# zenghjian/SceneSplat

Hardware: AMD Instinct MI355X
Metric: Gaussians/s encoder fwd+bwd, 102k-pt chunks (higher is better)
Workload: dtype bf16

## Files before the change

include/scenesplat_hip.h:

```cpp
#ifndef SCENESPLAT_HIP_H
#define SCENESPLAT_HIP_H
#include <stddef.h>
#include <stdint.h>

#ifdef __cplusplus
extern "C" {
#endif

struct ihipStream_t;
typedef struct ihipStream_t* ss_stream_t;

#define SS_MAX_ORDERS 8
enum { SS_ORDER_Z = 0, SS_ORDER_Z_TRANS = 1, SS_ORDER_HILBERT = 2, SS_ORDER_HILBERT_TRANS = 3 };
enum { SS_DTYPE_F32 = 0, SS_DTYPE_BF16 = 1 };
enum { SS_ATTN_SIMT = 0, SS_ATTN_MFMA = 1 };

int ss_version(void);

int ss_serialize_encode(const int32_t* grid_coord, const int32_t* batch, int64_t n, int depth, const int* orders,
                        int num_orders, int64_t* codes, ss_stream_t stream);
int ss_offsets_to_batch(const int32_t* offsets, int num_batches, int64_t n, int32_t* batch, ss_stream_t stream);
int ss_count_duplicates(const int64_t* sorted_keys, int64_t n, int32_t* count, ss_stream_t stream);
int ss_grid_coord_max(const int32_t* grid_coord, int64_t n, int32_t* out_max, ss_stream_t stream);
size_t ss_argsort_workspace_bytes(int64_t n, int num_segments);
int ss_argsort_i64(const int64_t* keys, int num_segments, int64_t n, int key_bits, int32_t* order_out,
                   int32_t* inverse_out, int64_t* sorted_keys_out, void* workspace, size_t workspace_bytes,
                   ss_stream_t stream);

size_t ss_pool_partition_workspace_bytes(int64_t n);
int ss_pool_partition(const int64_t* code0, const int32_t* order0, int64_t n, int shift_bits, int32_t* cluster,
                      int32_t* idx_ptr, int32_t* head, int32_t* n_out, void* workspace, size_t workspace_bytes,
                      ss_stream_t stream);
int ss_pool_level_attrs(const int32_t* head, int64_t n_out, int64_t n_in, const int32_t* grid_coord,
                        const int32_t* batch, const int64_t* codes, int num_orders, int pool_depth,
                        int32_t* grid_coord_out, int32_t* batch_out, int64_t* codes_out, ss_stream_t stream);
int ss_batch_offsets(const int32_t* batch, const int32_t* perm, int64_t n, int num_batches, int32_t* offsets,
                     ss_stream_t stream);

int ss_window_index(const int32_t* order, const int32_t* offsets, const int32_t* offsets_pad, int num_batches,
                    int patch_size, int64_t n_pad, int32_t* gidx, int32_t* sidx, ss_stream_t stream);
int ss_window_attn_fwd(const void* qkv, const int32_t* gidx, const int32_t* sidx, const int32_t* win_start,
                       int num_windows, int max_window, int64_t n, int64_t n_pad, int channels, int num_heads,
                       float scale, int dtype, int impl, void* out, float* lse, ss_stream_t stream);
size_t ss_window_attn_bwd_workspace_bytes(int64_t n, int64_t n_pad, int channels, int num_heads, int dtype);
int ss_window_attn_bwd(const void* qkv, const void* out, const void* dout, const float* lse, const int32_t* gidx,
                       const int32_t* sidx, const int32_t* win_start, int num_windows, int max_window, int64_t n,
                       int64_t n_pad, int channels, int num_heads, float scale, int dtype, int impl, void* dqkv,
                       void* workspace, size_t workspace_bytes, ss_stream_t stream);

int ss_cast_bf16_group(const int64_t* desc, const int32_t* wg_start, int nprob, int total_workgroups, ss_stream_t stream);
int ss_cast_bf16_group_elems_per_workgroup(void);

int ss_optim_group_elems_per_workgroup(void);
int ss_grad_sqnorm_group(const int64_t* desc, const int32_t* wg_start, int nprob, int total_workgroups, double* partials,
                         ss_stream_t stream);
int ss_grad_norm_finish(const double* partials, int num_partials, float max_norm, float* record, ss_stream_t stream);
int ss_adamw_group(const int64_t* desc, const int32_t* wg_start, int nprob, int total_workgroups, const float* record,
                   ss_stream_t stream);

int ss_pdnorm_channels_per_workgroup(void);
int ss_pdnorm_mod_fwd(const int64_t* table, const int32_t* wg_start, int num_layers, int total_workgroups, const float* context,
                      int context_channels, int vec4, ss_stream_t stream);
int ss_pdnorm_mod_bwd(const int64_t* table, const int32_t* wg_start, int num_layers, int total_workgroups, const float* context,
                      int context_channels, int vec4, int split_workgroup, float* partials, float* dcontext, ss_stream_t stream);

int ss_row_keep_scales(const int64_t* seed, const float* keep, float* out, int64_t n, ss_stream_t stream);

int ss_gelu(const void* x, const void* dy, void* out, int64_t numel, int dtype, ss_stream_t stream);

int ss_stream_capture_status(ss_stream_t stream);
unsigned long long ss_stream_capture_id(ss_stream_t stream);

int ss_linear_fwd_headmajor(const void* x, const int32_t* row_index, const void* weight, const float* bias, void* out_hm,
                            int64_t m, int k, int n_out, int channels, int head_dim, float sec0_scale, ss_stream_t stream);
int ss_headmajor_pack(const void* src, int in_dtype, const int32_t* gidx, void* hm, int64_t n_pad, int channels,
                      int num_heads, int sections, float sec0_scale, ss_stream_t stream);
int ss_window_attn_hm_fwd(const void* hm, const int32_t* sidx, const int32_t* win_start, int num_windows, int max_window,
                          int64_t n, int64_t n_pad, int channels, int num_heads, void* out, float* neg_lse2,
                          ss_stream_t stream);
size_t ss_window_attn_hm_bwd_workspace_bytes(int64_t n, int64_t n_pad, int channels, int num_heads);
int ss_window_attn_hm_bwd(const void* hm, const void* out, const void* dout, const float* neg_lse2, const int32_t* gidx,
                          const int32_t* sidx, const int32_t* win_start, int num_windows, int max_window, int64_t n,
                          int64_t n_pad, int channels, int num_heads, float scale, void* dqkv, void* workspace,
                          size_t workspace_bytes, ss_stream_t stream);

int ss_window_attn_rpe_fwd(const void* qkv, const int32_t* gidx, const int32_t* sidx, const int32_t* win_start,
                           int num_windows, int max_window, int64_t n, int64_t n_pad, int channels, int num_heads,
                           float scale, int dtype, int impl, const int32_t* grid_coord, const float* table, int pos_bnd,
                           void* out, float* lse, ss_stream_t stream);
size_t ss_window_attn_rpe_bwd_workspace_bytes(int64_t n, int64_t n_pad, int channels, int num_heads, int dtype,
                                              int num_windows, int max_window, int pos_bnd);
int ss_window_attn_rpe_bwd(const void* qkv, const void* out, const void* dout, const float* lse, const int32_t* gidx,
                           const int32_t* sidx, const int32_t* win_start, int num_windows, int max_window, int64_t n,
                           int64_t n_pad, int channels, int num_heads, float scale, int dtype, int impl,
                           const int32_t* grid_coord, const float* table, int pos_bnd, void* dqkv, float* dtable,
                           void* workspace, size_t workspace_bytes, ss_stream_t stream);

int ss_subm_rulebook(const int32_t* grid_coord, const int32_t* batch, int64_t n, int depth,
                     const int64_t* zkeys_sorted, const int32_t* zorder, int swap_xy, int kernel_size, int32_t* nbr,
                     ss_stream_t stream);
int ss_subm_tap_mask_keys(const int32_t* nbr, const int32_t* order, int64_t n, int taps, int coarse_bits, int64_t* keys,
                          ss_stream_t stream);
int64_t ss_subm_rulebook_table_size(int64_t n);
int ss_subm_rulebook_hashed(const int32_t* grid_coord, const int32_t* batch, int64_t n, int depth, int kernel_size, int32_t* nbr,
                            void* workspace, size_t workspace_bytes, ss_stream_t stream);

int ss_subm_conv_fwd(const void* in, const void* weight, const float* bias, const int32_t* nbr, const int32_t* rowperm,
                     void* out, int64_t n, int cin, int cout, int taps, int out_dtype, ss_stream_t stream);
int ss_subm_weight_mirror(const void* w, void* wt, int cout, int taps, int cin, ss_stream_t stream);
int ss_stream_create_cu_mask(int nwords, const uint32_t* mask, void** stream_out);
int ss_subm_im2col(const void* src, const int32_t* nbr, void* dst, int64_t n, int taps, int64_t row_bytes, ss_stream_t stream);
int ss_gemm8_ok(int64_t m, int k, int n, int taps);
int ss_subm_conv_fwd_pipe(const void* in, const void* weight, const float* bias, const int32_t* nbr, const int32_t* rowperm,
                          void* out, int64_t n, int cin, int cout, int taps, int out_dtype, ss_stream_t stream);
int ss_subm_conv_fwd_pipe_walk(const void* in, const void* weight, const float* bias, const int32_t* nbr_walk, const int32_t* rowperm,
                               void* out, int64_t n, int cin, int cout, int taps, int out_dtype, ss_stream_t stream);
int ss_subm_conv_fwd_uses_pipe(int64_t n, int cin, int cout, int taps);
int ss_subm_conv_fwd_walk(const void* in, const void* weight, const float* bias, const int32_t* nbr, const int32_t* nbr_walk,
                          const int32_t* rowperm, void* out, int64_t n, int cin, int cout, int taps, int out_dtype, ss_stream_t stream);
int ss_linear_fwd(const void* x, const void* weight, const float* bias, void* out, int64_t m, int k, int n, int out_dtype,
                  ss_stream_t stream);
int ss_wgrad_xcd_order(void);
int ss_wgrad_set_xcd_order(int on);
int ss_wgrad8_ok(int64_t n, int cin, int cout, int taps);
int ss_subm_conv_wgrad_pipe(const void* in, const void* dout, const int32_t* nbr, const int32_t* rowperm,
                            const int32_t* blk_count, const int32_t* blk_list, float* dweight, int64_t n, int cin, int cout,
                            int taps, ss_stream_t stream);
int ss_linear_wgrad(const void* x, const void* dy, float* dweight, float* dbias, int64_t m, int k_in, int n_out,
                    ss_stream_t stream);
int ss_linear_wgrad_group_plan(int64_t m, int k_in, int n_out, int64_t* desc_words);
int ss_linear_wgrad_tiles(int k_in, int n_out);
int ss_linear_wgrad_group_plan2(int64_t m, int k_in, int n_out, int launch_tiles, int64_t* desc_words);
int ss_linear_wgrad_group(const int64_t* desc, const int32_t* wg_start, int nprob, int total_workgroups, ss_stream_t stream);
int ss_subm_conv_splits(int64_t n, int cout, int taps);
int ss_subm_conv_fwd_splitk(const void* in, const void* weight, const float* bias, const int32_t* nbr, const int32_t* rowperm,
                            float* acc32, int64_t n, int cin, int cout, int taps, int splits, ss_stream_t stream);
int ss_subm_block_lists(const int32_t* nbr, const int32_t* rowperm, int64_t n, int taps, int32_t* blk_count,
                        int32_t* blk_list, ss_stream_t stream);
int ss_subm_conv_wgrad(const void* in, const void* dout, const int32_t* nbr, const int32_t* rowperm,
                       const int32_t* blk_count, const int32_t* blk_list, float* dweight, int64_t n, int cin, int cout,
                       int taps, ss_stream_t stream);

int ss_subm_f32_ok(int cin_padded, int cout);
int ss_subm_f32_fwd(const float* in, const float* wq, const float* bias, const int32_t* nbr_walk, const int32_t* rowperm,
                    float* out, int64_t n, int cin_padded, int cout, int taps, ss_stream_t stream);
int ss_subm_f32_dgrad_dup(const float* dout_folded, const float* wq, const int32_t* nbr_walk, const int32_t* rowperm, float* din,
                          int64_t n, int cin_padded, int cout, int taps, ss_stream_t stream);
int ss_subm_f32_wgrad(const float* in, const float* dout, const int32_t* nbr_walk, const int32_t* rowperm,
                      const int32_t* blk_count, const int32_t* blk_list, float* dweight, int64_t n, int cin_padded,
                      int cin, int cout, int taps, ss_stream_t stream);

int ss_subm_conv_wgrad_pipe_walk(const void* in, const void* dout, const int32_t* nbr_walk, const int32_t* rowperm,
                                 const int32_t* blk_count, const int32_t* blk_list, float* dweight, int64_t n, int cin, int cout,
                                 int taps, ss_stream_t stream);
int ss_subm_conv_wgrad_uses_pipe(int64_t n, int cin, int cout, int taps);
int ss_subm_conv_wgrad_walk(const void* in, const void* dout, const int32_t* nbr, const int32_t* nbr_walk, const int32_t* rowperm,
                            const int32_t* blk_count, const int32_t* blk_list, float* dweight, int64_t n, int cin, int cout,
                            int taps, ss_stream_t stream);

int ss_add_layernorm_fwd(const void* x, int x_dtype, const void* y, int y_dtype, const float* rowscale,
                         const float* gamma, const float* beta, float eps, void* xout, int xout_dtype, void* xcopy_bf16,
                         void* h, int h_dtype, float* mean, float* rstd, int64_t n, int channels, ss_stream_t stream);
int ss_ln_add_ln_fwd(const void* x, int x_dtype, const void* t, int t_dtype, const float* gamma0, const float* beta0, float eps0,
                     const float* gamma1, const float* beta1, float eps1, float* xout, void* h, int h_dtype, float* stats,
                     int64_t n, int channels, ss_stream_t stream);
int ss_ln_add_ln_bwd(const float* g_xout, const void* g_h, int g_h_dtype, const float* xout, const void* t, int t_dtype,
                     const float* stats, const float* gamma0, const float* gamma1, void* g_x, int g_x_dtype, void* g_t,
                     int g_t_dtype, float* part, int64_t n, int channels, int nblocks, ss_stream_t stream);
int ss_add_layernorm_bwd_blocks(int64_t n);
int ss_group_partial_sums_outputs_per_workgroup(void);
int ss_group_partial_sums(const int64_t* desc, const int32_t* wg_start, int nprob, int total_workgroups, ss_stream_t stream);
int ss_transpose16_group(const int64_t* desc, const int32_t* wg_start, int nprob, int total_workgroups, ss_stream_t stream);
int ss_subm_weight_mirror_group_tile(void);
int ss_subm_weight_mirror_group(const int64_t* desc, const int32_t* wg_start, int nprob, int total_workgroups, ss_stream_t stream);
int ss_add_layernorm_bwd(const void* g_xout, int g_xout_dtype, const void* g_xcopy, int g_xcopy_dtype, const void* g_h,
                         int g_h_dtype, const void* v, int v_dtype, const float* mean, const float* rstd,
                         const float* gamma, const float* rowscale, void* g_x, int g_x_dtype, void* g_y, int g_y_dtype,
                         float* dgamma_part, float* dbeta_part, int64_t n, int channels, int nblocks, ss_stream_t stream);

int ss_col_stats(const void* x, int x_dtype, float* shift_out, float* psum, float* psq, int64_t n, int channels,
                 int nblocks, ss_stream_t stream);
int ss_bn_stats_finish(const float* part, const float* shift, int nblocks, int channels, int64_t n, float momentum, float eps,
                       float* running_mean, float* running_var, int64_t* num_batches, float* mean, float* rstd,
                       ss_stream_t stream);
int ss_bn_bwd_finish(const float* part, int nblocks, int channels, int64_t n, float* sums, float* coef, ss_stream_t stream);
int ss_bn_act_fwd(const void* x, int x_dtype, const float* mean, const float* rstd, const float* gamma, const float* beta,
                  int act, void* y, int y_dtype, int64_t n, int channels, ss_stream_t stream);
int ss_bn_act_bwd_reduce(const void* dy, int dy_dtype, const void* x, int x_dtype, const float* mean, const float* rstd,
                         const float* gamma, const float* beta, int act, float* pdz, float* pdzx, int64_t n, int channels,
                         int nblocks, ss_stream_t stream);
int ss_bn_act_bwd_apply(const void* dy, int dy_dtype, const void* x, int x_dtype, const float* mean, const float* rstd,
                        const float* gamma, const float* beta, int act, const float* c1, const float* c2, void* dx,
                        int dx_dtype, int64_t n, int channels, ss_stream_t stream);

int ss_feat_text_scan(const void* feat_bf16, const void* text_bf16, int64_t n, int dim, int num_classes, float* max_prob,
                      int32_t* argmax, const int32_t* idx, float* pred_accum, ss_stream_t stream);

int ss_lang_head_blocks(int64_t n);
int ss_lang_head_fwd(const void* feat, int feat_dtype, const void* target, int target_dtype, const unsigned char* mask,
                     int normalize, void* p_out, int p_dtype, float* rowstat, float* part, float* sums, int64_t n,
                     int channels, ss_stream_t stream);
int ss_lang_head_bwd(const void* feat, int feat_dtype, const void* target, int target_dtype, const unsigned char* mask,
                     int normalize, const float* rowstat, const float* coef, const void* dp_extra, int dp_dtype,
                     void* dfeat, int dfeat_dtype, int64_t n, int channels, ss_stream_t stream);

size_t ss_seg_loss_workspace_bytes(int64_t n, int num_classes);
int ss_seg_loss_fwd(const void* logits, int dtype, const int64_t* labels, int64_t n, int num_classes, int64_t ignore_index,
                    const unsigned char* class_seen, int lovasz, float* rowstat, float* glov, int32_t* present, float* sums,
                    void* workspace, size_t workspace_bytes, ss_stream_t stream);
int ss_seg_loss_bwd(const void* logits, int dtype, const int64_t* labels, int64_t n, int num_classes, int64_t ignore_index,
                    const float* rowstat, const float* glov, const int32_t* present, const float* coef, void* dlogits,
                    ss_stream_t stream);
int ss_seg_iou(const void* logits, int dtype, const int32_t* pred, const int64_t* target, int64_t n, int num_classes,
               int64_t ignore_index, int64_t* out, ss_stream_t stream);

int ss_gather_rows(const void* src, const int32_t* idx, void* dst, int64_t n_dst, int64_t row_bytes, ss_stream_t stream);
int ss_scatter_rows(const void* src, const int32_t* idx, void* dst, int64_t n_src, int64_t row_bytes, ss_stream_t stream);
int ss_gather_add_rows(const void* a, const void* b, const int32_t* idx, void* dst, int64_t n, int channels, int dtype,
                       ss_stream_t stream);
int ss_dup_fold_rows(const void* src, const int64_t* sorted_keys, const int32_t* order, void* dst, int64_t n, int channels,
                     int dtype, ss_stream_t stream);
int ss_dup_zero_rows(const int64_t* sorted_keys, const int32_t* order, void* x, int64_t n, int64_t row_bytes, ss_stream_t stream);
int ss_segment_reduce(const void* src, const int32_t* indices, const int32_t* idx_ptr, void* out, int64_t n_seg,
                      int channels, int dtype, int mean, ss_stream_t stream);
int ss_segment_minmax(const void* src, const int32_t* indices, const int32_t* idx_ptr, void* out, int32_t* arg, int64_t n_seg,
                      int channels, int dtype, int is_max, ss_stream_t stream);
int ss_segment_minmax_bwd(const void* dout, const int32_t* arg, void* dsrc, int64_t n_seg, int channels, int dtype,
                          ss_stream_t stream);
int ss_segment_bcast(const void* dout, const int32_t* cluster, const int32_t* idx_ptr, void* dsrc, int64_t n,
                     int channels, int dtype, int mean, ss_stream_t stream);


int ss_aug_bbox_blocks(int64_t n);
int ss_aug_bbox(const float* x, int64_t n, const float* h_affine, float* partials, float* out6, ss_stream_t stream);
int ss_aug_gaussians(float* coord, float* quat, float* scale, float* normal, int64_t n, const float* h_affine,
                     const float* h_rquat, int flip, const float* h_scale_mul, const float* h_lin, int jitter, float jitter_sigma,
                     float jitter_clip, const float* noise, uint64_t seed, ss_stream_t stream);
int ss_aug_elastic(float* coord, int64_t n, const float* noise, int d0, int d1, int d2, const float* h_origin, float granularity,
                   float magnitude, ss_stream_t stream);
int ss_aug_color(float* color, int64_t n, int flags, const float* h_lo, const float* h_hi, float blend, const float* h_tr,
                 float jitter_std, const float* noise, uint64_t seed, int normalize, ss_stream_t stream);

int ss_knn_query(int m, int nsample, const float* xyz, const float* new_xyz, const int32_t* offset,
                 const int32_t* new_offset, int num_batches, int32_t* idx, float* dist2, ss_stream_t stream);
size_t ss_ball_query_workspace_bytes(int m);
int ss_ball_query(int m, int nsample, float min_radius, float max_radius, const float* xyz, const float* new_xyz,
                  const int32_t* offset, const int32_t* new_offset, int num_batches, int32_t* idx, float* dist2,
                  void* workspace, size_t workspace_bytes, ss_stream_t stream);
int ss_random_ball_query(int m, int nsample, float min_radius, float max_radius, const int32_t* order, const float* xyz,
                         const float* new_xyz, const int32_t* offset, const int32_t* new_offset, int num_batches,
                         int32_t* idx, float* dist2, ss_stream_t stream);
int ss_farthest_point_sampling(int num_batches, const float* xyz, const int32_t* offset, const int32_t* new_offset,
                               float* tmp, int32_t* idx, ss_stream_t stream);
int ss_grouping_fwd(int m, int nsample, int c, const float* input, const int32_t* idx, float* output, ss_stream_t stream);
int ss_grouping_bwd(int m, int nsample, int c, const float* grad_output, const int32_t* idx, float* grad_input, ss_stream_t stream);
int ss_subtraction_fwd(int n, int nsample, int c, const float* input1, const float* input2, const int32_t* idx, float* output, ss_stream_t stream);
int ss_subtraction_bwd(int n, int nsample, int c, const int32_t* idx, const float* grad_output, float* grad_input1, float* grad_input2, ss_stream_t stream);
int ss_aggregation_fwd(int n, int nsample, int c, int w_c, const float* input, const float* position, const float* weight, const int32_t* idx, float* output, ss_stream_t stream);
int ss_aggregation_bwd(int n, int nsample, int c, int w_c, const float* input, const float* position, const float* weight, const int32_t* idx, const float* grad_output, float* grad_input, float* grad_position, float* grad_weight, ss_stream_t stream);
int ss_interpolation_fwd(int n, int c, int k, const float* input, const int32_t* idx, const float* weight, float* output, ss_stream_t stream);
int ss_interpolation_bwd(int n, int c, int k, const float* grad_output, const int32_t* idx, const float* weight, float* grad_input, ss_stream_t stream);
int ss_attention_relation_fwd(int m, int g, int c, const float* query, const float* key, const float* weight, const int32_t* index_target, const int32_t* index_refer, float* output, ss_stream_t stream);
int ss_attention_relation_bwd(int m, int g, int c, const float* query, float* grad_query, const float* key, float* grad_key, const float* weight, float* grad_weight, const int32_t* index_target, const int32_t* index_refer, const float* grad_output, ss_stream_t stream);
int ss_attention_fusion_fwd(int m, int g, int c, const float* weight, const float* value, const int32_t* index_target, const int32_t* index_refer, float* output, ss_stream_t stream);
int ss_attention_fusion_bwd(int m, int g, int c, const float* weight, float* grad_weight, const float* value, float* grad_value, const int32_t* index_target, const int32_t* index_refer, const float* grad_output, ss_stream_t stream);
int ss_rpe_dot_prod_fwd(int n, int m, int h, int hdim, const float* q, const int32_t* index, const float* table, const int32_t* rel_idx, float* output, ss_stream_t stream);
int ss_rpe_dot_prod_bwd(int n, int m, int h, int hdim, const float* grad_out, const float* q, const int32_t* index, const float* table, const int32_t* rel_idx, float* grad_q, float* grad_table, ss_stream_t stream);
int ss_rpe_attn_step2_fwd(int n, int m, int h, int hdim, const float* attn, const float* v, const int32_t* index0, const int32_t* index1, const float* table, const int32_t* rel_idx, float* output, ss_stream_t stream);
int ss_rpe_attn_step2_bwd(int n, int m, int h, int hdim, const float* grad_out, const int32_t* index0, const int32_t* index1, const float* attn, const float* v, const float* table, const int32_t* rel_idx, float* grad_attn, float* grad_v, float* grad_table, ss_stream_t stream);
int64_t ss_knn_grid_table_size(int64_t n);
size_t ss_knn_grid_workspace_bytes(int64_t n);
int ss_knn_grid_keys(const float* xyz, const int32_t* offset, int num_batches, int64_t n, float origin_x, float origin_y, float origin_z,
                     float cell_size, int64_t* keys, ss_stream_t stream);
int ss_knn_grid_build(const float* xyz, const int64_t* sorted_keys, const int32_t* order, int64_t n, void* workspace,
                      size_t workspace_bytes, int32_t* ncell, ss_stream_t stream);
int ss_knn_grid_query(int m, int nsample, const float* new_xyz, const int32_t* qorder, const int32_t* offset, const int32_t* new_offset,
                      int num_batches, float origin_x, float origin_y, float origin_z, float cell_size, int dimx, int dimy, int dimz,
                      int64_t n, const void* workspace, int32_t* idx, float* dist2, ss_stream_t stream);
int ss_ball_grid_query(int m, int nsample, float min_radius, float max_radius, const float* xyz, const float* new_xyz,
                       const int32_t* qorder, const int32_t* offset, const int32_t* new_offset, int num_batches, float origin_x,
                       float origin_y, float origin_z, float cell_size, int dimx, int dimy, int dimz, int64_t n, const void* workspace,
                       int32_t* idx, float* dist2, ss_stream_t stream);
int ss_majority_vote(const int32_t* nn_idx, const int32_t* labels, int64_t m, int k, int ignore_label, int num_classes,
                     int32_t* out, ss_stream_t stream);
int ss_ballquery_batch_p(int n, int mean_active, float radius, const float* xyz, const int32_t* batch_idxs, const int32_t* batch_offsets, int32_t* idx, int32_t* start_len, int32_t* total, ss_stream_t stream);
int ss_bfs_cluster(const int32_t* semantic_label, const int32_t* ball_query_idxs, const int32_t* start_len, int n, int threshold, int32_t* cluster_idxs, int64_t cap_points, int32_t* cluster_offsets, int64_t cap_clusters, int32_t* n_clusters, int32_t* n_points);

#ifdef __cplusplus
}
#endif
#endif
```

scenesplat_amd/_lib.py:

```python
import ctypes
import os

import torch

_HERE = os.path.dirname(os.path.abspath(__file__))
LIB_PATH = os.path.join(_HERE, "lib", "libscenesplat_hip.so")

c_p = ctypes.c_void_p
c_i = ctypes.c_int
c_i64 = ctypes.c_int64
c_f = ctypes.c_float
c_sz = ctypes.c_size_t

PROTOTYPES = {
    "ss_version": (c_i, []),
    "ss_serialize_encode": (c_i, [c_p, c_p, c_i64, c_i, ctypes.POINTER(c_i), c_i, c_p, c_p]),
    "ss_offsets_to_batch": (c_i, [c_p, c_i, c_i64, c_p, c_p]),
    "ss_count_duplicates": (c_i, [c_p, c_i64, c_p, c_p]),
    "ss_grid_coord_max": (c_i, [c_p, c_i64, c_p, c_p]),
    "ss_argsort_workspace_bytes": (c_sz, [c_i64, c_i]),
    "ss_argsort_i64": (c_i, [c_p, c_i, c_i64, c_i, c_p, c_p, c_p, c_p, c_sz, c_p]),
    "ss_pool_partition_workspace_bytes": (c_sz, [c_i64]),
    "ss_pool_partition": (c_i, [c_p, c_p, c_i64, c_i, c_p, c_p, c_p, c_p, c_p, c_sz, c_p]),
    "ss_pool_level_attrs": (c_i, [c_p, c_i64, c_i64, c_p, c_p, c_p, c_i, c_i, c_p, c_p, c_p, c_p]),
    "ss_batch_offsets": (c_i, [c_p, c_p, c_i64, c_i, c_p, c_p]),
    "ss_window_index": (c_i, [c_p, c_p, c_p, c_i, c_i, c_i64, c_p, c_p, c_p]),
    "ss_window_attn_fwd": (c_i, [c_p, c_p, c_p, c_p, c_i, c_i, c_i64, c_i64, c_i, c_i, c_f, c_i, c_i, c_p, c_p, c_p]),
    "ss_window_attn_bwd_workspace_bytes": (c_sz, [c_i64, c_i64, c_i, c_i, c_i]),
    "ss_window_attn_bwd": (c_i, [c_p, c_p, c_p, c_p, c_p, c_p, c_p, c_i, c_i, c_i64, c_i64, c_i, c_i, c_f, c_i, c_i,
                                 c_p, c_p, c_sz, c_p]),
    "ss_window_attn_rpe_fwd": (c_i, [c_p, c_p, c_p, c_p, c_i, c_i, c_i64, c_i64, c_i, c_i, c_f, c_i, c_i, c_p, c_p, c_i,
                                     c_p, c_p, c_p]),
    "ss_window_attn_rpe_bwd_workspace_bytes": (c_sz, [c_i64, c_i64, c_i, c_i, c_i, c_i, c_i, c_i]),
    "ss_window_attn_rpe_bwd": (c_i, [c_p, c_p, c_p, c_p, c_p, c_p, c_p, c_i, c_i, c_i64, c_i64, c_i, c_i, c_f, c_i, c_i,
                                     c_p, c_p, c_i, c_p, c_p, c_p, c_sz, c_p]),
    "ss_gelu": (c_i, [c_p, c_p, c_p, c_i64, c_i, c_p]),
    "ss_row_keep_scales": (c_i, [c_p, c_p, c_p, c_i64, c_p]),
    "ss_stream_capture_status": (c_i, [c_p]),
    "ss_stream_capture_id": (ctypes.c_ulonglong, [c_p]),
    "ss_cast_bf16_group": (c_i, [c_p, c_p, c_i, c_i, c_p]),
    "ss_cast_bf16_group_elems_per_workgroup": (c_i, []),
    "ss_optim_group_elems_per_workgroup": (c_i, []),
    "ss_grad_sqnorm_group": (c_i, [c_p, c_p, c_i, c_i, c_p, c_p]),
    "ss_grad_norm_finish": (c_i, [c_p, c_i, c_f, c_p, c_p]),
    "ss_adamw_group": (c_i, [c_p, c_p, c_i, c_i, c_p, c_p]),
    "ss_pdnorm_channels_per_workgroup": (c_i, []),
    "ss_pdnorm_mod_fwd": (c_i, [c_p, c_p, c_i, c_i, c_p, c_i, c_i, c_p]),
    "ss_pdnorm_mod_bwd": (c_i, [c_p, c_p, c_i, c_i, c_p, c_i, c_i, c_i, c_p, c_p, c_p]),
    "ss_linear_fwd_headmajor": (c_i, [c_p, c_p, c_p, c_p, c_p, c_i64, c_i, c_i, c_i, c_i, c_f, c_p]),
    "ss_headmajor_pack": (c_i, [c_p, c_i, c_p, c_p, c_i64, c_i, c_i, c_i, c_f, c_p]),
    "ss_window_attn_hm_fwd": (c_i, [c_p, c_p, c_p, c_i, c_i, c_i64, c_i64, c_i, c_i, c_p, c_p, c_p]),
    "ss_window_attn_hm_bwd_workspace_bytes": (c_sz, [c_i64, c_i64, c_i, c_i]),
    "ss_window_attn_hm_bwd": (c_i, [c_p, c_p, c_p, c_p, c_p, c_p, c_p, c_i, c_i, c_i64, c_i64, c_i, c_i, c_f, c_p, c_p, c_sz, c_p]),
    "ss_subm_rulebook": (c_i, [c_p, c_p, c_i64, c_i, c_p, c_p, c_i, c_i, c_p, c_p]),
    "ss_subm_conv_fwd": (c_i, [c_p, c_p, c_p, c_p, c_p, c_p, c_i64, c_i, c_i, c_i, c_i, c_p]),
    "ss_stream_create_cu_mask": (c_i, [c_i, c_p, c_p]),
    "ss_ln_add_ln_fwd": (c_i, [c_p, c_i, c_p, c_i, c_p, c_p, c_f, c_p, c_p, c_f, c_p, c_p, c_i, c_p, c_i64, c_i, c_p]),
    "ss_ln_add_ln_bwd": (c_i, [c_p, c_p, c_i, c_p, c_p, c_i, c_p, c_p, c_p, c_p, c_i, c_p, c_i, c_p, c_i64, c_i, c_i, c_p]),
    "ss_segment_minmax": (c_i, [c_p, c_p, c_p, c_p, c_p, c_i64, c_i, c_i, c_i, c_p]),
    "ss_segment_minmax_bwd": (c_i, [c_p, c_p, c_p, c_i64, c_i, c_i, c_p]),
    "ss_subm_rulebook_table_size": (c_i64, [c_i64]),
    "ss_subm_rulebook_hashed": (c_i, [c_p, c_p, c_i64, c_i, c_i, c_p, c_p, ctypes.c_size_t, c_p]),
    "ss_subm_tap_mask_keys": (c_i, [c_p, c_p, c_i64, c_i, c_i, c_p, c_p]),
    "ss_subm_weight_mirror": (c_i, [c_p, c_p, c_i, c_i, c_i, c_p]),
    "ss_subm_im2col": (c_i, [c_p, c_p, c_p, c_i64, c_i, c_i64, c_p]),
    "ss_gemm8_ok": (c_i, [c_i64, c_i, c_i, c_i]),
    "ss_subm_conv_fwd_pipe": (c_i, [c_p, c_p, c_p, c_p, c_p, c_p, c_i64, c_i, c_i, c_i, c_i, c_p]),
    "ss_linear_fwd": (c_i, [c_p, c_p, c_p, c_p, c_i64, c_i, c_i, c_i, c_p]),
    "ss_wgrad_xcd_order": (c_i, []),
    "ss_wgrad_set_xcd_order": (c_i, [c_i]),
    "ss_wgrad8_ok": (c_i, [c_i64, c_i, c_i, c_i]),
    "ss_subm_conv_wgrad_pipe": (c_i, [c_p, c_p, c_p, c_p, c_p, c_p, c_p, c_i64, c_i, c_i, c_i, c_p]),
    "ss_linear_wgrad": (c_i, [c_p, c_p, c_p, c_p, c_i64, c_i, c_i, c_p]),
    "ss_linear_wgrad_group_plan": (c_i, [c_i64, c_i, c_i, c_p]),
    "ss_linear_wgrad_tiles": (c_i, [c_i, c_i]),
    "ss_linear_wgrad_group_plan2": (c_i, [c_i64, c_i, c_i, c_i, c_p]),
    "ss_linear_wgrad_group": (c_i, [c_p, c_p, c_i, c_i, c_p]),
    "ss_subm_conv_splits": (c_i, [c_i64, c_i, c_i]),
    "ss_subm_conv_fwd_splitk": (c_i, [c_p, c_p, c_p, c_p, c_p, c_p, c_i64, c_i, c_i, c_i, c_i, c_p]),
    "ss_subm_block_lists": (c_i, [c_p, c_p, c_i64, c_i, c_p, c_p, c_p]),
    "ss_subm_conv_wgrad": (c_i, [c_p, c_p, c_p, c_p, c_p, c_p, c_p, c_i64, c_i, c_i, c_i, c_p]),
    "ss_subm_conv_fwd_pipe_walk": (c_i, [c_p, c_p, c_p, c_p, c_p, c_p, c_i64, c_i, c_i, c_i, c_i, c_p]),
    "ss_subm_conv_fwd_uses_pipe": (c_i, [c_i64, c_i, c_i, c_i]),
    "ss_subm_conv_fwd_walk": (c_i, [c_p, c_p, c_p, c_p, c_p, c_p, c_p, c_i64, c_i, c_i, c_i, c_i, c_p]),
    "ss_subm_conv_wgrad_pipe_walk": (c_i, [c_p, c_p, c_p, c_p, c_p, c_p, c_p, c_i64, c_i, c_i, c_i, c_p]),
    "ss_subm_conv_wgrad_uses_pipe": (c_i, [c_i64, c_i, c_i, c_i]),
    "ss_subm_conv_wgrad_walk": (c_i, [c_p, c_p, c_p, c_p, c_p, c_p, c_p, c_p, c_i64, c_i, c_i, c_i, c_p]),
    "ss_subm_f32_ok": (c_i, [c_i, c_i]),
    "ss_subm_f32_fwd": (c_i, [c_p, c_p, c_p, c_p, c_p, c_p, c_i64, c_i, c_i, c_i, c_p]),
    "ss_subm_f32_dgrad_dup": (c_i, [c_p, c_p, c_p, c_p, c_p, c_i64, c_i, c_i, c_i, c_p]),
    "ss_dup_fold_rows": (c_i, [c_p, c_p, c_p, c_p, c_i64, c_i, c_i, c_p]),
    "ss_dup_zero_rows": (c_i, [c_p, c_p, c_p, c_i64, c_i64, c_p]),
    "ss_subm_f32_wgrad": (c_i, [c_p, c_p, c_p, c_p, c_p, c_p, c_p, c_i64, c_i, c_i, c_i, c_i, c_p]),
    "ss_add_layernorm_fwd": (c_i, [c_p, c_i, c_p, c_i, c_p, c_p, c_p, c_f, c_p, c_i, c_p, c_p, c_i, c_p, c_p, c_i64, c_i, c_p]),
    "ss_add_layernorm_bwd_blocks": (c_i, [c_i64]),
    "ss_group_partial_sums_outputs_per_workgroup": (c_i, []),
    "ss_group_partial_sums": (c_i, [c_p, c_p, c_i, c_i, c_p]),
    "ss_transpose16_group": (c_i, [c_p, c_p, c_i, c_i, c_p]),
    "ss_subm_weight_mirror_group_tile": (c_i, []),
    "ss_subm_weight_mirror_group": (c_i, [c_p, c_p, c_i, c_i, c_p]),
    "ss_add_layernorm_bwd": (c_i, [c_p, c_i, c_p, c_i, c_p, c_i, c_p, c_i, c_p, c_p, c_p, c_p, c_p, c_i, c_p, c_i, c_p, c_p,
                                   c_i64, c_i, c_i, c_p]),
    "ss_col_stats": (c_i, [c_p, c_i, c_p, c_p, c_p, c_i64, c_i, c_i, c_p]),
    "ss_bn_stats_finish": (c_i, [c_p, c_p, c_i, c_i, c_i64, c_f, c_f, c_p, c_p, c_p, c_p, c_p, c_p]),
    "ss_bn_bwd_finish": (c_i, [c_p, c_i, c_i, c_i64, c_p, c_p, c_p]),
    "ss_bn_act_fwd": (c_i, [c_p, c_i, c_p, c_p, c_p, c_p, c_i, c_p, c_i, c_i64, c_i, c_p]),
    "ss_bn_act_bwd_reduce": (c_i, [c_p, c_i, c_p, c_i, c_p, c_p, c_p, c_p, c_i, c_p, c_p, c_i64, c_i, c_i, c_p]),
    "ss_bn_act_bwd_apply": (c_i, [c_p, c_i, c_p, c_i, c_p, c_p, c_p, c_p, c_i, c_p, c_p, c_p, c_i, c_i64, c_i, c_p]),
    "ss_feat_text_scan": (c_i, [c_p, c_p, c_i64, c_i, c_i, c_p, c_p, c_p, c_p, c_p]),
    "ss_lang_head_blocks": (c_i, [c_i64]),
    "ss_lang_head_fwd": (c_i, [c_p, c_i, c_p, c_i, c_p, c_i, c_p, c_i, c_p, c_p, c_p, c_i64, c_i, c_p]),
    "ss_lang_head_bwd": (c_i, [c_p, c_i, c_p, c_i, c_p, c_i, c_p, c_p, c_p, c_i, c_p, c_i, c_i64, c_i, c_p]),
    "ss_seg_loss_workspace_bytes": (c_sz, [c_i64, c_i]),
    "ss_seg_loss_fwd": (c_i, [c_p, c_i, c_p, c_i64, c_i, c_i64, c_p, c_i, c_p, c_p, c_p, c_p, c_p, c_sz, c_p]),
    "ss_seg_loss_bwd": (c_i, [c_p, c_i, c_p, c_i64, c_i, c_i64, c_p, c_p, c_p, c_p, c_p, c_p]),
    "ss_seg_iou": (c_i, [c_p, c_i, c_p, c_p, c_i64, c_i, c_i64, c_p, c_p]),
    "ss_gather_rows": (c_i, [c_p, c_p, c_p, c_i64, c_i64, c_p]),
    "ss_scatter_rows": (c_i, [c_p, c_p, c_p, c_i64, c_i64, c_p]),
    "ss_gather_add_rows": (c_i, [c_p, c_p, c_p, c_p, c_i64, c_i, c_i, c_p]),
    "ss_segment_reduce": (c_i, [c_p, c_p, c_p, c_p, c_i64, c_i, c_i, c_i, c_p]),
    "ss_segment_bcast": (c_i, [c_p, c_p, c_p, c_p, c_i64, c_i, c_i, c_i, c_p]),
    "ss_aug_bbox_blocks": (c_i, [c_i64]),
    "ss_aug_bbox": (c_i, [c_p, c_i64, c_p, c_p, c_p, c_p]),
    "ss_aug_gaussians": (c_i, [c_p, c_p, c_p, c_p, c_i64, c_p, c_p, c_i, c_p, c_p, c_i, c_f, c_f, c_p, ctypes.c_uint64, c_p]),
    "ss_aug_elastic": (c_i, [c_p, c_i64, c_p, c_i, c_i, c_i, c_p, c_f, c_f, c_p]),
    "ss_aug_color": (c_i, [c_p, c_i64, c_i, c_p, c_p, c_f, c_p, c_f, c_p, ctypes.c_uint64, c_i, c_p]),
    "ss_knn_grid_table_size": (c_i64, [c_i64]),
    "ss_knn_grid_workspace_bytes": (c_sz, [c_i64]),
    "ss_knn_grid_keys": (c_i, [c_p, c_p, c_i, c_i64, c_f, c_f, c_f, c_f, c_p, c_p]),
    "ss_knn_grid_build": (c_i, [c_p, c_p, c_p, c_i64, c_p, c_sz, c_p, c_p]),
    "ss_knn_grid_query": (c_i, [c_i, c_i, c_p, c_p, c_p, c_p, c_i, c_f, c_f, c_f, c_f, c_i, c_i, c_i, c_i64, c_p, c_p, c_p, c_p]),
    "ss_ball_grid_query": (c_i, [c_i, c_i, c_f, c_f, c_p, c_p, c_p, c_p, c_p, c_i, c_f, c_f, c_f, c_f, c_i, c_i, c_i, c_i64, c_p, c_p, c_p, c_p]),
    "ss_knn_query": (c_i, [c_i, c_i, c_p, c_p, c_p, c_p, c_i, c_p, c_p, c_p]),
    "ss_ball_query_workspace_bytes": (c_sz, [c_i]),
    "ss_ball_query": (c_i, [c_i, c_i, c_f, c_f, c_p, c_p, c_p, c_p, c_i, c_p, c_p, c_p, c_sz, c_p]),
    "ss_random_ball_query": (c_i, [c_i, c_i, c_f, c_f, c_p, c_p, c_p, c_p, c_p, c_i, c_p, c_p, c_p]),
    "ss_farthest_point_sampling": (c_i, [c_i, c_p, c_p, c_p, c_p, c_p, c_p]),
    "ss_grouping_fwd": (c_i, [c_i, c_i, c_i, c_p, c_p, c_p, c_p]),
    "ss_grouping_bwd": (c_i, [c_i, c_i, c_i, c_p, c_p, c_p, c_p]),
    "ss_subtraction_fwd": (c_i, [c_i, c_i, c_i, c_p, c_p, c_p, c_p, c_p]),
    "ss_subtraction_bwd": (c_i, [c_i, c_i, c_i, c_p, c_p, c_p, c_p, c_p]),
    "ss_aggregation_fwd": (c_i, [c_i, c_i, c_i, c_i, c_p, c_p, c_p, c_p, c_p, c_p]),
    "ss_aggregation_bwd": (c_i, [c_i, c_i, c_i, c_i, c_p, c_p, c_p, c_p, c_p, c_p, c_p, c_p, c_p]),
    "ss_interpolation_fwd": (c_i, [c_i, c_i, c_i, c_p, c_p, c_p, c_p, c_p]),
    "ss_interpolation_bwd": (c_i, [c_i, c_i, c_i, c_p, c_p, c_p, c_p, c_p]),
    "ss_attention_relation_fwd": (c_i, [c_i, c_i, c_i, c_p, c_p, c_p, c_p, c_p, c_p, c_p]),
    "ss_attention_relation_bwd": (c_i, [c_i, c_i, c_i, c_p, c_p, c_p, c_p, c_p, c_p, c_p, c_p, c_p, c_p]),
    "ss_attention_fusion_fwd": (c_i, [c_i, c_i, c_i, c_p, c_p, c_p, c_p, c_p, c_p]),
    "ss_attention_fusion_bwd": (c_i, [c_i, c_i, c_i, c_p, c_p, c_p, c_p, c_p, c_p, c_p, c_p]),
    "ss_rpe_dot_prod_fwd": (c_i, [c_i, c_i, c_i, c_i, c_p, c_p, c_p, c_p, c_p, c_p]),
    "ss_rpe_dot_prod_bwd": (c_i, [c_i, c_i, c_i, c_i, c_p, c_p, c_p, c_p, c_p, c_p, c_p, c_p]),
    "ss_rpe_attn_step2_fwd": (c_i, [c_i, c_i, c_i, c_i, c_p, c_p, c_p, c_p, c_p, c_p, c_p, c_p]),
    "ss_rpe_attn_step2_bwd": (c_i, [c_i, c_i, c_i, c_i, c_p, c_p, c_p, c_p, c_p, c_p, c_p, c_p, c_p, c_p, c_p]),
    "ss_majority_vote": (c_i, [c_p, c_p, c_i64, c_i, c_i, c_i, c_p, c_p]),
    "ss_ballquery_batch_p": (c_i, [c_i, c_i, c_f, c_p, c_p, c_p, c_p, c_p, c_p, c_p]),
    "ss_bfs_cluster": (c_i, [c_p, c_p, c_p, c_i, c_i, c_p, c_i64, c_p, c_i64, c_p, c_p]),
}

_lib = None


def load():
    global _lib
    if _lib is not None:
        return _lib
    if not os.path.exists(LIB_PATH):
        raise RuntimeError(
            f"{LIB_PATH} is missing: build it with `python -m scenesplat_amd.build` "
            "(hipcc --offload-arch=gfx950). scenesplat_amd has no CPU fallback.")
    lib = ctypes.CDLL(LIB_PATH)
    for name, (res, args) in PROTOTYPES.items():
        fn = getattr(lib, name)
        fn.restype = res
        fn.argtypes = args
    _lib = lib
    return lib


class NativeError(RuntimeError):
    pass


_STATUS = {1: "bad argument", 2: "kernel launch failed", 3: "workspace too small"}


def check(rc, name):
    if rc != 0:
        raise NativeError(f"{name} failed: status {rc} ({_STATUS.get(rc, 'unknown')})")
```

scenesplat_amd/csrc/norm.hip:

```cpp
#include "common.h"
#include "../../include/scenesplat_hip.h"

#define LN_THREADS 256
#define LN_MAXIT 4

__device__ __forceinline__ float4 ln_ld4(const void* p, int dtype, int64_t idx) {
  if (dtype == SS_F32) return *reinterpret_cast<const float4*>((const float*)p + idx);
  uint2 u = *reinterpret_cast<const uint2*>((const unsigned short*)p + idx);
  return make_float4(__uint_as_float(u.x << 16), __uint_as_float(u.x & 0xffff0000u), __uint_as_float(u.y << 16),
                     __uint_as_float(u.y & 0xffff0000u));
}
__device__ __forceinline__ void ln_st4(void* p, int dtype, int64_t idx, float4 v) {
  if (dtype == SS_F32) { *reinterpret_cast<float4*>((float*)p + idx) = v; return; }
  uint2 u; u.x = pack_bf16x2(v.x, v.y); u.y = pack_bf16x2(v.z, v.w);
  *reinterpret_cast<uint2*>((unsigned short*)p + idx) = u;
}

template <int IT>
__global__ void __launch_bounds__(LN_THREADS)
k_add_ln_fwd(const void* __restrict__ x, int x_dt, const void* __restrict__ y, int y_dt, const float* __restrict__ rowscale,
             const float* __restrict__ gamma, const float* __restrict__ beta, float eps, void* __restrict__ xout, int xout_dt,
             void* __restrict__ xcopy, void* __restrict__ h, int h_dt, float* __restrict__ mean, float* __restrict__ rstd,
             int64_t n, int C) {
  const int lane = threadIdx.x & 63;
  const int64_t row = (int64_t)blockIdx.x * (LN_THREADS / 64) + (threadIdx.x >> 6);
  if (row >= n) return;
  const float rs = rowscale ? rowscale[row] : 1.f;
  float4 v[IT];
  float sum = 0.f;
#pragma unroll
  for (int i = 0; i < IT; ++i) {
    int j = i * 256 + lane * 4;
    v[i] = make_float4(0.f, 0.f, 0.f, 0.f);
    if (j < C) {
      float4 a = ln_ld4(x, x_dt, row * C + j);
      if (y) { float4 b = ln_ld4(y, y_dt, row * C + j); a.x += rs * b.x; a.y += rs * b.y; a.z += rs * b.z; a.w += rs * b.w; }
      v[i] = a;
      if (xout) ln_st4(xout, xout_dt, row * C + j, a);
      if (xcopy) ln_st4(xcopy, SS_BF16, row * C + j, a);
      sum += a.x + a.y + a.z + a.w;
    }
  }
  if (!gamma) return;
  const float mu = wave_reduce_sum(sum) / C;
  float sq = 0.f;
#pragma unroll
  for (int i = 0; i < IT; ++i) {
    int j = i * 256 + lane * 4;
    if (j < C) {
      float dx = v[i].x - mu, dy = v[i].y - mu, dz = v[i].z - mu, dw = v[i].w - mu;
      sq += dx * dx + dy * dy + dz * dz + dw * dw;
    }
  }
  const float r = rsqrtf(wave_reduce_sum(sq) / C + eps);
  if (lane == 0) { mean[row] = mu; rstd[row] = r; }
#pragma unroll
  for (int i = 0; i < IT; ++i) {
    int j = i * 256 + lane * 4;
    if (j < C) {
      float4 g = *reinterpret_cast<const float4*>(gamma + j), b = *reinterpret_cast<const float4*>(beta + j);
      float4 o = make_float4((v[i].x - mu) * r * g.x + b.x, (v[i].y - mu) * r * g.y + b.y, (v[i].z - mu) * r * g.z + b.z,
                             (v[i].w - mu) * r * g.w + b.w);
      ln_st4(h, h_dt, row * C + j, o);
    }
  }
}

template <int IT>
__global__ void __launch_bounds__(LN_THREADS)
k_add_ln_bwd(const void* __restrict__ g_xout, int gxo_dt, const void* __restrict__ g_xcopy, int gxc_dt,
             const void* __restrict__ g_h, int gh_dt,
             const void* __restrict__ v_in, int v_dt, const float* __restrict__ mean, const float* __restrict__ rstd,
             const float* __restrict__ gamma, const float* __restrict__ rowscale, void* __restrict__ g_x, int gx_dt,
             void* __restrict__ g_y, int gy_dt, float* __restrict__ dgamma_part, float* __restrict__ dbeta_part, int64_t n,
             int C) {
  __shared__ float red[2][LN_THREADS / 64][LN_MAXIT * 256 / 64][64];
  const int lane = threadIdx.x & 63, wave = threadIdx.x >> 6;
  const int waves_total = gridDim.x * (LN_THREADS / 64);
  const bool ln = g_h != nullptr;
  float4 dg[IT], db[IT], gm[IT];
#pragma unroll
  for (int i = 0; i < IT; ++i) {
    dg[i] = make_float4(0.f, 0.f, 0.f, 0.f); db[i] = dg[i]; gm[i] = dg[i];
    int j = i * 256 + lane * 4;
    if (ln && j < C) gm[i] = *reinterpret_cast<const float4*>(gamma + j);
  }
  for (int64_t row = (int64_t)blockIdx.x * (LN_THREADS / 64) + wave; row < n; row += waves_total) {
    float4 gv[IT];
    if (ln) {
      const float mu = mean[row], r = rstd[row];
      float4 xh[IT], gy[IT];
      float c1 = 0.f, c2 = 0.f;
#pragma unroll
      for (int i = 0; i < IT; ++i) {
        int j = i * 256 + lane * 4;
        xh[i] = make_float4(0.f, 0.f, 0.f, 0.f); gy[i] = xh[i];
        if (j < C) {
          float4 a = ln_ld4(v_in, v_dt, row * C + j), g = ln_ld4(g_h, gh_dt, row * C + j);
          xh[i] = make_float4((a.x - mu) * r, (a.y - mu) * r, (a.z - mu) * r, (a.w - mu) * r);
          gy[i] = make_float4(g.x * gm[i].x, g.y * gm[i].y, g.z * gm[i].z, g.w * gm[i].w);
          c1 += gy[i].x + gy[i].y + gy[i].z + gy[i].w;
          c2 += gy[i].x * xh[i].x + gy[i].y * xh[i].y + gy[i].z * xh[i].z + gy[i].w * xh[i].w;
          dg[i].x += g.x * xh[i].x; dg[i].y += g.y * xh[i].y; dg[i].z += g.z * xh[i].z; dg[i].w += g.w * xh[i].w;
          db[i].x += g.x; db[i].y += g.y; db[i].z += g.z; db[i].w += g.w;
        }
      }
      c1 = wave_reduce_sum(c1) / C; c2 = wave_reduce_sum(c2) / C;
#pragma unroll
      for (int i = 0; i < IT; ++i)
        gv[i] = make_float4(r * (gy[i].x - c1 - xh[i].x * c2), r * (gy[i].y - c1 - xh[i].y * c2),
                            r * (gy[i].z - c1 - xh[i].z * c2), r * (gy[i].w - c1 - xh[i].w * c2));
    } else {
#pragma unroll
      for (int i = 0; i < IT; ++i) gv[i] = make_float4(0.f, 0.f, 0.f, 0.f);
    }
    const float rs = rowscale ? rowscale[row] : 1.f;
#pragma unroll
    for (int i = 0; i < IT; ++i) {
      int j = i * 256 + lane * 4;
      if (j < C) {
        if (g_xout) { float4 e = ln_ld4(g_xout, gxo_dt, row * C + j); gv[i].x += e.x; gv[i].y += e.y; gv[i].z += e.z; gv[i].w += e.w; }
        if (g_xcopy) { float4 e = ln_ld4(g_xcopy, gxc_dt, row * C + j); gv[i].x += e.x; gv[i].y += e.y; gv[i].z += e.z; gv[i].w += e.w; }
        if (g_x) ln_st4(g_x, gx_dt, row * C + j, gv[i]);
        if (g_y) ln_st4(g_y, gy_dt, row * C + j, make_float4(rs * gv[i].x, rs * gv[i].y, rs * gv[i].z, rs * gv[i].w));
      }
    }
  }
  if (!ln) return;
#pragma unroll
  for (int i = 0; i < IT; ++i) {
    red[0][wave][i * 4 + 0][lane] = dg[i].x; red[0][wave][i * 4 + 1][lane] = dg[i].y;
    red[0][wave][i * 4 + 2][lane] = dg[i].z; red[0][wave][i * 4 + 3][lane] = dg[i].w;
    red[1][wave][i * 4 + 0][lane] = db[i].x; red[1][wave][i * 4 + 1][lane] = db[i].y;
    red[1][wave][i * 4 + 2][lane] = db[i].z; red[1][wave][i * 4 + 3][lane] = db[i].w;
  }
  __syncthreads();
  if (wave == 0) {
#pragma unroll
    for (int i = 0; i < IT; ++i)
#pragma unroll
      for (int e = 0; e < 4; ++e) {
        int j = i * 256 + lane * 4 + e;
        if (j < C) {
          float a = 0.f, b = 0.f;
          for (int w = 0; w < LN_THREADS / 64; ++w) { a += red[0][w][i * 4 + e][lane]; b += red[1][w][i * 4 + e][lane]; }
          dgamma_part[(int64_t)blockIdx.x * C + j] = a;
          dbeta_part[(int64_t)blockIdx.x * C + j] = b;
        }
      }
  }
}

extern "C" int ss_add_layernorm_fwd(const void* x, int x_dtype, const void* y, int y_dtype, const float* rowscale,
                                    const float* gamma, const float* beta, float eps, void* xout, int xout_dtype,
                                    void* xcopy_bf16, void* h, int h_dtype, float* mean, float* rstd, int64_t n, int channels,
                                    hipStream_t stream) {
  if (n < 0 || channels <= 0 || (channels & 3) || channels > LN_MAXIT * 256) return SS_ERR_ARG;
  if (gamma && (!beta || !h || !mean || !rstd)) return SS_ERR_ARG;
  if (n == 0) return SS_OK;
  dim3 g(ss_div_up(n, LN_THREADS / 64)), b(LN_THREADS);
  const int it = (channels + 255) / 256;
#define SS_LN_FWD(ITN) SS_LAUNCH(k_add_ln_fwd<ITN>, g, b, 0, stream, x, x_dtype, y, y_dtype, rowscale, gamma, beta, eps, xout, xout_dtype, xcopy_bf16, h, h_dtype, mean, rstd, n, channels)
  switch (it) { case 1: SS_LN_FWD(1); break; case 2: SS_LN_FWD(2); break; case 3: SS_LN_FWD(3); break; default: SS_LN_FWD(4); break; }
#undef SS_LN_FWD
  return SS_OK;
}

extern "C" int ss_add_layernorm_bwd_blocks(int64_t n) {
  const int rows_per_wave = n >= 32768 ? 8 : 2;
  int64_t b = (n + (LN_THREADS / 64) * rows_per_wave - 1) / ((LN_THREADS / 64) * rows_per_wave);
  if (b > 1024) b = 1024;
  if (b < 1) b = 1;
  return (int)b;
}

extern "C" int ss_add_layernorm_bwd(const void* g_xout, int g_xout_dtype, const void* g_xcopy, int g_xcopy_dtype,
                                    const void* g_h, int g_h_dtype, const void* v,
                                    int v_dtype, const float* mean, const float* rstd, const float* gamma,
                                    const float* rowscale, void* g_x, int g_x_dtype, void* g_y, int g_y_dtype,
                                    float* dgamma_part, float* dbeta_part, int64_t n, int channels, int nblocks,
                                    hipStream_t stream) {
  if (n < 0 || channels <= 0 || (channels & 3) || channels > LN_MAXIT * 256 || nblocks < 1) return SS_ERR_ARG;
  if (g_h && (!v || !mean || !rstd || !gamma || !dgamma_part || !dbeta_part)) return SS_ERR_ARG;
  if (n == 0) return SS_OK;
  dim3 g(nblocks), b(LN_THREADS);
  const int it = (channels + 255) / 256;
#define SS_LN_BWD(ITN) SS_LAUNCH(k_add_ln_bwd<ITN>, g, b, 0, stream, g_xout, g_xout_dtype, g_xcopy, g_xcopy_dtype, g_h, g_h_dtype, v, v_dtype, mean, rstd, gamma, rowscale, g_x, g_x_dtype, g_y, g_y_dtype, dgamma_part, dbeta_part, n, channels)
  switch (it) { case 1: SS_LN_BWD(1); break; case 2: SS_LN_BWD(2); break; case 3: SS_LN_BWD(3); break; default: SS_LN_BWD(4); break; }
#undef SS_LN_BWD
  return SS_OK;
}

template <int IT>
__global__ void __launch_bounds__(LN_THREADS)
k_ln_add_ln_fwd(const void* __restrict__ x, int x_dt, const void* __restrict__ t, int t_dt, const float* __restrict__ gamma0,
                const float* __restrict__ beta0, float eps0, const float* __restrict__ gamma1, const float* __restrict__ beta1,
                float eps1, float* __restrict__ xout, void* __restrict__ h, int h_dt, float* __restrict__ stats, int64_t n,
                int C) {
  const int lane = threadIdx.x & 63;
  const int64_t row = (int64_t)blockIdx.x * (LN_THREADS / 64) + (threadIdx.x >> 6);
  if (row >= n) return;
  float4 v[IT];
  float sum = 0.f;
#pragma unroll
  for (int i = 0; i < IT; ++i) {
    int j = i * 256 + lane * 4;
    v[i] = make_float4(0.f, 0.f, 0.f, 0.f);
    if (j < C) { v[i] = ln_ld4(t, t_dt, row * C + j); sum += v[i].x + v[i].y + v[i].z + v[i].w; }
  }
  const float mu0 = wave_reduce_sum(sum) / C;
  float sq = 0.f;
#pragma unroll
  for (int i = 0; i < IT; ++i) {
    int j = i * 256 + lane * 4;
    if (j < C) { float a = v[i].x - mu0, b = v[i].y - mu0, c = v[i].z - mu0, d = v[i].w - mu0; sq += a * a + b * b + c * c + d * d; }
  }
  const float r0 = rsqrtf(wave_reduce_sum(sq) / C + eps0);
  sum = 0.f;
#pragma unroll
  for (int i = 0; i < IT; ++i) {
    int j = i * 256 + lane * 4;
    if (j < C) {
      float4 g = *reinterpret_cast<const float4*>(gamma0 + j), b = *reinterpret_cast<const float4*>(beta0 + j);
      float4 a = ln_ld4(x, x_dt, row * C + j);
      a.x += (v[i].x - mu0) * r0 * g.x + b.x; a.y += (v[i].y - mu0) * r0 * g.y + b.y;
      a.z += (v[i].z - mu0) * r0 * g.z + b.z; a.w += (v[i].w - mu0) * r0 * g.w + b.w;
      v[i] = a;
      *reinterpret_cast<float4*>(xout + row * C + j) = a;
      sum += a.x + a.y + a.z + a.w;
    }
  }
  const float mu1 = wave_reduce_sum(sum) / C;
  sq = 0.f;
#pragma unroll
  for (int i = 0; i < IT; ++i) {
    int j = i * 256 + lane * 4;
    if (j < C) { float a = v[i].x - mu1, b = v[i].y - mu1, c = v[i].z - mu1, d = v[i].w - mu1; sq += a * a + b * b + c * c + d * d; }
  }
  const float r1 = rsqrtf(wave_reduce_sum(sq) / C + eps1);
  if (lane == 0) *reinterpret_cast<float4*>(stats + row * 4) = make_float4(mu0, r0, mu1, r1);
#pragma unroll
  for (int i = 0; i < IT; ++i) {
    int j = i * 256 + lane * 4;
    if (j < C) {
      float4 g = *reinterpret_cast<const float4*>(gamma1 + j), b = *reinterpret_cast<const float4*>(beta1 + j);
      ln_st4(h, h_dt, row * C + j, make_float4((v[i].x - mu1) * r1 * g.x + b.x, (v[i].y - mu1) * r1 * g.y + b.y,
                                               (v[i].z - mu1) * r1 * g.z + b.z, (v[i].w - mu1) * r1 * g.w + b.w));
    }
  }
}

#define LN_ROW_BWD(XH, GY, R, OUT)                                                                        \
  {                                                                                                       \
    float c1_ = 0.f, c2_ = 0.f;                                                                           \
    _Pragma("unroll") for (int i = 0; i < IT; ++i) {                                                      \
      c1_ += GY[i].x + GY[i].y + GY[i].z + GY[i].w;                                                       \
      c2_ += GY[i].x * XH[i].x + GY[i].y * XH[i].y + GY[i].z * XH[i].z + GY[i].w * XH[i].w;               \
    }                                                                                                     \
    c1_ = wave_reduce_sum(c1_) / C; c2_ = wave_reduce_sum(c2_) / C;                                       \
    _Pragma("unroll") for (int i = 0; i < IT; ++i)                                                        \
      OUT[i] = make_float4(R * (GY[i].x - c1_ - XH[i].x * c2_), R * (GY[i].y - c1_ - XH[i].y * c2_),      \
                           R * (GY[i].z - c1_ - XH[i].z * c2_), R * (GY[i].w - c1_ - XH[i].w * c2_));     \
  }

template <int IT>
__global__ void __launch_bounds__(LN_THREADS, (IT <= 3 ? 4 : 2))
k_ln_add_ln_bwd(const float* __restrict__ g_xout, const void* __restrict__ g_h, int gh_dt, const float* __restrict__ xout,
                const void* __restrict__ t, int t_dt, const float* __restrict__ stats, const float* __restrict__ gamma0,
                const float* __restrict__ gamma1, void* __restrict__ g_x, int gx_dt, void* __restrict__ g_t, int gt_dt,
                float* __restrict__ part , int64_t n, int C) {
  __shared__ float red[2][LN_THREADS / 64][IT * 4][64];
  const int lane = threadIdx.x & 63, wave = threadIdx.x >> 6;
  const int waves_total = gridDim.x * (LN_THREADS / 64);
  __shared__ __attribute__((aligned(16))) float gam[2][IT * 256];
  for (int j = threadIdx.x; j < IT * 256; j += LN_THREADS) { gam[0][j] = j < C ? gamma0[j] : 0.f; gam[1][j] = j < C ? gamma1[j] : 0.f; }
  __syncthreads();
  float4 dg0[IT], db0[IT], dg1[IT], db1[IT];
#pragma unroll
  for (int i = 0; i < IT; ++i) { dg0[i] = make_float4(0.f, 0.f, 0.f, 0.f); db0[i] = dg0[i]; dg1[i] = dg0[i]; db1[i] = dg0[i]; }
  for (int64_t row = (int64_t)blockIdx.x * (LN_THREADS / 64) + wave; row < n; row += waves_total) {
    const float4 st = *reinterpret_cast<const float4*>(stats + row * 4);
    float4 xh[IT], gy[IT], gv[IT];
#pragma unroll
    for (int i = 0; i < IT; ++i) {
      int j = i * 256 + lane * 4;
      xh[i] = make_float4(0.f, 0.f, 0.f, 0.f); gy[i] = xh[i];
      if (j < C) {
        float4 a = *reinterpret_cast<const float4*>(xout + row * C + j), g = make_float4(0.f, 0.f, 0.f, 0.f);
        if (g_h) g = ln_ld4(g_h, gh_dt, row * C + j);
        xh[i] = make_float4((a.x - st.z) * st.w, (a.y - st.z) * st.w, (a.z - st.z) * st.w, (a.w - st.z) * st.w);
        const float4 gm1 = *reinterpret_cast<const float4*>(&gam[1][j]);
        gy[i] = make_float4(g.x * gm1.x, g.y * gm1.y, g.z * gm1.z, g.w * gm1.w);
        dg1[i].x += g.x * xh[i].x; dg1[i].y += g.y * xh[i].y; dg1[i].z += g.z * xh[i].z; dg1[i].w += g.w * xh[i].w;
        db1[i].x += g.x; db1[i].y += g.y; db1[i].z += g.z; db1[i].w += g.w;
      }
    }
    LN_ROW_BWD(xh, gy, st.w, gv)
#pragma unroll
    for (int i = 0; i < IT; ++i) {
      int j = i * 256 + lane * 4;
      if (j < C) {
        if (g_xout) { float4 e = *reinterpret_cast<const float4*>(g_xout + row * C + j); gv[i].x += e.x; gv[i].y += e.y; gv[i].z += e.z; gv[i].w += e.w; }
        ln_st4(g_x, gx_dt, row * C + j, gv[i]);
      } else {
        gv[i] = make_float4(0.f, 0.f, 0.f, 0.f);
      }
    }
#pragma unroll
    for (int i = 0; i < IT; ++i) {
      int j = i * 256 + lane * 4;
      xh[i] = make_float4(0.f, 0.f, 0.f, 0.f); gy[i] = xh[i];
      if (j < C) {
        float4 a = ln_ld4(t, t_dt, row * C + j);
        xh[i] = make_float4((a.x - st.x) * st.y, (a.y - st.x) * st.y, (a.z - st.x) * st.y, (a.w - st.x) * st.y);
        const float4 gm0 = *reinterpret_cast<const float4*>(&gam[0][j]);
        gy[i] = make_float4(gv[i].x * gm0.x, gv[i].y * gm0.y, gv[i].z * gm0.z, gv[i].w * gm0.w);
        dg0[i].x += gv[i].x * xh[i].x; dg0[i].y += gv[i].y * xh[i].y; dg0[i].z += gv[i].z * xh[i].z; dg0[i].w += gv[i].w * xh[i].w;
        db0[i].x += gv[i].x; db0[i].y += gv[i].y; db0[i].z += gv[i].z; db0[i].w += gv[i].w;
      }
    }
    LN_ROW_BWD(xh, gy, st.y, gv)
#pragma unroll
    for (int i = 0; i < IT; ++i) {
      int j = i * 256 + lane * 4;
      if (j < C) ln_st4(g_t, gt_dt, row * C + j, gv[i]);
    }
  }
#pragma unroll
  for (int round = 0; round < 2; ++round) {
    if (round) __syncthreads();
#pragma unroll
    for (int i = 0; i < IT; ++i) {
      const float4 a = round ? dg1[i] : dg0[i], b = round ? db1[i] : db0[i];
      red[0][wave][i * 4 + 0][lane] = a.x; red[0][wave][i * 4 + 1][lane] = a.y; red[0][wave][i * 4 + 2][lane] = a.z; red[0][wave][i * 4 + 3][lane] = a.w;
      red[1][wave][i * 4 + 0][lane] = b.x; red[1][wave][i * 4 + 1][lane] = b.y; red[1][wave][i * 4 + 2][lane] = b.z; red[1][wave][i * 4 + 3][lane] = b.w;
    }
    __syncthreads();
    if (wave < 2) {
      const int q = wave;
#pragma unroll
      for (int i = 0; i < IT; ++i)
#pragma unroll
        for (int e = 0; e < 4; ++e) {
          int j = i * 256 + lane * 4 + e;
          if (j < C) {
            float acc = 0.f;
            for (int w = 0; w < LN_THREADS / 64; ++w) acc += red[q][w][i * 4 + e][lane];
            part[((int64_t)(2 * round + q) * gridDim.x + blockIdx.x) * C + j] = acc;
          }
        }
    }
  }
}
#undef LN_ROW_BWD

extern "C" int ss_ln_add_ln_fwd(const void* x, int x_dtype, const void* t, int t_dtype, const float* gamma0, const float* beta0,
                                float eps0, const float* gamma1, const float* beta1, float eps1, float* xout, void* h,
                                int h_dtype, float* stats, int64_t n, int channels, hipStream_t stream) {
  if (n < 0 || channels <= 0 || (channels & 3) || channels > LN_MAXIT * 256) return SS_ERR_ARG;
  if (!x || !t || !gamma0 || !beta0 || !gamma1 || !beta1 || !xout || !h || !stats) return SS_ERR_ARG;
  if (n == 0) return SS_OK;
  dim3 g(ss_div_up(n, LN_THREADS / 64)), b(LN_THREADS);
#define SS_LN2_FWD(ITN) SS_LAUNCH(k_ln_add_ln_fwd<ITN>, g, b, 0, stream, x, x_dtype, t, t_dtype, gamma0, beta0, eps0, gamma1, beta1, eps1, xout, h, h_dtype, stats, n, channels)
  switch ((channels + 255) / 256) { case 1: SS_LN2_FWD(1); break; case 2: SS_LN2_FWD(2); break; case 3: SS_LN2_FWD(3); break; default: SS_LN2_FWD(4); break; }
#undef SS_LN2_FWD
  return SS_OK;
}

extern "C" int ss_ln_add_ln_bwd(const float* g_xout, const void* g_h, int g_h_dtype, const float* xout, const void* t, int t_dtype,
                                const float* stats, const float* gamma0, const float* gamma1, void* g_x, int g_x_dtype, void* g_t,
                                int g_t_dtype, float* part, int64_t n, int channels, int nblocks, hipStream_t stream) {
  if (n < 0 || channels <= 0 || (channels & 3) || channels > LN_MAXIT * 256 || nblocks < 1) return SS_ERR_ARG;
  if (!xout || !t || !stats || !gamma0 || !gamma1 || !g_x || !g_t || !part || (!g_xout && !g_h)) return SS_ERR_ARG;
  if (n == 0) return SS_OK;
  dim3 g(nblocks), b(LN_THREADS);
#define SS_LN2_BWD(ITN) SS_LAUNCH(k_ln_add_ln_bwd<ITN>, g, b, 0, stream, g_xout, g_h, g_h_dtype, xout, t, t_dtype, stats, gamma0, gamma1, g_x, g_x_dtype, g_t, g_t_dtype, part, n, channels)
  switch ((channels + 255) / 256) { case 1: SS_LN2_BWD(1); break; case 2: SS_LN2_BWD(2); break; case 3: SS_LN2_BWD(3); break; default: SS_LN2_BWD(4); break; }
#undef SS_LN2_BWD
  return SS_OK;
}

__device__ __forceinline__ float gelu_f(float z) { return 0.5f * z * (1.f + erff(z * 0.70710678118654752f)); }
__device__ __forceinline__ float dgelu_f(float z) {
  return 0.5f * (1.f + erff(z * 0.70710678118654752f)) + z * 0.3989422804014327f * __expf(-0.5f * z * z);
}

template <int IT>
__device__ __forceinline__ void col_partials_store(float4 (&a)[IT], float4 (&b)[IT], float* pa, float* pb, int C) {
  __shared__ float red[2][LN_THREADS / 64][IT * 4][64];
  const int lane = threadIdx.x & 63, wave = threadIdx.x >> 6;
#pragma unroll
  for (int i = 0; i < IT; ++i) {
    red[0][wave][i * 4 + 0][lane] = a[i].x; red[0][wave][i * 4 + 1][lane] = a[i].y;
    red[0][wave][i * 4 + 2][lane] = a[i].z; red[0][wave][i * 4 + 3][lane] = a[i].w;
    red[1][wave][i * 4 + 0][lane] = b[i].x; red[1][wave][i * 4 + 1][lane] = b[i].y;
    red[1][wave][i * 4 + 2][lane] = b[i].z; red[1][wave][i * 4 + 3][lane] = b[i].w;
  }
  __syncthreads();
  if (wave == 0) {
#pragma unroll
    for (int i = 0; i < IT; ++i)
#pragma unroll
      for (int e = 0; e < 4; ++e) {
        int j = i * 256 + lane * 4 + e;
        if (j < C) {
          float s0 = 0.f, s1 = 0.f;
          for (int w = 0; w < LN_THREADS / 64; ++w) { s0 += red[0][w][i * 4 + e][lane]; s1 += red[1][w][i * 4 + e][lane]; }
          pa[(int64_t)blockIdx.x * C + j] = s0;
          pb[(int64_t)blockIdx.x * C + j] = s1;
        }
      }
  }
}

template <int IT>
__global__ void __launch_bounds__(LN_THREADS)
k_col_stats(const void* __restrict__ x, int x_dt, float* __restrict__ shift_out, float* __restrict__ psum,
            float* __restrict__ psq, int64_t n, int C) {
  const int lane = threadIdx.x & 63, wave = threadIdx.x >> 6;
  const int waves_total = gridDim.x * (LN_THREADS / 64);
  float4 s[IT], q[IT], sh[IT];
#pragma unroll
  for (int i = 0; i < IT; ++i) {
    s[i] = make_float4(0.f, 0.f, 0.f, 0.f); q[i] = s[i]; sh[i] = s[i];
    int j = i * 256 + lane * 4;
    if (n > 0 && j < C) {
      sh[i] = ln_ld4(x, x_dt, j);
      if (shift_out && blockIdx.x == 0 && wave == 0) *reinterpret_cast<float4*>(shift_out + j) = sh[i];
    }
  }
  for (int64_t row = (int64_t)blockIdx.x * (LN_THREADS / 64) + wave; row < n; row += waves_total) {
#pragma unroll
    for (int i = 0; i < IT; ++i) {
      int j = i * 256 + lane * 4;
      if (j < C) {
        float4 a = ln_ld4(x, x_dt, row * C + j);
        a.x -= sh[i].x; a.y -= sh[i].y; a.z -= sh[i].z; a.w -= sh[i].w;
        s[i].x += a.x; s[i].y += a.y; s[i].z += a.z; s[i].w += a.w;
        q[i].x += a.x * a.x; q[i].y += a.y * a.y; q[i].z += a.z * a.z; q[i].w += a.w * a.w;
      }
    }
  }
  col_partials_store<IT>(s, q, psum, psq, C);
}

template <int IT>
__global__ void __launch_bounds__(LN_THREADS)
k_bn_act_fwd(const void* __restrict__ x, int x_dt, const float* __restrict__ mean, const float* __restrict__ rstd,
             const float* __restrict__ gamma, const float* __restrict__ beta, int act, void* __restrict__ y, int y_dt,
             int64_t n, int C) {
  const int lane = threadIdx.x & 63;
  const int64_t row = (int64_t)blockIdx.x * (LN_THREADS / 64) + (threadIdx.x >> 6);
  if (row >= n) return;
#pragma unroll
  for (int i = 0; i < IT; ++i) {
    int j = i * 256 + lane * 4;
    if (j < C) {
      float4 a = ln_ld4(x, x_dt, row * C + j);
      float4 m = *reinterpret_cast<const float4*>(mean + j), r = *reinterpret_cast<const float4*>(rstd + j);
      float4 g = *reinterpret_cast<const float4*>(gamma + j), b = *reinterpret_cast<const float4*>(beta + j);
      float4 z = make_float4((a.x - m.x) * r.x * g.x + b.x, (a.y - m.y) * r.y * g.y + b.y, (a.z - m.z) * r.z * g.z + b.z,
                             (a.w - m.w) * r.w * g.w + b.w);
      if (act) z = make_float4(gelu_f(z.x), gelu_f(z.y), gelu_f(z.z), gelu_f(z.w));
      ln_st4(y, y_dt, row * C + j, z);
    }
  }
}

template <int IT>
__global__ void __launch_bounds__(LN_THREADS)
k_bn_act_bwd_reduce(const void* __restrict__ dy, int dy_dt, const void* __restrict__ x, int x_dt,
                    const float* __restrict__ mean, const float* __restrict__ rstd, const float* __restrict__ gamma,
                    const float* __restrict__ beta, int act, float* __restrict__ pdz, float* __restrict__ pdzx, int64_t n,
                    int C) {
  const int lane = threadIdx.x & 63, wave = threadIdx.x >> 6;
  const int waves_total = gridDim.x * (LN_THREADS / 64);
  float4 s[IT], q[IT], m[IT], r[IT], g[IT], b[IT];
#pragma unroll
  for (int i = 0; i < IT; ++i) {
    s[i] = make_float4(0.f, 0.f, 0.f, 0.f); q[i] = s[i]; m[i] = s[i]; r[i] = s[i]; g[i] = s[i]; b[i] = s[i];
    int j = i * 256 + lane * 4;
    if (j < C) {
      m[i] = *reinterpret_cast<const float4*>(mean + j); r[i] = *reinterpret_cast<const float4*>(rstd + j);
      g[i] = *reinterpret_cast<const float4*>(gamma + j); b[i] = *reinterpret_cast<const float4*>(beta + j);
    }
  }
  for (int64_t row = (int64_t)blockIdx.x * (LN_THREADS / 64) + wave; row < n; row += waves_total) {
#pragma unroll
    for (int i = 0; i < IT; ++i) {
      int j = i * 256 + lane * 4;
      if (j < C) {
        float4 a = ln_ld4(x, x_dt, row * C + j), d = ln_ld4(dy, dy_dt, row * C + j);
        float4 xh = make_float4((a.x - m[i].x) * r[i].x, (a.y - m[i].y) * r[i].y, (a.z - m[i].z) * r[i].z, (a.w - m[i].w) * r[i].w);
        if (act) {
          d.x *= dgelu_f(xh.x * g[i].x + b[i].x); d.y *= dgelu_f(xh.y * g[i].y + b[i].y);
          d.z *= dgelu_f(xh.z * g[i].z + b[i].z); d.w *= dgelu_f(xh.w * g[i].w + b[i].w);
        }
        s[i].x += d.x; s[i].y += d.y; s[i].z += d.z; s[i].w += d.w;
        q[i].x += d.x * xh.x; q[i].y += d.y * xh.y; q[i].z += d.z * xh.z; q[i].w += d.w * xh.w;
      }
    }
  }
  col_partials_store<IT>(s, q, pdz, pdzx, C);
}

template <int IT>
__global__ void __launch_bounds__(LN_THREADS)
k_bn_act_bwd_apply(const void* __restrict__ dy, int dy_dt, const void* __restrict__ x, int x_dt,
                   const float* __restrict__ mean, const float* __restrict__ rstd, const float* __restrict__ gamma,
                   const float* __restrict__ beta, int act, const float* __restrict__ c1, const float* __restrict__ c2,
                   void* __restrict__ dx, int dx_dt, int64_t n, int C) {
  const int lane = threadIdx.x & 63;
  const int64_t row = (int64_t)blockIdx.x * (LN_THREADS / 64) + (threadIdx.x >> 6);
  if (row >= n) return;
#pragma unroll
  for (int i = 0; i < IT; ++i) {
    int j = i * 256 + lane * 4;
    if (j < C) {
      float4 a = ln_ld4(x, x_dt, row * C + j), d = ln_ld4(dy, dy_dt, row * C + j);
      float4 m = *reinterpret_cast<const float4*>(mean + j), r = *reinterpret_cast<const float4*>(rstd + j);
      float4 g = *reinterpret_cast<const float4*>(gamma + j), b = *reinterpret_cast<const float4*>(beta + j);
      float4 k1 = c1 ? *reinterpret_cast<const float4*>(c1 + j) : make_float4(0.f, 0.f, 0.f, 0.f);
      float4 k2 = c2 ? *reinterpret_cast<const float4*>(c2 + j) : make_float4(0.f, 0.f, 0.f, 0.f);
      float4 xh = make_float4((a.x - m.x) * r.x, (a.y - m.y) * r.y, (a.z - m.z) * r.z, (a.w - m.w) * r.w);
      if (act) {
        d.x *= dgelu_f(xh.x * g.x + b.x); d.y *= dgelu_f(xh.y * g.y + b.y);
        d.z *= dgelu_f(xh.z * g.z + b.z); d.w *= dgelu_f(xh.w * g.w + b.w);
      }
      float4 o = make_float4(g.x * r.x * (d.x - k1.x - xh.x * k2.x), g.y * r.y * (d.y - k1.y - xh.y * k2.y),
                             g.z * r.z * (d.z - k1.z - xh.z * k2.z), g.w * r.w * (d.w - k1.w - xh.w * k2.w));
      ln_st4(dx, dx_dt, row * C + j, o);
    }
  }
}

#define BNF_THREADS 1024
__device__ __forceinline__ void bnf_reduce(const float* __restrict__ part, int nb, int C, int c, int rg, float& s, float& q) {
  __shared__ float sh[2][32][33];
  float a = 0.f, b_ = 0.f;
  if (c < C) {
#pragma unroll 4
    for (int b = rg; b < nb; b += 32) { a += part[(int64_t)b * C + c]; b_ += part[((int64_t)nb + b) * C + c]; }
  }
  const int cl = threadIdx.x & 31;
  sh[0][rg][cl] = a; sh[1][rg][cl] = b_;
  __syncthreads();
  s = 0.f; q = 0.f;
  if (rg == 0) {
#pragma unroll
    for (int r = 0; r < 32; ++r) { s += sh[0][r][cl]; q += sh[1][r][cl]; }
  }
}
__global__ void __launch_bounds__(BNF_THREADS)
k_bn_stats_finish(const float* __restrict__ part, const float* __restrict__ shift , int nb, int C,
                  float n, float unbias, float momentum, float eps, float* __restrict__ running_mean, float* __restrict__ running_var,
                  long long* __restrict__ num_batches, float* __restrict__ mean, float* __restrict__ rstd) {
  const int c = blockIdx.x * 32 + (threadIdx.x & 31), rg = threadIdx.x >> 5;
  if (blockIdx.x == 0 && threadIdx.x == 0 && num_batches) *num_batches += 1;
  float s, q;
  bnf_reduce(part, nb, C, c, rg, s, q);
  if (rg != 0 || c >= C) return;
  const float d = s / n;
  const float m = (shift ? shift[c] : 0.f) + d;
  const float var = fmaxf(q / n - d * d, 0.f);
  mean[c] = m;
  rstd[c] = rsqrtf(var + eps);
  if (running_mean) {
    running_mean[c] = running_mean[c] * (1.f - momentum) + m * momentum;
    running_var[c] = running_var[c] * (1.f - momentum) + (var * unbias) * momentum;
  }
}
__global__ void __launch_bounds__(BNF_THREADS)
k_bn_bwd_finish(const float* __restrict__ part, int nb, int C, float n, float* __restrict__ sums, float* __restrict__ coef) {
  const int c = blockIdx.x * 32 + (threadIdx.x & 31), rg = threadIdx.x >> 5;
  float a, b_;
  bnf_reduce(part, nb, C, c, rg, a, b_);
  if (rg != 0 || c >= C) return;
  sums[c] = a; sums[C + c] = b_;
  if (coef) { coef[c] = a / n; coef[C + c] = b_ / n; }
}

#define SS_IT_SWITCH(MACRO) switch (it) { case 1: MACRO(1); break; case 2: MACRO(2); break; case 3: MACRO(3); break; default: MACRO(4); break; }

extern "C" int ss_col_stats(const void* x, int x_dtype, float* shift_out, float* psum, float* psq, int64_t n, int channels,
                            int nblocks, hipStream_t stream) {
  if (n < 0 || channels <= 0 || (channels & 3) || channels > LN_MAXIT * 256 || nblocks < 1) return SS_ERR_ARG;
  const int it = (channels + 255) / 256;
#define SS_CS(ITN) SS_LAUNCH(k_col_stats<ITN>, dim3(nblocks), dim3(LN_THREADS), 0, stream, x, x_dtype, shift_out, psum, psq, n, channels)
  SS_IT_SWITCH(SS_CS)
#undef SS_CS
  return SS_OK;
}
extern "C" int ss_bn_act_fwd(const void* x, int x_dtype, const float* mean, const float* rstd, const float* gamma,
                             const float* beta, int act, void* y, int y_dtype, int64_t n, int channels, hipStream_t stream) {
  if (n < 0 || channels <= 0 || (channels & 3) || channels > LN_MAXIT * 256) return SS_ERR_ARG;
  if (n == 0) return SS_OK;
  const int it = (channels + 255) / 256;
  dim3 g(ss_div_up(n, LN_THREADS / 64)), b(LN_THREADS);
#define SS_BF(ITN) SS_LAUNCH(k_bn_act_fwd<ITN>, g, b, 0, stream, x, x_dtype, mean, rstd, gamma, beta, act, y, y_dtype, n, channels)
  SS_IT_SWITCH(SS_BF)
#undef SS_BF
  return SS_OK;
}
extern "C" int ss_bn_act_bwd_reduce(const void* dy, int dy_dtype, const void* x, int x_dtype, const float* mean,
                                    const float* rstd, const float* gamma, const float* beta, int act, float* pdz, float* pdzx,
                                    int64_t n, int channels, int nblocks, hipStream_t stream) {
  if (n < 0 || channels <= 0 || (channels & 3) || channels > LN_MAXIT * 256 || nblocks < 1) return SS_ERR_ARG;
  const int it = (channels + 255) / 256;
#define SS_BR(ITN) SS_LAUNCH(k_bn_act_bwd_reduce<ITN>, dim3(nblocks), dim3(LN_THREADS), 0, stream, dy, dy_dtype, x, x_dtype, mean, rstd, gamma, beta, act, pdz, pdzx, n, channels)
  SS_IT_SWITCH(SS_BR)
#undef SS_BR
  return SS_OK;
}
extern "C" int ss_bn_act_bwd_apply(const void* dy, int dy_dtype, const void* x, int x_dtype, const float* mean,
                                   const float* rstd, const float* gamma, const float* beta, int act, const float* c1,
                                   const float* c2, void* dx, int dx_dtype, int64_t n, int channels, hipStream_t stream) {
  if (n < 0 || channels <= 0 || (channels & 3) || channels > LN_MAXIT * 256) return SS_ERR_ARG;
  if (n == 0) return SS_OK;
  const int it = (channels + 255) / 256;
  dim3 g(ss_div_up(n, LN_THREADS / 64)), b(LN_THREADS);
#define SS_BA(ITN) SS_LAUNCH(k_bn_act_bwd_apply<ITN>, g, b, 0, stream, dy, dy_dtype, x, x_dtype, mean, rstd, gamma, beta, act, c1, c2, dx, dx_dtype, n, channels)
  SS_IT_SWITCH(SS_BA)
#undef SS_BA
  return SS_OK;
}


#define GPS_COLS 32
__global__ void __launch_bounds__(256)
k_group_partial_sums(const int64_t* __restrict__ desc, const int32_t* __restrict__ wg_start, int nprob) {
  __shared__ float red[8][GPS_COLS];
  const int b = blockIdx.x;
  int p = 0;
  while (p + 1 < nprob && wg_start[p + 1] <= b) ++p;
  const int64_t* d = desc + (int64_t)p * 4;
  const float* part = reinterpret_cast<const float*>(d[0]);
  float* dst = reinterpret_cast<float*>(d[1]);
  const int nb = (int)d[2];
  const int C = (int)((uint64_t)d[3] & 0xffffffffu), KC = (int)((uint64_t)d[3] >> 32);
  const int cg = threadIdx.x & (GPS_COLS - 1), rg = threadIdx.x / GPS_COLS;
  const int j = (b - wg_start[p]) * GPS_COLS + cg;
  float a0 = 0.f, a1 = 0.f, a2 = 0.f, a3 = 0.f;
  if (j < KC) {
    const int k = j / C, c = j - k * C;
    const float* src = part + (int64_t)k * nb * C + c;
    int bb = rg;
    for (; bb + 24 < nb; bb += 32) {
      a0 += src[(int64_t)bb * C]; a1 += src[(int64_t)(bb + 8) * C]; a2 += src[(int64_t)(bb + 16) * C]; a3 += src[(int64_t)(bb + 24) * C];
    }
    for (; bb < nb; bb += 8) a0 += src[(int64_t)bb * C];
  }
  red[rg][cg] = (a0 + a1) + (a2 + a3);
  __syncthreads();
  if (rg == 0 && j < KC) {
    float s = 0.f;
#pragma unroll
    for (int r = 0; r < 8; ++r) s += red[r][cg];
    dst[j] = s;
  }
}

extern "C" int ss_group_partial_sums_outputs_per_workgroup(void) { return GPS_COLS; }
extern "C" int ss_group_partial_sums(const int64_t* desc, const int32_t* wg_start, int nprob, int total_workgroups,
                                     ss_stream_t stream) {
  if (nprob <= 0 || total_workgroups <= 0) return SS_OK;
  if (!desc || !wg_start) return SS_ERR_ARG;
  SS_LAUNCH(k_group_partial_sums, dim3((unsigned)total_workgroups), dim3(256), 0, stream, desc, wg_start, nprob);
  return SS_OK;
}

extern "C" int ss_bn_stats_finish(const float* part, const float* shift, int nblocks, int channels, int64_t n, float momentum,
                                  float eps, float* running_mean, float* running_var, int64_t* num_batches, float* mean,
                                  float* rstd, hipStream_t stream) {
  if (!part || !mean || !rstd || nblocks < 1 || channels <= 0 || n <= 0 || ((running_mean == nullptr) != (running_var == nullptr)))
    return SS_ERR_ARG;
  const float unbias = (float)((double)n / (double)(n > 1 ? n - 1 : 1));
  SS_LAUNCH(k_bn_stats_finish, dim3(ss_div_up(channels, 32)), dim3(BNF_THREADS), 0, stream, part, shift, nblocks, channels, (float)n,
            unbias, momentum, eps, running_mean, running_var, (long long*)num_batches, mean, rstd);
  return SS_OK;
}
extern "C" int ss_bn_bwd_finish(const float* part, int nblocks, int channels, int64_t n, float* sums, float* coef,
                                hipStream_t stream) {
  if (!part || !sums || nblocks < 1 || channels <= 0 || n <= 0) return SS_ERR_ARG;
  SS_LAUNCH(k_bn_bwd_finish, dim3(ss_div_up(channels, 32)), dim3(BNF_THREADS), 0, stream, part, nblocks, channels, (float)n, sums, coef);
  return SS_OK;
}


__device__ __forceinline__ float dgelu_exact(float z) {
  return 0.5f * (1.f + erff(z * 0.70710678118654752f)) + z * 0.3989422804014327f * expf(-0.5f * z * z);
}
__device__ __forceinline__ void bf8_unpack(const uint4& u, float (&v)[8]) {
  v[0] = __uint_as_float(u.x << 16); v[1] = __uint_as_float(u.x & 0xffff0000u); v[2] = __uint_as_float(u.y << 16); v[3] = __uint_as_float(u.y & 0xffff0000u);
  v[4] = __uint_as_float(u.z << 16); v[5] = __uint_as_float(u.z & 0xffff0000u); v[6] = __uint_as_float(u.w << 16); v[7] = __uint_as_float(u.w & 0xffff0000u);
}
__device__ __forceinline__ uint4 bf8_pack(const float (&v)[8]) {
  uint4 o; o.x = pack_bf16x2(v[0], v[1]); o.y = pack_bf16x2(v[2], v[3]); o.z = pack_bf16x2(v[4], v[5]); o.w = pack_bf16x2(v[6], v[7]);
  return o;
}

template <bool BWD>
__global__ void __launch_bounds__(256)
k_gelu_bf16(const unsigned short* __restrict__ x, const unsigned short* __restrict__ dy, unsigned short* __restrict__ out, int64_t n) {
  const int64_t i = ((int64_t)blockIdx.x * 256 + threadIdx.x) * 8;
  if (i + 8 <= n) {
    float a[8], g[8], r[8];
    bf8_unpack(*reinterpret_cast<const uint4*>(x + i), a);
    if (BWD) bf8_unpack(*reinterpret_cast<const uint4*>(dy + i), g);
#pragma unroll
    for (int e = 0; e < 8; ++e) r[e] = BWD ? g[e] * dgelu_exact(a[e]) : gelu_f(a[e]);
    *reinterpret_cast<uint4*>(out + i) = bf8_pack(r);
  } else {
    for (int64_t k = i; k < n; ++k) {
      const float a = bf16_to_f32(x[k]);
      out[k] = f32_to_bf16(BWD ? bf16_to_f32(dy[k]) * dgelu_exact(a) : gelu_f(a));
    }
  }
}
template <bool BWD>
__global__ void __launch_bounds__(256)
k_gelu_f32(const float* __restrict__ x, const float* __restrict__ dy, float* __restrict__ out, int64_t n) {
  const int64_t i = ((int64_t)blockIdx.x * 256 + threadIdx.x) * 4;
  if (i + 4 <= n) {
    const float4 a = *reinterpret_cast<const float4*>(x + i);
    float4 g = make_float4(1.f, 1.f, 1.f, 1.f);
    if (BWD) g = *reinterpret_cast<const float4*>(dy + i);
    float4 r;
    r.x = BWD ? g.x * dgelu_exact(a.x) : gelu_f(a.x); r.y = BWD ? g.y * dgelu_exact(a.y) : gelu_f(a.y);
    r.z = BWD ? g.z * dgelu_exact(a.z) : gelu_f(a.z); r.w = BWD ? g.w * dgelu_exact(a.w) : gelu_f(a.w);
    *reinterpret_cast<float4*>(out + i) = r;
  } else {
    for (int64_t k = i; k < n; ++k) out[k] = BWD ? dy[k] * dgelu_exact(x[k]) : gelu_f(x[k]);
  }
}

extern "C" int ss_gelu(const void* x, const void* dy, void* out, int64_t numel, int dtype, hipStream_t stream) {
  if (numel < 0 || (dtype != SS_F32 && dtype != SS_BF16)) return SS_ERR_ARG;
  if (numel == 0) return SS_OK;
  if (!x || !out || (((uintptr_t)x | (uintptr_t)out | (uintptr_t)dy) & 15)) return SS_ERR_ARG;
  const int per = dtype == SS_BF16 ? 8 : 4;
  dim3 g((unsigned)ss_div_up(ss_div_up(numel, per), 256)), b(256);
  if (dtype == SS_BF16) {
    if (dy) SS_LAUNCH((k_gelu_bf16<true>), g, b, 0, stream, (const unsigned short*)x, (const unsigned short*)dy, (unsigned short*)out, numel);
    else SS_LAUNCH((k_gelu_bf16<false>), g, b, 0, stream, (const unsigned short*)x, (const unsigned short*)nullptr, (unsigned short*)out, numel);
  } else {
    if (dy) SS_LAUNCH((k_gelu_f32<true>), g, b, 0, stream, (const float*)x, (const float*)dy, (float*)out, numel);
    else SS_LAUNCH((k_gelu_f32<false>), g, b, 0, stream, (const float*)x, (const float*)nullptr, (float*)out, numel);
  }
  return SS_OK;
}
```

scenesplat_amd/functional.py:

```python
import os
import weakref

import torch
from torch.utils.weak import WeakIdKeyDictionary

from . import native as nv


class _WindowAttention(torch.autograd.Function):
    @staticmethod
    def forward(ctx, qkv, win, num_heads, scale, impl):
        qkv = qkv.contiguous()
        out, lse = nv.window_attn_fwd(qkv, win, num_heads, scale, impl)
        ctx.save_for_backward(qkv, out, lse)
        ctx.win, ctx.num_heads, ctx.scale, ctx.impl = win, num_heads, scale, impl
        return out

    @staticmethod
    def backward(ctx, dout):
        qkv, out, lse = ctx.saved_tensors
        dqkv = nv.window_attn_bwd(qkv, out, dout.contiguous().to(qkv.dtype), lse, ctx.win, ctx.num_heads, ctx.scale, ctx.impl)
        return dqkv, None, None, None, None


def window_attention(qkv, win, num_heads, scale, impl=nv.ATTN_SIMT):
    return _WindowAttention.apply(qkv, win, num_heads, scale, impl)


class _WindowAttentionRPE(torch.autograd.Function):
    @staticmethod
    def forward(ctx, qkv, table, win, grid_coord, pos_bnd, num_heads, scale, impl):
        qkv = qkv.contiguous()
        tab = table.detach().float().contiguous()
        out, lse = nv.window_attn_rpe_fwd(qkv, win, grid_coord, tab, pos_bnd, num_heads, scale, impl)
        ctx.save_for_backward(qkv, out, lse, tab)
        ctx.win, ctx.grid_coord, ctx.pos_bnd, ctx.num_heads, ctx.scale, ctx.impl = win, grid_coord, pos_bnd, num_heads, scale, impl
        ctx.table_dtype = table.dtype
        return out

    @staticmethod
    def backward(ctx, dout):
        qkv, out, lse, tab = ctx.saved_tensors
        dqkv, dtable = nv.window_attn_rpe_bwd(qkv, out, dout.contiguous().to(qkv.dtype), lse, ctx.win, ctx.grid_coord, tab,
                                              ctx.pos_bnd, ctx.num_heads, ctx.scale, ctx.impl)
        return dqkv, dtable.to(ctx.table_dtype), None, None, None, None, None, None


def window_attention_rpe(qkv, win, grid_coord, table, pos_bnd, num_heads, scale, impl=nv.ATTN_SIMT):
    return _WindowAttentionRPE.apply(qkv, table, win, grid_coord, pos_bnd, num_heads, scale, impl)


class _SegmentMean(torch.autograd.Function):
    @staticmethod
    def forward(ctx, src, level, mean):
        src = src.contiguous()
        ctx.level, ctx.mean = level, mean
        return nv.segment_reduce(src, level.indices, level.idx_ptr, level.n, mean)

    @staticmethod
    def backward(ctx, dout):
        lv = ctx.level
        return nv.segment_bcast(dout.contiguous(), lv.cluster, lv.idx_ptr, ctx.mean), None, None


class _SegmentMinMax(torch.autograd.Function):
    @staticmethod
    def forward(ctx, src, level, is_max):
        src = src.contiguous()
        out, arg = nv.segment_minmax(src, level.indices, level.idx_ptr, level.n, is_max)
        ctx.save_for_backward(arg)
        ctx.n_src = src.shape[0]
        return out

    @staticmethod
    def backward(ctx, dout):
        (arg,) = ctx.saved_tensors
        return nv.segment_minmax_bwd(dout.contiguous(), arg, ctx.n_src), None, None


def segment_minmax(src, level, is_max):
    return _SegmentMinMax.apply(src, level, is_max)


def segment_mean(src, level, mean=True):
    return _SegmentMean.apply(src, level, mean)


class _UnpoolAdd(torch.autograd.Function):
    @staticmethod
    def forward(ctx, skip, up, level):
        ctx.level = level
        return nv.gather_add_rows(skip.contiguous(), up.contiguous(), level.cluster)

    @staticmethod
    def backward(ctx, g):
        lv = ctx.level
        g = g.contiguous()
        return g, nv.segment_reduce(g, lv.indices, lv.idx_ptr, lv.n, False), None


def unpool_add(skip, up, level):
    return _UnpoolAdd.apply(skip, up, level)


class _SubMConv3d(torch.autograd.Function):

    @staticmethod
    def forward(ctx, feat, weight, bias, nbr, has_dup, compute_dtype):
        taps, n = nbr.shape
        cout = weight.shape[0]
        x = feat.to(compute_dtype).contiguous()
        w = weight.reshape(cout, taps, -1).to(compute_dtype)
        out = torch.zeros((n, cout), dtype=compute_dtype, device=feat.device) if bias is None else \
            bias.to(compute_dtype).unsqueeze(0).repeat(n, 1)
        buf = torch.empty_like(x)
        for t in range(taps):
            nv.gather_rows(x, nbr[t], out=buf)
            out.addmm_(buf, w[:, t, :].t())
        ctx.save_for_backward(x, weight, nbr)
        ctx.has_bias, ctx.has_dup, ctx.compute_dtype, ctx.in_dtype = bias is not None, has_dup, compute_dtype, feat.dtype
        return out

    @staticmethod
    def backward(ctx, dout):
        x, weight, nbr = ctx.saved_tensors
        taps, n = nbr.shape
        cout = weight.shape[0]
        cd = ctx.compute_dtype
        g = dout.to(cd).contiguous()
        w = weight.reshape(cout, taps, -1).to(cd)
        dx = dw = db = None
        if ctx.needs_input_grad[0]:
            dx = torch.zeros_like(x)
            if not ctx.has_dup:
                buf = torch.empty_like(g)
                for t in range(taps):
                    nv.gather_rows(g, nbr[t], out=buf)
                    dx.addmm_(buf, w[:, taps - 1 - t, :])
            else:
                for t in range(taps):
                    rows = torch.nonzero(nbr[t] >= 0, as_tuple=True)[0]
                    if rows.numel():
                        dx.index_add_(0, nbr[t][rows].long(), g[rows] @ w[:, t, :])
            dx = dx.to(ctx.in_dtype)
        if ctx.needs_input_grad[1]:
            dw = torch.empty((taps, cout, x.shape[1]), dtype=cd, device=x.device)
            buf = torch.empty_like(x)
            gt = g.t()
            for t in range(taps):
                nv.gather_rows(x, nbr[t], out=buf)
                torch.mm(gt, buf, out=dw[t])
            dw = dw.permute(1, 0, 2).reshape(weight.shape).to(weight.dtype)
        if ctx.has_bias and ctx.needs_input_grad[2]:
            db = g.sum(0).to(weight.dtype)
        return dx, dw, db, None, None, None, None


class _SubMConv3dFused(torch.autograd.Function):

    @staticmethod
    def forward(ctx, feat, weight, bias, nbr, rowperm, blocks_fn, has_dup, walk_fn=None, dup_fn=None):
        taps, n = nbr.shape
        cout, cin = weight.shape[0], weight.shape[-1]
        pad = (-cin) % 8
        ctx.dup_fn = dup_fn
        x = feat.to(torch.bfloat16)
        w = bf16_of(weight).reshape(cout, taps, cin)
        if pad:
            x = torch.nn.functional.pad(x, (0, pad)); w = torch.nn.functional.pad(w, (0, pad))
        x, w = x.contiguous(), w.contiguous()
        ctx.meta = (feat.dtype, weight.dtype, weight.shape, cin, bias is not None)
        ctx.blocks_fn, ctx.has_dup = blocks_fn, has_dup
        ctx.wt = mirrored_of(weight) if not pad else None
        ctx.im2col = n <= CONV_IM2COL_MAX_SITES
        out_dtype = torch.bfloat16 if torch.is_autocast_enabled() else torch.float32
        if ctx.im2col:
            cols = nv.subm_im2col(x, nbr)
            out = torch.nn.functional.linear(cols, w.view(cout, -1), bf16_of(bias))
            ctx.save_for_backward(cols, w, nbr, rowperm)
            return out.to(out_dtype)
        walk = None
        if CONV_WALK_RULEBOOK and walk_fn is not None and rowperm is not None and nv.subm_conv_fwd_uses_pipe(n, cin + pad, cout, taps):
            walk = walk_fn()
        ctx.has_walk = walk is not None
        out = nv.subm_conv_fwd(x, w, None if bias is None else bias.float().contiguous(), nbr, rowperm, out_dtype, nbr_walk=walk)
        ctx.save_for_backward(x, w, nbr, rowperm, *(() if walk is None else (walk,)))
        return out

    @staticmethod
    def backward(ctx, dout):
        x, w, nbr, rowperm = ctx.saved_tensors[:4]
        walk = ctx.saved_tensors[4] if getattr(ctx, "has_walk", False) else None
        in_dtype, w_dtype, w_shape, cin, has_bias = ctx.meta
        g = dout.to(torch.bfloat16).contiguous()
        dx = dw = db = None
        runs = gd = None
        if ctx.has_dup and ctx.needs_input_grad[0]:
            runs = ctx.dup_fn() if ctx.dup_fn is not None else nv.dup_runs_from_rulebook(nbr)
            gd = nv.dup_fold_rows(g, runs)
        if ctx.im2col:
            cols = x
            taps = nbr.shape[0]
            if ctx.needs_input_grad[0]:
                wt = ctx.wt if ctx.wt is not None else nv.subm_weight_mirror(w)
                dx = torch.nn.functional.linear(nv.subm_im2col(g if gd is None else gd, nbr), wt.view(wt.shape[0], -1))
                if runs is not None:
                    nv.dup_zero_rows_(dx, runs)
                dx = dx[:, :cin].to(in_dtype)
            if ctx.needs_input_grad[1]:
                dw = _mm_f32(g.t(), cols).view(w.shape)[:, :, :cin].reshape(w_shape).to(w_dtype)
            if has_bias and ctx.needs_input_grad[2]:
                db = g.sum(0, dtype=torch.float32).to(w_dtype)
            return dx, dw, db, None, None, None, None, None, None
        if ctx.needs_input_grad[0]:
            wt = ctx.wt if ctx.wt is not None else nv.subm_weight_mirror(w)
            dx = nv.subm_conv_fwd(g if gd is None else gd, wt, None, nbr, rowperm, nbr_walk=walk)
            if runs is not None:
                nv.dup_zero_rows_(dx, runs)
            dx = dx[:, :cin].to(in_dtype)
        if ctx.needs_input_grad[1]:
            blocks = ctx.blocks_fn() if ctx.blocks_fn is not None else nv.subm_block_lists(nbr, rowperm)
            dw = nv.subm_conv_wgrad(x, g, nbr, rowperm, blocks, nbr_walk=walk)[:, :, :cin].reshape(w_shape).to(w_dtype)
        if has_bias and ctx.needs_input_grad[2]:
            db = g.sum(0, dtype=torch.float32).to(w_dtype)
        return dx, dw, db, None, None, None, None, None, None


def _split_bf16(t):
    t = t.float()
    hi = t.to(torch.bfloat16)
    return hi, (t - hi.float()).to(torch.bfloat16)


class _SubMConv3dSplit(torch.autograd.Function):

    @staticmethod
    def forward(ctx, feat, weight, bias, nbr, rowperm, blocks_fn, has_dup=False, dup_fn=None):
        taps, n = nbr.shape
        cout, cin = weight.shape[0], weight.shape[-1]
        pad = (-cin) % 8
        ctx.has_dup, ctx.dup_fn = has_dup, dup_fn
        x = feat.float()
        w = weight.float().reshape(cout, taps, cin)
        if pad:
            x = torch.nn.functional.pad(x, (0, pad)); w = torch.nn.functional.pad(w, (0, pad))
        xh, xl = _split_bf16(x)
        wh, wl = _split_bf16(w)
        x3 = torch.cat([xh, xl, xh], 1).contiguous()
        w3 = torch.cat([wh, wh, wl], 2).contiguous()
        out = nv.subm_conv_fwd(x3, w3, None if bias is None else bias.float().contiguous(), nbr, rowperm, torch.float32)
        ctx.save_for_backward(xh, xl, wh, wl, nbr, rowperm)
        ctx.meta = (feat.dtype, weight.dtype, weight.shape, cin, bias is not None)
        ctx.blocks_fn = blocks_fn
        return out

    @staticmethod
    def backward(ctx, dout):
        xh, xl, wh, wl, nbr, rowperm = ctx.saved_tensors
        in_dtype, w_dtype, w_shape, cin, has_bias = ctx.meta
        gh, gl = _split_bf16(dout.contiguous())
        dx = dw = db = None
        if ctx.needs_input_grad[0]:
            wt3 = torch.cat([nv.subm_weight_mirror(wh), nv.subm_weight_mirror(wh), nv.subm_weight_mirror(wl)], 2).contiguous()
            runs = None
            fh, fl = gh, gl
            if ctx.has_dup:
                runs = ctx.dup_fn() if ctx.dup_fn is not None else nv.dup_runs_from_rulebook(nbr)
                fh, fl = _split_bf16(nv.dup_fold_rows(dout.float().contiguous(), runs))
            g3 = torch.cat([fh, fl, fh], 1).contiguous()
            dx = nv.subm_conv_fwd(g3, wt3, None, nbr, rowperm, torch.float32)
            if runs is not None:
                nv.dup_zero_rows_(dx, runs)
            dx = dx[:, :cin].to(in_dtype)
        if ctx.needs_input_grad[1]:
            blocks = ctx.blocks_fn() if ctx.blocks_fn is not None else nv.subm_block_lists(nbr, rowperm)
            cp = xh.shape[1]
            d2 = nv.subm_conv_wgrad(torch.cat([xh, xl], 1).contiguous(), gh, nbr, rowperm, blocks)
            d1 = nv.subm_conv_wgrad(xh, gl, nbr, rowperm, blocks)
            dw = (d2[:, :, :cp] + d2[:, :, cp:] + d1)[:, :, :cin].reshape(w_shape).to(w_dtype)
        if has_bias and ctx.needs_input_grad[2]:
            db = dout.sum(0, dtype=torch.float32).to(w_dtype)
        return dx, dw, db, None, None, None, None, None


class _SubMConv3dF32(torch.autograd.Function):

    @staticmethod
    def forward(ctx, feat, weight, bias, nbr, rowperm, blocks_fn, walk_fn, has_dup=False, dup_fn=None):
        taps, n = nbr.shape
        cout, cin = weight.shape[0], weight.shape[-1]
        cp = 16 if cin <= 16 else 32
        ctx.has_dup, ctx.dup_fn, ctx.plain_nbr = has_dup, dup_fn, nbr
        ctx.orig_nbr = nbr if blocks_fn is None else None
        nbr = walk_fn() if walk_fn is not None else nv.subm_walk_rulebook(nbr, rowperm)
        x = feat.float()
        if cp != cin:
            x = torch.nn.functional.pad(x, (0, cp - cin))
        x = x.contiguous()
        w = weight.float().reshape(cout, taps, cin)
        out = nv.subm_f32_fwd(x, nv.subm_f32_weight_layout(w), None if bias is None else bias.float().contiguous(), nbr, rowperm)
        ctx.save_for_backward(x, w, nbr, rowperm)
        ctx.meta = (feat.dtype, weight.dtype, weight.shape, cin, bias is not None)
        ctx.blocks_fn = blocks_fn
        return out

    @staticmethod
    def backward(ctx, dout):
        x, w, nbr, rowperm = ctx.saved_tensors
        in_dtype, w_dtype, w_shape, cin, has_bias = ctx.meta
        g = dout.float().contiguous()
        dx = dw = db = None
        if ctx.needs_input_grad[0]:
            if ctx.has_dup:
                runs = ctx.dup_fn() if ctx.dup_fn is not None else nv.dup_runs_from_rulebook(ctx.plain_nbr)
                dx = nv.subm_f32_fwd(nv.dup_fold_rows(g, runs), nv.subm_f32_weight_layout(w, mirror=True), None, nbr, rowperm,
                                     winners_only=True).to(in_dtype)
            else:
                dx = nv.subm_f32_fwd(g, nv.subm_f32_weight_layout(w, mirror=True), None, nbr, rowperm).to(in_dtype)
        if ctx.needs_input_grad[1]:
            blocks = ctx.blocks_fn() if ctx.blocks_fn is not None else nv.subm_block_lists(ctx.orig_nbr, rowperm)
            dw = nv.subm_f32_wgrad(x, g, nbr, rowperm, blocks, cin).reshape(w_shape).to(w_dtype)
        if has_bias and ctx.needs_input_grad[2]:
            db = g.sum(0, dtype=torch.float32).to(w_dtype)
        return dx, dw, db, None, None, None, None, None, None


CONV_WALK_RULEBOOK = os.environ.get("SS_CONV_WALK", "1") != "0"
CONV_F32_MFMA = os.environ.get("SS_CONV_F32_MFMA", "1") != "0"
CONV_IM2COL_MAX_SITES = int(os.environ.get("SS_CONV_IM2COL_MAX", "8192"))


def _mm_f32(a, b):
    try:
        return torch.mm(a, b, out_dtype=torch.float32)
    except (RuntimeError, NotImplementedError, TypeError):
        return torch.mm(a, b).float()


def subm_conv3d(feat, weight, bias, nbr, has_dup=False, compute_dtype=torch.float32, rowperm=None, blocks_fn=None, walk_fn=None,
                dup_fn=None):
    if compute_dtype == torch.bfloat16 and weight.shape[0] % 8 == 0:
        return _SubMConv3dFused.apply(feat, weight, bias, nbr, rowperm, blocks_fn, has_dup, walk_fn, dup_fn)
    if compute_dtype == "bf16x3":
        if (CONV_F32_MFMA and weight.shape[0] == 32 and weight.shape[-1] <= 32 and feat.is_cuda
                and (weight.shape[-1] == 32 or not feat.requires_grad)):
            return _SubMConv3dF32.apply(feat, weight, bias, nbr, rowperm, blocks_fn, walk_fn, has_dup, dup_fn)
        if weight.shape[0] % 8 == 0 and feat.is_cuda:
            return _SubMConv3dSplit.apply(feat, weight, bias, nbr, rowperm, blocks_fn, has_dup, dup_fn)
        compute_dtype = torch.float32
    return _SubMConv3d.apply(feat, weight, bias, nbr, has_dup, compute_dtype)


class _Gelu(torch.autograd.Function):

    @staticmethod
    def forward(ctx, x):
        x = x.contiguous()
        ctx.save_for_backward(x)
        return nv.gelu(x)

    @staticmethod
    def backward(ctx, dy):
        (x,) = ctx.saved_tensors
        dy = dy.contiguous().to(x.dtype)
        if not _aligned16(dy):
            dy = dy.clone()
        return nv.gelu(x, dy)


GELU_HIP = os.environ.get("SS_GELU_HIP", "1") != "0"


def _aligned16(t):
    return t.data_ptr() % 16 == 0 and t.storage_offset() * t.element_size() % 16 == 0


def gelu(x):
    if GELU_HIP and x.is_cuda and x.dtype in (torch.float32, torch.bfloat16) and _aligned16(x):
        return _Gelu.apply(x)
    return torch.nn.functional.gelu(x)


def lang_head_release():
    _HEAD_CACHE.clear()


class _LangHead(torch.autograd.Function):

    @staticmethod
    def forward(ctx, feat, target, mask, normalize, want_p):
        feat = feat.contiguous()
        if target is not None:
            target = target.contiguous()
            if target.dtype not in (torch.float32, torch.bfloat16):
                target = target.float()
        p, sums, rowstat = nv.lang_head_fwd(feat, target, mask, normalize, want_p=want_p)
        ctx.save_for_backward(feat, target, mask, rowstat)
        ctx.normalize = normalize
        ctx.set_materialize_grads(False)
        return p, sums

    @staticmethod
    def backward(ctx, dp, dsums):
        feat, target, mask, rowstat = ctx.saved_tensors
        if dp is None and (dsums is None or target is None):
            return None, None, None, None, None
        coef = None
        if target is not None:
            coef = (dsums[:2] if dsums is not None else torch.zeros(2, device=feat.device)).float().contiguous()
        dp = dp.contiguous() if dp is not None else None
        return nv.lang_head_bwd(feat, target, mask, ctx.normalize, rowstat, coef, dp), None, None, None, None


_HEAD_CACHE = {}


def lang_head(feat, target=None, mask=None, normalize=True):
    p, sums = _LangHead.apply(feat, target, mask, normalize, True)
    if target is not None:
        _HEAD_CACHE["last"] = (weakref.ref(p), weakref.ref(target), weakref.ref(mask), target._version, mask._version, sums)
    return p, sums


def lang_head_sums(pred, target, mask):
    ent = _HEAD_CACHE.get("last")
    if ent is not None and ent[0]() is pred and ent[1]() is target and ent[2]() is mask and ent[3] == target._version \
            and ent[4] == mask._version:
        return ent[5]
    _, sums = _LangHead.apply(pred, target, mask, False, False)
    _HEAD_CACHE["last"] = (weakref.ref(pred), weakref.ref(target), weakref.ref(mask), target._version, mask._version, sums)
    return sums


_SHADOW = WeakIdKeyDictionary()
_SHADOW_T = WeakIdKeyDictionary()
_SHADOW_M = WeakIdKeyDictionary()


def _stamp(p):
    return (p._version, p.data_ptr())


def _shadow_current(ent, p):
    tag = ent[1]
    if tag is None:
        return False
    if tag[0] == "capture":
        return tag[1] != 0 and torch.cuda.is_current_stream_capturing() and tag[1] == nv.stream_capture_id()
    return tag == _stamp(p)


def register_shadows(params):
    src, dst = [], []
    for p in params:
        if p is None or p.dtype != torch.float32 or not p.is_cuda:
            continue
        ent = _SHADOW.get(p)
        if ent is None or ent[0].shape != p.shape or ent[0].device != p.device:
            ent = [torch.empty_like(p, dtype=torch.bfloat16), None]
            _SHADOW[p] = ent
        src.append(p); dst.append(ent[0])
    return src, dst


SHADOW_GROUP_CAST = os.environ.get("SS_SHADOW_GROUP_CAST", "1") != "0"


@torch.no_grad()
def refresh_shadows(src, dst):
    todo_s, todo_d = [], []
    everything = torch.cuda.is_current_stream_capturing()
    cap = ("capture", nv.stream_capture_id()) if everything else None
    for p, d in zip(src, dst):
        ent = _SHADOW.get(p)
        st = _stamp(p)
        if everything or ent is None or ent[0] is not d or ent[1] != st:
            todo_s.append(p); todo_d.append(d)
            if ent is not None and ent[0] is d:
                ent[1] = cap if everything else st
    if todo_s:
        fast = [(s_, d_) for s_, d_ in zip(todo_s, todo_d) if s_.is_cuda and s_.dtype == torch.float32 and d_.dtype == torch.bfloat16
                and s_.is_contiguous() and d_.is_contiguous() and s_.numel() == d_.numel()
                and s_.data_ptr() % 16 == 0 and d_.data_ptr() % 16 == 0]
        if SHADOW_GROUP_CAST and fast:
            nv.cast_bf16_group([a for a, _ in fast], [b for _, b in fast])
            if len(fast) != len(todo_s):
                done = {id(d_) for _, d_ in fast}
                rest = [(s_, d_) for s_, d_ in zip(todo_s, todo_d) if id(d_) not in done]
                torch._foreach_copy_([d_ for _, d_ in rest], [s_ for s_, _ in rest])
        else:
            torch._foreach_copy_(todo_d, todo_s)
        pairs = [(d, _SHADOW_T[p]) for p, d in zip(todo_s, todo_d) if p in _SHADOW_T]
        if pairs:
            nv.transpose16_group(pairs)
        pairs = [(d.view(d.shape[0], -1, d.shape[-1]), _SHADOW_M[p]) for p, d in zip(todo_s, todo_d) if p in _SHADOW_M]
        if pairs:
            nv.subm_weight_mirror_group(pairs)


def register_mirrored(weights):
    for p in weights:
        ent = _SHADOW.get(p)
        if ent is None or p.dim() != 5 or p.shape[-1] % 8:
            continue
        cout, cin = p.shape[0], p.shape[-1]
        taps = p.numel() // (cout * cin)
        m = _SHADOW_M.get(p)
        if m is None or m.shape != (cin, taps, cout) or m.device != p.device:
            _SHADOW_M[p] = torch.empty((cin, taps, cout), dtype=torch.bfloat16, device=p.device)
            ent[1] = None


def mirrored_of(p):
    if not isinstance(p, torch.nn.Parameter):
        return None
    m = _SHADOW_M.get(p)
    if m is None:
        return None
    ent = _SHADOW.get(p)
    return m if (ent is not None and _shadow_current(ent, p)) else None


def register_transposed(weights):
    for p in weights:
        ent = _SHADOW.get(p)
        if ent is None or p.dim() != 2:
            continue
        t = _SHADOW_T.get(p)
        if t is None or t.shape != (p.shape[1], p.shape[0]) or t.device != p.device:
            _SHADOW_T[p] = torch.empty((p.shape[1], p.shape[0]), dtype=torch.bfloat16, device=p.device)
            ent[1] = None


def bf16_t_of(p):
    if not isinstance(p, torch.nn.Parameter):
        return None
    t = _SHADOW_T.get(p)
    if t is None:
        return None
    ent = _SHADOW.get(p)
    return t if (ent is not None and _shadow_current(ent, p)) else None


def bf16_of(p):
    if p is None:
        return None
    if p.dtype == torch.bfloat16:
        return p
    ent = _SHADOW.get(p) if isinstance(p, torch.nn.Parameter) else None
    if ent is not None and _shadow_current(ent, p):
        return ent[0]
    return p.to(torch.bfloat16)


WGRAD_GROUP_MAX_ROWS = int(os.environ.get("SS_WGRAD_GROUP_MAX", str(1 << 22)))
_STAGE = {"cur": None, "route": {}}
_UNFLUSHED = set()


WGRAD_GROUP_MAX_BYTES = int(float(os.environ.get("SS_WGRAD_GROUP_MAX_GIB", "8")) * (1 << 30))


class _WgradStage:
    def __init__(self):
        self.queue = []
        self.redq = []
        self.bytes = 0

    def add(self, x, dy, dw, db):
        self.queue.append((x, dy, dw, db))
        self.bytes += x.numel() * x.element_size() + dy.numel() * dy.element_size()
        if self.bytes > WGRAD_GROUP_MAX_BYTES:
            q, self.queue, self.bytes = self.queue, [], 0
            nv.linear_wgrad_group(q)

    def flush(self):
        _UNFLUSHED.discard(self)
        q, self.queue, self.bytes = self.queue, [], 0
        r, self.redq = self.redq, []
        nv.linear_wgrad_group(q)
        nv.group_partial_sums(r)


class _StageParams(torch.autograd.Function):
    @staticmethod
    def forward(ctx, stage, *params):
        ctx.stage = stage
        ctx.set_materialize_grads(False)
        return tuple(p.view_as(p) for p in params)

    @staticmethod
    def backward(ctx, *grads):
        ctx.stage.flush()
        return (None,) + grads


def stage_begin(linears, n_rows):
    _STAGE["cur"], _STAGE["route"] = None, {}
    if not (WGRAD_GROUP_MAX_ROWS and LINEAR_WGRAD_MIN_ROWS <= n_rows <= WGRAD_GROUP_MAX_ROWS and torch.is_grad_enabled()
            and torch.is_autocast_enabled() and torch.get_autocast_dtype("cuda") == torch.bfloat16):
        return
    params = [p for m in linears for p in (m.weight, m.bias) if p is not None and p.requires_grad and p.dtype == torch.float32 and p.is_cuda]
    if not params:
        return
    stage = _WgradStage()
    aliases = _StageParams.apply(stage, *params)
    _STAGE["cur"], _STAGE["route"] = stage, {id(p): a for p, a in zip(params, aliases)}


def stage_end():
    _STAGE["cur"], _STAGE["route"] = None, {}


def reset_state():
    stage_end()
    _UNFLUSHED.clear()
    _HEAD_CACHE.clear()


def _routed(p):
    a = _STAGE["route"].get(id(p)) if (p is not None and _STAGE["route"]) else None
    return (a, _STAGE["cur"]) if a is not None else (p, None)


class _Linear(torch.autograd.Function):

    @staticmethod
    def forward(ctx, x, weight, bias, w16, b16, stage, w16t=None):
        y = torch.nn.functional.linear(x, w16, b16)
        ctx.save_for_backward(x, w16 if w16t is None else w16t)
        ctx.meta = (weight.dtype, bias is not None)
        ctx.dgrad_nt = w16t is not None
        ctx.stage = stage
        return y

    @staticmethod
    def backward(ctx, dy):
        x, w16 = ctx.saved_tensors
        w_dtype, has_bias = ctx.meta
        dx, dw, db = _linear_backward(x, w16, ctx.dgrad_nt, w_dtype, has_bias, ctx.stage, dy.contiguous(), ctx.needs_input_grad[0],
                                      ctx.needs_input_grad[1], ctx.needs_input_grad[2])
        return dx, dw, db, None, None, None, None


class _LinearGelu(torch.autograd.Function):

    @staticmethod
    def forward(ctx, x, weight, bias, w16, b16, stage, w16t=None):
        u = torch.nn.functional.linear(x, w16, b16)
        ctx.save_for_backward(x, w16 if w16t is None else w16t, u)
        ctx.meta = (weight.dtype, bias is not None)
        ctx.dgrad_nt = w16t is not None
        ctx.stage = stage
        return nv.gelu(u)

    @staticmethod
    def backward(ctx, dy):
        x, w16, u = ctx.saved_tensors
        w_dtype, has_bias = ctx.meta
        dy = dy.contiguous()
        if not _aligned16(dy):
            dy = dy.clone()
        du = nv.gelu(u, dy)
        dx, dw, db = _linear_backward(x, w16, ctx.dgrad_nt, w_dtype, has_bias, ctx.stage, du, ctx.needs_input_grad[0],
                                      ctx.needs_input_grad[1], ctx.needs_input_grad[2])
        return dx, dw, db, None, None, None, None


def _linear_backward(x, w16, dgrad_nt, w_dtype, has_bias, stage, dy, need_x, need_w, need_b):
    dx = dw = db = None
    if need_x:
        dx = torch.nn.functional.linear(dy, w16) if dgrad_nt else dy @ w16
    want_db = has_bias and need_b
    if need_w:
        m, k = x.shape
        if m >= LINEAR_WGRAD_MIN_ROWS and nv.lib().ss_wgrad8_ok(m, k, dy.shape[1], 1):
            if stage is not None and w_dtype == torch.float32:
                dw, db_ = nv.linear_wgrad_alloc(k, dy.shape[1], want_db, x.device)
                stage.add(x, dy, dw, db_)
                if want_db:
                    db, want_db = db_, False
            elif want_db:
                dw, db = nv.linear_wgrad(x, dy, True)
                dw, db = dw.to(w_dtype), db.to(w_dtype)
                want_db = False
            else:
                dw = nv.linear_wgrad(x, dy).to(w_dtype)
        else:
            dw = _mm_f32(dy.t(), x).to(w_dtype)
    if want_db:
        db = dy.sum(0, dtype=torch.float32).to(w_dtype)
    return dx, dw, db


LINEAR_WGRAD_MIN_ROWS = 1024


def linear(x, weight, bias=None):
    if x.is_cuda and x.dim() == 2 and torch.is_autocast_enabled() and torch.get_autocast_dtype("cuda") == torch.bfloat16 \
            and weight.dtype == torch.float32:
        route = _STAGE["route"]
        wr = route.get(id(weight)) if route else None
        if wr is not None and torch.is_grad_enabled():
            br = route.get(id(bias)) if bias is not None else None
            return _Linear.apply(x.to(torch.bfloat16).contiguous(), wr, br if br is not None else bias, bf16_of(weight), bf16_of(bias),
                                 _STAGE["cur"], bf16_t_of(weight))
        return _Linear.apply(x.to(torch.bfloat16).contiguous(), weight, bias, bf16_of(weight), bf16_of(bias), None, bf16_t_of(weight))
    return torch.nn.functional.linear(x, weight, bias)


def linear_gelu(x, weight, bias=None):
    if GELU_HIP and x.is_cuda and x.dim() == 2 and torch.is_autocast_enabled() and torch.get_autocast_dtype("cuda") == torch.bfloat16 \
            and weight.dtype == torch.float32 and torch.is_grad_enabled():
        route = _STAGE["route"]
        wr = route.get(id(weight)) if route else None
        if wr is not None:
            br = route.get(id(bias)) if bias is not None else None
            return _LinearGelu.apply(x.to(torch.bfloat16).contiguous(), wr, br if br is not None else bias, bf16_of(weight), bf16_of(bias),
                                     _STAGE["cur"], bf16_t_of(weight))
        return _LinearGelu.apply(x.to(torch.bfloat16).contiguous(), weight, bias, bf16_of(weight), bf16_of(bias), None, bf16_t_of(weight))
    return gelu(linear(x, weight, bias))


class _QkvWindowAttentionHM(torch.autograd.Function):

    @staticmethod
    def forward(ctx, x, weight, bias, w16, stage, w16t, win, num_heads, scale):
        sec0 = float(scale) * nv.LOG2E
        b32 = bias.detach() if bias is not None else None
        if nv.headmajor_eligible(x.shape[1]) and x.shape[0] >= HM_FUSED_MIN_ROWS and x.shape[1] >= HM_FUSED_MIN_CHANNELS:
            hm = nv.linear_fwd_headmajor(x, win, w16, b32.float() if b32 is not None else None, num_heads, sec0)
        else:
            qkv = _mm_f32(x, w16.t())
            if b32 is not None:
                qkv = qkv + b32.float()
            hm = nv.headmajor_pack(qkv.contiguous(), win, num_heads, 3, sec0)
        out, nlse2 = nv.window_attn_hm_fwd(hm, win, num_heads)
        ctx.save_for_backward(x, w16 if w16t is None else w16t, hm, out, nlse2)
        ctx.meta = (weight.dtype, bias is not None)
        ctx.dgrad_nt = w16t is not None
        ctx.stage, ctx.win, ctx.num_heads, ctx.scale = stage, win, num_heads, scale
        return out

    @staticmethod
    def backward(ctx, dout):
        x, w16, hm, out, nlse2 = ctx.saved_tensors
        w_dtype, has_bias = ctx.meta
        dqkv = nv.window_attn_hm_bwd(hm, out, dout.contiguous().to(torch.bfloat16), nlse2, ctx.win, ctx.num_heads, ctx.scale)
        dx, dw, db = _linear_backward(x, w16, ctx.dgrad_nt, w_dtype, has_bias, ctx.stage, dqkv, ctx.needs_input_grad[0],
                                      ctx.needs_input_grad[1], ctx.needs_input_grad[2])
        return dx, dw, db, None, None, None, None, None, None


HM_FUSED_MIN_ROWS = int(os.environ.get("SS_HM_FUSED_MIN_ROWS", "1024"))
HM_FUSED_MIN_CHANNELS = int(os.environ.get("SS_HM_FUSED_MIN_CHANNELS", "64"))


def qkv_window_attention(x, weight, bias, win, num_heads, scale):
    route = _STAGE["route"]
    wr = route.get(id(weight)) if (route and torch.is_grad_enabled()) else None
    br = route.get(id(bias)) if (wr is not None and bias is not None) else None
    stage = _STAGE["cur"] if wr is not None else None
    return _QkvWindowAttentionHM.apply(x.to(torch.bfloat16).contiguous(), wr if wr is not None else weight,
                                       br if br is not None else bias, bf16_of(weight), stage, bf16_t_of(weight), win, num_heads,
                                       scale)


def window_attention_hm(qkv, win, num_heads, scale):
    return _WindowAttentionHM.apply(qkv, win, num_heads, scale)


class _WindowAttentionHM(torch.autograd.Function):
    @staticmethod
    def forward(ctx, qkv, win, num_heads, scale):
        hm = nv.headmajor_pack(qkv.contiguous(), win, num_heads, 3, float(scale) * nv.LOG2E)
        out, nlse2 = nv.window_attn_hm_fwd(hm, win, num_heads)
        ctx.save_for_backward(hm, out, nlse2)
        ctx.win, ctx.num_heads, ctx.scale, ctx.in_dtype = win, num_heads, scale, qkv.dtype
        return out

    @staticmethod
    def backward(ctx, dout):
        hm, out, nlse2 = ctx.saved_tensors
        dqkv = nv.window_attn_hm_bwd(hm, out, dout.contiguous().to(torch.bfloat16), nlse2, ctx.win, ctx.num_heads, ctx.scale)
        return dqkv.to(ctx.in_dtype), None, None, None


class _LayerNorm(torch.autograd.Function):

    @staticmethod
    def forward(ctx, x, gamma, beta, eps, out_dtype):
        x = x.contiguous()
        _, _, h, mean, rstd = nv.add_layernorm_fwd(x, None, None, gamma.float().contiguous(), beta.float().contiguous(), eps,
                                                   False, False, out_dtype)
        ctx.save_for_backward(x, mean, rstd, gamma)
        return h

    @staticmethod
    def backward(ctx, g_h):
        x, mean, rstd, gamma = ctx.saved_tensors
        g_x, _, dg, db = nv.add_layernorm_bwd(None, None, g_h.contiguous(), x, mean, rstd, gamma.float().contiguous(), None,
                                              x.dtype, None)
        return g_x, dg.to(gamma.dtype), db.to(gamma.dtype), None, None


def layer_norm(x, gamma, beta, eps=1e-5, out_dtype=None):
    return _LayerNorm.apply(x, gamma, beta, eps, out_dtype or x.dtype)


class _AddLayerNorm(torch.autograd.Function):

    @staticmethod
    def forward(ctx, x, y, rowscale, gamma, beta, eps, want_copy, h_dtype, stage):
        x, y = x.contiguous(), y.contiguous()
        g32 = gamma.float().contiguous() if gamma is not None else None
        b32 = beta.float().contiguous() if beta is not None else None
        xout, xcopy, h, mean, rstd = nv.add_layernorm_fwd(x, y, rowscale, g32, b32, eps, True, want_copy, h_dtype)
        ctx.save_for_backward(xout, mean, rstd, g32, rowscale)
        ctx.meta = (x.dtype, y.dtype, gamma.dtype if gamma is not None else None)
        ctx.stage = stage
        ctx.set_materialize_grads(False)
        return xout, h, xcopy

    @staticmethod
    def backward(ctx, g_xout, g_h, g_xcopy):
        xout, mean, rstd, g32, rowscale = ctx.saved_tensors
        x_dt, y_dt, g_dt = ctx.meta
        g_xout = g_xout.contiguous() if g_xout is not None else None
        g_h = g_h.contiguous() if g_h is not None else None
        g_xcopy = g_xcopy.contiguous() if g_xcopy is not None else None
        if g_xout is None and g_h is None and g_xcopy is None:
            return (None,) * 9
        if ctx.stage is not None and g_dt == torch.float32:
            g_x, g_y, part, _ = nv.add_layernorm_bwd(g_xout, g_xcopy, g_h, xout, mean, rstd, g32, rowscale, x_dt, y_dt, reduce=False)
            dg = db = None
            if part is not None:
                dst = torch.empty((2, part.shape[2]), dtype=torch.float32, device=part.device)
                ctx.stage.redq.append((part, dst))
                _UNFLUSHED.add(ctx.stage)
                dg, db = dst[0], dst[1]
            return g_x, g_y, None, dg, db, None, None, None, None
        g_x, g_y, dg, db = nv.add_layernorm_bwd(g_xout, g_xcopy, g_h, xout, mean, rstd, g32, rowscale, x_dt, y_dt)
        return (g_x, g_y, None, dg.to(g_dt) if dg is not None else None, db.to(g_dt) if db is not None else None,
                None, None, None, None)


class _LnAddLn(torch.autograd.Function):

    @staticmethod
    def forward(ctx, x, t, g0, b0, eps0, g1, b1, eps1, h_dtype, stage):
        x, t = x.contiguous(), t.contiguous()
        p32 = [p.float().contiguous() for p in (g0, b0, g1, b1)]
        xout, h, stats = nv.ln_add_ln_fwd(x, t, p32[0], p32[1], eps0, p32[2], p32[3], eps1, h_dtype)
        ctx.save_for_backward(xout, t, stats, p32[0], p32[2])
        ctx.meta = (x.dtype, t.dtype, g0.dtype)
        ctx.stage = stage
        ctx.set_materialize_grads(False)
        return xout, h

    @staticmethod
    def backward(ctx, g_xout, g_h):
        xout, t, stats, g0, g1 = ctx.saved_tensors
        x_dt, t_dt, p_dt = ctx.meta
        if g_xout is None and g_h is None:
            return (None,) * 10
        g_xout = g_xout.float().contiguous() if g_xout is not None else None
        g_h = g_h.contiguous() if g_h is not None else None
        if ctx.stage is not None and p_dt == torch.float32:
            g_x, g_t, part = nv.ln_add_ln_bwd(g_xout, g_h, xout, t, stats, g0, g1, x_dt, t_dt, reduce=False)
            dst = torch.empty((4, part.shape[2]), dtype=torch.float32, device=part.device)
            ctx.stage.redq.append((part, dst))
            _UNFLUSHED.add(ctx.stage)
            return g_x, g_t, dst[0], dst[1], None, dst[2], dst[3], None, None, None
        g_x, g_t, dg0, db0, dg1, db1 = nv.ln_add_ln_bwd(g_xout, g_h, xout, t, stats, g0, g1, x_dt, t_dt)
        return g_x, g_t, dg0.to(p_dt), db0.to(p_dt), None, dg1.to(p_dt), db1.to(p_dt), None, None, None


def _eff_stage(*ts):
    cur = _STAGE["cur"]
    return cur if cur is not None and all(getattr(t, "pdnorm_eff", False) for t in ts) else None


def ln_add_ln(x, t, ln0, ln1, h_dtype=torch.float32):
    (g0, s0), (b0, s1), (g1, s2), (b1, s3) = _routed(ln0.weight), _routed(ln0.bias), _routed(ln1.weight), _routed(ln1.bias)
    stage = s0 if (s0 is not None and s0 is s1 and s0 is s2 and s0 is s3) else None
    if stage is None:
        g0, b0, g1, b1 = ln0.weight, ln0.bias, ln1.weight, ln1.bias
        stage = _eff_stage(g0, b0, g1, b1)
    return _LnAddLn.apply(x, t, g0, b0, ln0.eps, g1, b1, ln1.eps, h_dtype, stage)


def add_layer_norm(x, y, rowscale=None, gamma=None, beta=None, eps=1e-5, want_copy=False, h_dtype=torch.float32):
    (ga, s0), (be, s1) = _routed(gamma), _routed(beta)
    stage = s0 if (s0 is not None and s0 is s1) else None
    if stage is None:
        ga, be = gamma, beta
        stage = _eff_stage(ga, be) if ga is not None else None
    return _AddLayerNorm.apply(x, y, rowscale, ga, be, eps, want_copy, h_dtype, stage)


class _BatchNormAct(torch.autograd.Function):

    @staticmethod
    def forward(ctx, x, gamma, beta, running_mean, running_var, num_batches, training, momentum, eps, act):
        x = x.contiguous()
        n = x.shape[0]
        if training and running_mean.dtype == torch.float32 and running_var.dtype == torch.float32 and momentum is not None:
            with torch.no_grad():
                mean, rstd = nv.bn_batch_stats(x, running_mean, running_var, num_batches, momentum, eps)
        else:
            if training:
                shift, s, q = nv.col_stats(x)
                d = s / n
                mean = shift + d
                var = (q / n - d * d).clamp_(min=0.0)
                with torch.no_grad():
                    mom = momentum if momentum is not None else 1.0 / float(num_batches.item() + 1 if num_batches is not None else 1)
                    running_mean.mul_(1 - mom).add_(mean.to(running_mean.dtype), alpha=mom)
                    running_var.mul_(1 - mom).add_((var * (n / max(n - 1, 1))).to(running_var.dtype), alpha=mom)
                    if num_batches is not None:
                        num_batches.add_(1)
            else:
                mean, var = running_mean.float(), running_var.float()
            rstd = torch.rsqrt(var + eps).contiguous()
            mean = mean.contiguous()
        g32, b32 = gamma.float().contiguous(), beta.float().contiguous()
        y = nv.bn_act_fwd(x, mean, rstd, g32, b32, act, x.dtype)
        ctx.save_for_backward(x, mean, rstd, g32, b32)
        ctx.meta = (training, act, gamma.dtype)
        return y

    @staticmethod
    def backward(ctx, dy):
        x, mean, rstd, g32, b32 = ctx.saved_tensors
        training, act, pdt = ctx.meta
        dx, dg, db = nv.bn_act_bwd(dy.contiguous(), x, mean, rstd, g32, b32, act, training)
        return dx, dg.to(pdt), db.to(pdt), None, None, None, None, None, None, None


def batch_norm_act(x, bn, act=False):
    return _BatchNormAct.apply(x, bn.weight, bn.bias, bn.running_mean, bn.running_var, bn.num_batches_tracked if bn.training else None,
                               bn.training, bn.momentum, bn.eps, act)


class PDNormGroup:

    def __init__(self, rows, split_row=0):
        self.rows = [tuple(r) for r in rows]
        self.split_row = int(split_row)
        self.tab = None

    def table(self, context_channels):
        if self.tab is None or self.tab.cc != context_channels or not self.tab.current(self.rows):
            self.tab = nv.PDNormTable(self.rows, context_channels)
        return self.tab


class _PDNormModulation(torch.autograd.Function):

    @staticmethod
    def forward(ctx, group, context, *params):
        c32 = context.detach().float().contiguous()
        tab = group.table(c32.numel())
        ctx.split_row = group.split_row
        geff, beff, ops = nv.pdnorm_mod_fwd(c32, tab)
        ctx.save_for_backward(c32, ops, *[p for p in params if p is not None])
        ctx.tab, ctx.context_meta = tab, (context.shape, context.dtype)
        ctx.set_materialize_grads(False)
        return tuple(geff) + tuple(beff)

    @staticmethod
    def backward(ctx, *grads):
        c32, ops = ctx.saved_tensors[:2]
        n = len(grads) // 2
        if all(g is None for g in grads):
            return (None,) * (2 + 4 * n)
        for st in list(_UNFLUSHED):
            st.flush()
        grads = [g.float().contiguous() if g is not None else None for g in grads]
        dctx, dW, db, dg, dbt = nv.pdnorm_mod_bwd(c32, ctx.tab, ops, grads[:n], grads[n:], ctx.split_row)
        shape, dtype = ctx.context_meta
        out = [None, dctx.view(shape).to(dtype)]
        for l in range(n):
            out += [dW[l], db[l], dg[l], dbt[l]]
        return tuple(out)


def pdnorm_modulation(group, context):
    if not (torch.is_tensor(context) and context.is_cuda):
        raise RuntimeError("pdnorm_modulation: context must be a GPU tensor (no CPU fallback)")
    flat = [t for r in group.rows for t in r]
    outs = _PDNormModulation.apply(group, context, *flat)
    for o in outs:
        o.pdnorm_eff = True
    n = len(group.rows)
    return list(zip(outs[:n], outs[n:]))
```

scenesplat_amd/pointcept_api/ptv3.py:

```python
import os
from functools import partial

import torch
import torch.nn as nn
import torch.nn.functional as F

from .. import functional as SF
from .. import native as nv
from ..plan import build_plan
from .pdnorm import PDNorm, PointModule, ResolvedNorm, pdnorm_layers, resolved as _rn
from .registry import MODELS
from .structure import Point

RUNTIME = dict(attn_impl=nv.ATTN_SIMT, conv_dtype=None,
               attn_headmajor=os.environ.get("SS_ATTN_HM", "1") != "0",
               param_shadows=os.environ.get("SS_PARAM_SHADOWS", "1") != "0")


def bench_runtime():
    return dict(attn_impl=nv.ATTN_MFMA, conv_dtype=torch.bfloat16,
                conv_split_max_channels=int(os.environ.get("SS_CONV_SPLIT_MAX", "32")))


def conv_wants_walk(n_sites, channels, ksize):
    cin, cout = channels if isinstance(channels, (tuple, list)) else (channels, channels)
    cd = conv_dtype_for(cout)
    if cd == "bf16x3":
        return bool(SF.CONV_F32_MFMA and cout == 32 and cin <= 32)
    if cd == torch.bfloat16 and cout % 8 == 0:
        return bool(SF.CONV_WALK_RULEBOOK and n_sites > SF.CONV_IM2COL_MAX_SITES
                    and nv.subm_conv_fwd_uses_pipe(n_sites, cin + (-cin) % 8, cout, ksize ** 3))
    return False


def conv_dtype_for(out_channels):
    cd = RUNTIME["conv_dtype"] or torch.float32
    if cd == torch.bfloat16 and out_channels <= RUNTIME.get("conv_split_max_channels", 0):
        return "bf16x3"
    return cd


class DropPath(nn.Module):

    def __init__(self, p=0.0):
        super().__init__()
        self.p = float(p)

    def forward(self, x):
        if self.p == 0.0 or not self.training:
            return x
        keep = 1.0 - self.p
        mask = x.new_empty((x.shape[0], 1)).bernoulli_(keep)
        if keep > 0.0:
            mask.div_(keep)
        return x * mask


class SubMConv3d(nn.Module):

    def __init__(self, in_channels, out_channels, kernel_size, bias=True, indice_key=None):
        super().__init__()
        k = kernel_size
        self.kernel_size, self.indice_key = k, indice_key
        self.weight = nn.Parameter(torch.empty(out_channels, k, k, k, in_channels))
        self.bias = nn.Parameter(torch.zeros(out_channels)) if bias else None
        nn.init.kaiming_uniform_(self.weight.view(out_channels, -1), a=5 ** 0.5)

    def forward(self, feat, level):
        cd = conv_dtype_for(self.weight.shape[0])
        return SF.subm_conv3d(feat, self.weight, self.bias, level.neighbors(self.kernel_size),
                              level.has_duplicates, cd, level.conv_rowperm(),
                              lambda: level.conv_blocks(self.kernel_size), lambda: level.neighbors_walk(self.kernel_size),
                              level.dup_runs)


def _lin(mod, x):
    return SF.linear(x, mod.weight, mod.bias)


class RPE(nn.Module):

    def __init__(self, patch_size, num_heads):
        super().__init__()
        self.patch_size, self.num_heads = patch_size, num_heads
        self.pos_bnd = int((4 * patch_size) ** (1 / 3) * 2)
        self.rpe_num = 2 * self.pos_bnd + 1
        self.rpe_table = nn.Parameter(torch.zeros(3 * self.rpe_num, num_heads))
        nn.init.trunc_normal_(self.rpe_table, std=0.02)


class SerializedAttention(PointModule):
    def __init__(self, channels, num_heads, patch_size, qkv_bias=True, qk_scale=None, attn_drop=0.0,
                 proj_drop=0.0, order_index=0, enable_rpe=False, enable_flash=True, upcast_attention=True,
                 upcast_softmax=True):
        super().__init__()
        assert channels % num_heads == 0
        if enable_rpe and enable_flash:
            raise AssertionError("Set enable_rpe to False when enable Flash Attention")
        if attn_drop != 0.0 or proj_drop != 0.0:
            raise NotImplementedError("attention / projection dropout are 0 in the reference configs")
        self.channels, self.num_heads, self.patch_size = channels, num_heads, patch_size
        self.scale = qk_scale or (channels // num_heads) ** -0.5
        self.order_index = order_index
        self.enable_rpe = bool(enable_rpe)
        self.qkv = nn.Linear(channels, channels * 3, bias=qkv_bias)
        self.proj = nn.Linear(channels, channels)
        self.rpe = RPE(patch_size, num_heads) if enable_rpe else None

    def rpe_window_size(self, level):
        k = min(min(level.counts), self.patch_size)
        if k < 1:
            raise ValueError("enable_rpe: every batch element needs at least one point")
        return k

    def _forward_rpe(self, x, level):
        win = level.window(self.order_index, self.rpe_window_size(level))
        qkv = _lin(self.qkv, x)
        bf16 = (x.is_cuda and torch.is_autocast_enabled() and torch.get_autocast_dtype("cuda") == torch.bfloat16) \
            or qkv.dtype == torch.bfloat16
        if bf16 and (self.channels // self.num_heads) in (16, 32, 48, 64):
            impl = nv.ATTN_MFMA
        else:
            impl = nv.ATTN_SIMT
        a = qkv.to(torch.bfloat16) if bf16 else qkv
        feat = SF.window_attention_rpe(a, win, level.grid_coord, self.rpe.rpe_table, self.rpe.pos_bnd, self.num_heads,
                                       self.scale, impl).to(qkv.dtype)
        return _lin(self.proj, feat)

    def forward(self, x, level):
        if self.enable_rpe:
            return self._forward_rpe(x, level)
        win = level.window(self.order_index, self.patch_size)
        impl = RUNTIME["attn_impl"]
        if (impl == nv.ATTN_MFMA and RUNTIME.get("attn_headmajor", True) and x.is_cuda and torch.is_autocast_enabled()
                and torch.get_autocast_dtype("cuda") == torch.bfloat16 and self.qkv.weight.dtype == torch.float32
                and (self.channels // self.num_heads) in (16, 32, 48, 64)):
            feat = SF.qkv_window_attention(x, self.qkv.weight, self.qkv.bias, win, self.num_heads, self.scale)
            return _lin(self.proj, feat)
        qkv = _lin(self.qkv, x)
        if impl == nv.ATTN_MFMA and qkv.dtype != torch.bfloat16:
            feat = SF.window_attention(qkv.to(torch.bfloat16), win, self.num_heads, self.scale, impl).to(qkv.dtype)
        else:
            feat = SF.window_attention(qkv, win, self.num_heads, self.scale, impl)
        return _lin(self.proj, feat)


class MLP(nn.Module):
    def __init__(self, in_channels, hidden_channels=None, out_channels=None, act_layer=nn.GELU, drop=0.0):
        super().__init__()
        out_channels = out_channels or in_channels
        hidden_channels = hidden_channels or in_channels
        self.fc1 = nn.Linear(in_channels, hidden_channels)
        self.act = act_layer()
        self.fc2 = nn.Linear(hidden_channels, out_channels)

    def forward(self, x):
        if type(self.act) is nn.GELU and getattr(self.act, "approximate", "none") == "none":
            h = SF.linear_gelu(x, self.fc1.weight, self.fc1.bias)
        else:
            h = self.act(_lin(self.fc1, x))
        return _lin(self.fc2, h)


class Block(PointModule):
    def __init__(self, channels, num_heads, patch_size=48, mlp_ratio=4.0, qkv_bias=True, qk_scale=None,
                 attn_drop=0.0, proj_drop=0.0, drop_path=0.0, norm_layer=nn.LayerNorm, act_layer=nn.GELU,
                 pre_norm=True, order_index=0, cpe_indice_key=None, enable_rpe=False, enable_flash=True,
                 upcast_attention=True, upcast_softmax=True):
        super().__init__()
        self.channels, self.pre_norm = channels, pre_norm
        self.cpe = nn.Sequential(SubMConv3d(channels, channels, 3, bias=True, indice_key=cpe_indice_key),
                                 nn.Linear(channels, channels), norm_layer(channels))
        self.norm1 = nn.Sequential(norm_layer(channels))
        self.attn = SerializedAttention(channels, num_heads, patch_size, qkv_bias, qk_scale, attn_drop, proj_drop,
                                        order_index, enable_rpe, enable_flash, upcast_attention, upcast_softmax)
        self.norm2 = nn.Sequential(norm_layer(channels))
        self.mlp = nn.Sequential(MLP(channels, int(channels * mlp_ratio), channels, act_layer, proj_drop))
        self.drop_path = nn.Sequential(DropPath(drop_path) if drop_path > 0.0 else nn.Identity())

    def forward(self, x, conv_in, level, want_copy=False):
        if not self.pre_norm:
            return self._forward_post_norm(x, conv_in, level), None
        hdt = torch.bfloat16 if torch.is_autocast_enabled() else torch.float32
        ln0, ln1, ln2 = _rn(self.cpe[2]), _rn(self.norm1[0]), _rn(self.norm2[0])
        t = _lin(self.cpe[1], self.cpe[0](conv_in, level))
        if RUNTIME.get("fuse_ln_seam", True) and x.shape[1] % 4 == 0 and x.shape[1] <= 1024:
            x, h = SF.ln_add_ln(x, t, ln0, ln1, hdt)
        else:
            t = SF.layer_norm(t, ln0.weight, ln0.bias, ln0.eps)
            x, h, _ = SF.add_layer_norm(x, t, None, ln1.weight, ln1.bias, ln1.eps, False, hdt)
        x, h, _ = SF.add_layer_norm(x, self.attn(h, level), self._row_scale(x), ln2.weight, ln2.bias, ln2.eps, False, hdt)
        x, _, xb = SF.add_layer_norm(x, self.mlp(h), self._row_scale(x), None, None, 0.0, want_copy, hdt)
        return x, xb

    def _row_scale(self, x):
        dp = self.drop_path[0]
        if not isinstance(dp, DropPath) or dp.p == 0.0 or not self.training:
            return None
        pre = self.__dict__.get("_row_scales")
        if pre:
            rs = pre.pop()
            if rs.shape[0] == x.shape[0]:
                return rs
        keep = 1.0 - dp.p
        return x.new_empty(x.shape[0], dtype=torch.float32).bernoulli_(keep).div_(keep)

    def _forward_post_norm(self, x, conv_in, level):
        c = self.cpe[0](conv_in, level)
        x = x + self.cpe[2](self.cpe[1](c))
        x = self.norm1(x + self.drop_path(self.attn(x, level)))
        return self.norm2(x + self.drop_path(self.mlp(x)))


def _norm_act(x, norm, act):
    norm = _rn(norm)
    if (isinstance(norm, nn.BatchNorm1d) or getattr(norm, "is_bn", False)) and norm.affine and norm.track_running_stats \
            and (act is None or isinstance(act, nn.GELU)) \
            and x.shape[1] % 4 == 0 and x.shape[1] <= 1024:
        return SF.batch_norm_act(x, norm, act is not None)
    if norm is not None:
        x = norm(x)
    return act(x) if act is not None else x


def _seq_lin_norm_act(seq, x):
    mods = [_rn(m) for m in seq]
    x = _lin(mods[0], x) if isinstance(mods[0], nn.Linear) else mods[0](x)
    norm = mods[1] if len(mods) > 1 and (isinstance(mods[1], nn.BatchNorm1d) or getattr(mods[1], "is_bn", False)) else None
    act = mods[-1] if len(mods) > 1 and isinstance(mods[-1], nn.GELU) else None
    if norm is None and act is None:
        for mod in mods[1:]:
            x = mod(x)
        return x
    return _norm_act(x, norm, act)


class SerializedPooling(PointModule):
    def __init__(self, in_channels, out_channels, stride=2, norm_layer=None, act_layer=None, reduce="mean",
                 shuffle_orders=True, traceable=True):
        super().__init__()
        if reduce not in ("mean", "sum", "min", "max"):
            raise ValueError(f"unknown reduce {reduce!r} (torch_scatter.segment_csr: sum / mean / min / max)")
        self.reduce = reduce
        self.in_channels, self.out_channels, self.stride = in_channels, out_channels, stride
        self.shuffle_orders = shuffle_orders
        self.proj = nn.Linear(in_channels, out_channels)
        self.norm = nn.Sequential(norm_layer(out_channels)) if norm_layer is not None else None
        self.act = act_layer() if act_layer is not None else None

    def forward(self, x, coarse_level):
        if self.reduce in ("min", "max"):
            x = SF.segment_minmax(_lin(self.proj, x), coarse_level, self.reduce == "max")
        else:
            x = SF.segment_mean(_lin(self.proj, x), coarse_level, mean=(self.reduce == "mean"))
        return _norm_act(x, self.norm[0] if self.norm is not None else None, self.act)


class SerializedUnpooling(PointModule):
    def __init__(self, in_channels, skip_channels, out_channels, norm_layer=None, act_layer=None, traceable=False):
        super().__init__()
        self.proj = nn.Sequential(nn.Linear(in_channels, out_channels))
        self.proj_skip = nn.Sequential(nn.Linear(skip_channels, out_channels))
        if norm_layer is not None:
            self.proj.append(norm_layer(out_channels)); self.proj_skip.append(norm_layer(out_channels))
        if act_layer is not None:
            self.proj.append(act_layer()); self.proj_skip.append(act_layer())

    def forward(self, x, skip, coarse_level):
        skip, up = _seq_lin_norm_act(self.proj_skip, skip), _seq_lin_norm_act(self.proj, x)
        return SF.unpool_add(skip, up, coarse_level), skip


class _Stem(nn.Module):
    pass


class Embedding(PointModule):
    def __init__(self, in_channels, embed_channels, norm_layer=None, act_layer=None):
        super().__init__()
        self.in_channels, self.embed_channels = in_channels, embed_channels
        self.stem = _Stem()
        self.stem.conv = SubMConv3d(in_channels, embed_channels, 5, bias=False, indice_key="stem")
        if norm_layer is not None:
            self.stem.norm = norm_layer(embed_channels)
        if act_layer is not None:
            self.stem.act = act_layer()

    def forward(self, feat, level):
        x = self.stem.conv(feat, level)
        return _norm_act(x, getattr(self.stem, "norm", None), getattr(self.stem, "act", None))


class _Stage(nn.Module):
    pass


def backward_in_two(outputs, grad_outputs, cut, between=None):
    torch.autograd.backward(outputs, grad_tensors=grad_outputs)
    if between is not None:
        between()
    backward_tail(cut)


def backward_tail(cut):
    pairs = [(o, l.grad) for o, l in cut if l.grad is not None]
    if pairs:
        torch.autograd.backward([o for o, _ in pairs], grad_tensors=[g for _, g in pairs])
    for _, l in cut:
        l.grad = None


@MODELS.register_module("PT-v3m1")
class PointTransformerV3(PointModule):
    def __init__(self, in_channels=6, order=("z", "z-trans"), stride=(2, 2, 2, 2), enc_depths=(2, 2, 2, 6, 2),
                 enc_channels=(32, 64, 128, 256, 512), enc_num_head=(2, 4, 8, 16, 32),
                 enc_patch_size=(48, 48, 48, 48, 48), dec_depths=(2, 2, 2, 2), dec_channels=(64, 64, 128, 256),
                 dec_num_head=(4, 4, 8, 16), dec_patch_size=(48, 48, 48, 48), mlp_ratio=4, qkv_bias=True,
                 qk_scale=None, attn_drop=0.0, proj_drop=0.0, drop_path=0.3, pre_norm=True, shuffle_orders=True,
                 enable_rpe=False, enable_flash=True, upcast_attention=False, upcast_softmax=False, cls_mode=False,
                 pdnorm_bn=False, pdnorm_ln=False, pdnorm_decouple=True, pdnorm_adaptive=False, pdnorm_affine=True,
                 pdnorm_conditions=("ScanNet", "S3DIS", "Structured3D")):
        super().__init__()
        if (pdnorm_bn or pdnorm_ln) and not pdnorm_decouple:
            raise ValueError("pdnorm_decouple=False cannot run in the reference (PDNorm keeps the un-called norm_layer factory and calls "
                             "it on the features): refused instead of inventing semantics")
        self.num_stages = len(enc_depths)
        self.order = [order] if isinstance(order, str) else list(order)
        self.cls_mode, self.shuffle_orders = cls_mode, shuffle_orders
        self.stride = tuple(stride)
        assert self.num_stages == len(stride) + 1 == len(enc_channels) == len(enc_num_head) == len(enc_patch_size)
        assert cls_mode or self.num_stages == len(dec_depths) + 1 == len(dec_channels) + 1
        assert cls_mode or self.num_stages == len(dec_num_head) + 1 == len(dec_patch_size) + 1

        pdn = dict(conditions=pdnorm_conditions, decouple=pdnorm_decouple, adaptive=pdnorm_adaptive)
        if pdnorm_bn:
            bn_layer = partial(PDNorm, norm_layer=partial(nn.BatchNorm1d, eps=1e-3, momentum=0.01, affine=pdnorm_affine), **pdn)
        else:
            bn_layer = partial(nn.BatchNorm1d, eps=1e-3, momentum=0.01)
        if pdnorm_ln:
            ln_layer = partial(PDNorm, norm_layer=partial(nn.LayerNorm, elementwise_affine=pdnorm_affine), **pdn)
        else:
            ln_layer = nn.LayerNorm
        act_layer = nn.GELU
        self.enc_channels = tuple(enc_channels)
        self.dec_channels_ = tuple(dec_channels) if not cls_mode else ()
        self.embedding = Embedding(in_channels, enc_channels[0], bn_layer, act_layer)
        blk = dict(mlp_ratio=mlp_ratio, qkv_bias=qkv_bias, qk_scale=qk_scale, attn_drop=attn_drop, proj_drop=proj_drop,
                   norm_layer=ln_layer, act_layer=act_layer, pre_norm=pre_norm, enable_rpe=enable_rpe,
                   enable_flash=enable_flash, upcast_attention=upcast_attention, upcast_softmax=upcast_softmax)
        enc_dp = [x.item() for x in torch.linspace(0, drop_path, sum(enc_depths))]
        self.enc = _Stage()
        for s in range(self.num_stages):
            dp = enc_dp[sum(enc_depths[:s]):sum(enc_depths[:s + 1])]
            enc = _Stage()
            if s > 0:
                enc.down = SerializedPooling(enc_channels[s - 1], enc_channels[s], stride[s - 1], bn_layer, act_layer)
            for i in range(enc_depths[s]):
                setattr(enc, f"block{i}", Block(enc_channels[s], enc_num_head[s], enc_patch_size[s], drop_path=dp[i],
                                               order_index=i % len(self.order), cpe_indice_key=f"stage{s}", **blk))
            setattr(self.enc, f"enc{s}", enc)
        self.enc_depths, self.dec_depths = tuple(enc_depths), tuple(dec_depths)
        if not cls_mode:
            dec_dp = [x.item() for x in torch.linspace(0, drop_path, sum(dec_depths))]
            self.dec = _Stage()
            dec_channels = list(dec_channels) + [enc_channels[-1]]
            for s in reversed(range(self.num_stages - 1)):
                dp = dec_dp[sum(dec_depths[:s]):sum(dec_depths[:s + 1])]
                dp.reverse()
                dec = _Stage()
                dec.up = SerializedUnpooling(dec_channels[s + 1], enc_channels[s], dec_channels[s], bn_layer, act_layer)
                for i in range(dec_depths[s]):
                    setattr(dec, f"block{i}", Block(dec_channels[s], dec_num_head[s], dec_patch_size[s], drop_path=dp[i],
                                                   order_index=i % len(self.order), cpe_indice_key=f"stage{s}", **blk))
                setattr(self.dec, f"dec{s}", dec)

    def draw_perms(self):
        K = len(self.order)
        perms = [torch.randperm(K).tolist() if self.shuffle_orders else list(range(K))]
        for s in range(1, self.num_stages):
            down = getattr(self.enc, f"enc{s}").down
            perms.append(torch.randperm(K).tolist() if down.shuffle_orders else list(range(K)))
        return perms

    def plan_specs(self):
        K = len(self.order)
        wide = list(self.enc_channels)
        if not self.cls_mode:
            for s, c in enumerate(self.dec_channels_):
                wide[s] = max(wide[s], c)
        walk = [[c for c in {self.enc_channels[s], wide[s]}] for s in range(self.num_stages)]
        wins, ks = [], [(0, 5, [(self.embedding.in_channels, self.enc_channels[0])])]
        for s in range(self.num_stages):
            enc = getattr(self.enc, f"enc{s}")
            ks.append((s, 3, walk[s]))
            for i in range(self.enc_depths[s]):
                attn = getattr(enc, f"block{i}").attn
                if not attn.enable_rpe:
                    wins.append((s, i % K, attn.patch_size))
        if not self.cls_mode:
            for s in range(self.num_stages - 1):
                dec = getattr(self.dec, f"dec{s}")
                for i in range(self.dec_depths[s]):
                    attn = getattr(dec, f"block{i}").attn
                    if not attn.enable_rpe:
                        wins.append((s, i % K, attn.patch_size))
        return wins, ks

    def prepare_plan(self, data_dict, perms=None, stream=None):
        if "grid_coord" not in data_dict:
            raise KeyError("prepare_plan needs grid_coord")
        perms = perms if perms is not None else self.draw_perms()
        if stream is None:
            plan = build_plan(data_dict["grid_coord"], data_dict["offset"], self.order, self.stride, perms)
            plan.materialize(*self.plan_specs())
            return plan
        with torch.cuda.stream(stream):
            plan = build_plan(data_dict["grid_coord"], data_dict["offset"], self.order, self.stride, perms)
            plan.materialize(*self.plan_specs())
            plan.ready_event = torch.cuda.Event()
            plan.ready_event.record(stream)
        return plan

    def _stage_linears(self, stage):
        cache = self.__dict__.setdefault("_stage_linear_cache", {})
        ls = cache.get(id(stage))
        if ls is None:
            skip = self._modulation_linears()
            ls = [m for m in stage.modules() if isinstance(m, (nn.Linear, nn.LayerNorm)) and id(m) not in skip]
            cache[id(stage)] = ls
        return ls

    def _refresh_shadows(self):
        ps = self.__dict__.get("_shadow_lists")
        if ps is None or ps[2] != next(self.parameters()).device:
            params, skip = [], self._modulation_linears()
            for m in self.modules():
                if isinstance(m, nn.Linear) and id(m) not in skip:
                    params += [m.weight, m.bias]
                elif isinstance(m, SubMConv3d):
                    params += [m.weight, m.bias]
            src, dst = SF.register_shadows(params)
            wide = []
            for st in [getattr(self.enc, f"enc{s}", None) for s in (0, 1)] + [getattr(getattr(self, "dec", None), f"dec{s}", None) for s in (0, 1)]:
                if st is not None:
                    wide += [m.weight for m in st.modules() if isinstance(m, nn.Linear) and m.weight.numel() >= 65536]
            if RUNTIME.get("dgrad_nt", True):
                SF.register_transposed(wide)
            SF.register_mirrored([m.weight for m in self.modules() if isinstance(m, SubMConv3d)
                                  and conv_dtype_for(m.weight.shape[0]) == torch.bfloat16])
            total = sum(((p.numel() + 3) & ~3) for p in params if p is not None) + 4 * len(params)
            ps = (src, dst, next(self.parameters()).device, total)
            self.__dict__["_shadow_lists"] = ps
        SF.refresh_shadows(ps[0], ps[1])
        if torch.is_grad_enabled():
            nv.zero_arena_begin(ps[3], ps[2])

    def _pdnorm(self):
        pds = self.__dict__.get("_pdnorm_list")
        if pds is None:
            pds = self.__dict__["_pdnorm_list"] = pdnorm_layers(self)
        return pds

    def _modulation_linears(self):
        return {id(m.modulation[1]) for m in self._pdnorm() if m.adaptive}

    def _resolve_pdnorm(self, point):
        pds = self._pdnorm()
        assert "condition" in point.keys(), f"feat and condition must be in point.keys(): {point.keys()}"
        idx = pds[0].index_of(point["condition"])
        if not pds[0].adaptive:
            for m in pds:
                m.__dict__["_resolved"] = m.resolve_static(idx)
            return
        assert "context" in point.keys()
        split = (not self.cls_mode and torch.is_grad_enabled() and point.get("backward_cut", None) is not None)
        cache = self.__dict__.setdefault("_pdnorm_groups", {})
        groups = cache.get((idx, split))
        if groups is None:
            last = {id(m) for m in pdnorm_layers(self.dec.dec0)} if not self.cls_mode else set()
            parts = [[m for m in pds if id(m) not in last], [m for m in pds if id(m) in last]]
            if not split:
                parts = [(parts[0] + parts[1], len(parts[0]))]
            else:
                parts = [(ms, 0) for ms in parts if ms]
            groups = cache[(idx, split)] = [(ms, SF.PDNormGroup([m.row(idx) for m in ms], sp)) for ms, sp in parts]
        for ms, group in groups:
            for m, (g, b) in zip(ms, SF.pdnorm_modulation(group, point["context"])):
                m.__dict__["_resolved"] = ResolvedNorm(g, b, m.norm[idx])

    def _draw_row_scales(self, levels, device):
        blocks = []
        for s in range(self.num_stages):
            enc = getattr(self.enc, f"enc{s}")
            blocks += [(getattr(enc, f"block{i}"), levels[s].n) for i in range(self.enc_depths[s])]
        if not self.cls_mode:
            for s in reversed(range(self.num_stages - 1)):
                dec = getattr(self.dec, f"dec{s}")
                blocks += [(getattr(dec, f"block{i}"), levels[s].n) for i in range(self.dec_depths[s])]
        segs = []
        for blk, n in blocks:
            dp = blk.drop_path[0]
            if isinstance(dp, DropPath) and dp.p > 0.0:
                segs += [(blk, n, 1.0 - dp.p)] * 2
            blk.__dict__["_row_scales"] = []
        if not segs:
            return
        key = tuple((n, k) for _, n, k in segs) + (str(device),)
        cache = self.__dict__.get("_keep_vec")
        if cache is None or cache[0] != key:
            kv = torch.cat([torch.full((n,), k, dtype=torch.float32) for _, n, k in segs]).pin_memory().to(device, non_blocking=True)
            cache = (key, kv)
            self.__dict__["_keep_vec"] = cache
        kv = cache[1]
        scales = nv.row_keep_scales(kv)
        off = 0
        for blk, n, _ in segs:
            blk.__dict__["_row_scales"].append(scales[off:off + n])
            off += n

    def forward(self, data_dict, perms=None):
        point = data_dict if isinstance(data_dict, Point) else Point(data_dict)
        feat = point["feat"]
        if not feat.is_cuda:
            raise RuntimeError("PT-v3m1 (scenesplat_amd) runs on the GPU only: the HIP path has no CPU fallback")
        if "grid_coord" not in point:
            if not {"grid_size", "coord"} <= set(point.keys()):
                raise KeyError("need grid_coord, or coord + grid_size (structure.py:54-62)")
            c = point["coord"]
            point["grid_coord"] = torch.div(c - c.min(0)[0], point["grid_size"], rounding_mode="trunc").int()
        if dict.__contains__(point, "offset"):
            offset = point["offset"]
        else:
            offset = point["offset"]
        self._want_copy = (RUNTIME["conv_dtype"] == torch.bfloat16)
        if (torch.is_autocast_enabled() or self._want_copy) and RUNTIME.get("param_shadows", True):
            self._refresh_shadows()
        plan = point.get("plan", None)
        if plan is None:
            plan = build_plan(point["grid_coord"], offset, self.order, self.stride,
                              perms if perms is not None else self.draw_perms())
        elif plan.ready_event is not None:
            torch.cuda.current_stream().wait_event(plan.ready_event)
            plan.record_stream(torch.cuda.current_stream())
            plan.ready_event = None
        levels = plan.levels
        if self.training:
            self._draw_row_scales(levels, feat.device)
        if self._pdnorm():
            self._resolve_pdnorm(point)
            try:
                return self._forward_levels(point, feat, plan)
            finally:
                for m in self._pdnorm():
                    m.__dict__.pop("_resolved", None)
        return self._forward_levels(point, feat, plan)

    def _forward_levels(self, point, feat, plan):
        levels = plan.levels
        x = self.embedding(feat, levels[0])
        skips = []
        for s in range(self.num_stages):
            enc = getattr(self.enc, f"enc{s}")
            SF.stage_begin(self._stage_linears(enc), levels[s].n)
            if s > 0:
                skips.append(x)
                x = enc.down(x, levels[s])
            xb = None
            for i in range(self.enc_depths[s]):
                wc = self._want_copy and conv_dtype_for(x.shape[1]) == torch.bfloat16
                x, xb = getattr(enc, f"block{i}")(x, x if xb is None else xb, levels[s], wc and i + 1 < self.enc_depths[s])
            SF.stage_end()
        lv = self.num_stages - 1
        if not self.cls_mode:
            cut = point.get("backward_cut", None) if torch.is_grad_enabled() else None
            for s in reversed(range(self.num_stages - 1)):
                dec = getattr(self.dec, f"dec{s}")
                if cut is not None and s == 0 and x.requires_grad:
                    leaves = (x.detach().requires_grad_(True), skips[0].detach().requires_grad_(True))
                    cut.extend([(x, leaves[0]), (skips[0], leaves[1])])
                    x, skips[0] = leaves
                SF.stage_begin(self._stage_linears(dec), levels[s].n)
                x, conv_in = dec.up(x, skips[s], levels[s + 1])
                xb = None
                for i in range(self.dec_depths[s]):
                    wc = self._want_copy and conv_dtype_for(x.shape[1]) == torch.bfloat16
                    x, xb = getattr(dec, f"block{i}")(x, conv_in if i == 0 else (x if xb is None else xb), levels[s],
                                                      wc and i + 1 < self.dec_depths[s])
                SF.stage_end()
            lv = 0
        out = Point(feat=x, plan=plan, level=lv)
        for k in ("coord", "grid_coord", "offset"):
            if lv == 0 and dict.__contains__(point, k):
                out[k] = point[k]
        return out
```

Before: 2.815 million.

## Fuse attention proj, residual LayerNorm and MLP into one block-tail kernel

Adds a fused HIP kernel pair that, per 32-row tile, runs the attention output projection, residual add with drop-path scale, LayerNorm, fc1, GELU, fc2 and the second residual in LDS using bf16 MFMA. The backward fuses the matching dgrad chain and the LayerNorm gamma/beta partial sums, and weight grads still come from separate linear backward calls. This removes several kernel launches and the global round trips of the intermediate activations between the proj, LN and MLP stages. In exchange the GEMMs run at small per-block tiles with recomputed weight reads from global memory, and transposed weight shadows must be registered for these layers.

```diff
diff --git a/include/scenesplat_hip.h b/include/scenesplat_hip.h
--- a/include/scenesplat_hip.h
+++ b/include/scenesplat_hip.h
@@ -168,6 +168,17 @@
                      const float* stats, const float* gamma0, const float* gamma1, void* g_x, int g_x_dtype, void* g_t,
                      int g_t_dtype, float* part, int64_t n, int channels, int nblocks, ss_stream_t stream);
 int ss_add_layernorm_bwd_blocks(int64_t n);
+
+int ss_block_tail_rows(void);
+int ss_block_tail_bwd_blocks(int64_t n);
+int ss_block_tail_fwd(const void* feat, const float* x, const float* rs1, const float* rs2, const void* wp, const void* bp,
+                      const void* w1, const void* b1, const void* w2, const void* b2, int bias_dtype, const float* gamma, const float* beta,
+                      float eps, float* x_mid, float* mean, float* rstd, void* h2, void* u, void* a, float* x_out,
+                      void* xcopy_bf16, int64_t n, int channels, ss_stream_t stream);
+int ss_block_tail_bwd(const float* g_xout, const void* g_xcopy_bf16, const float* x_mid, const float* mean, const float* rstd,
+                      const void* u, const float* rs1, const float* rs2, const float* gamma, const void* wp_t, const void* w1_t,
+                      const void* w2_t, float* g_mid, void* dfeat, void* dy2, void* du, void* dy1, float* part, int64_t n,
+                      int channels, int nblocks, ss_stream_t stream);
 int ss_group_partial_sums_outputs_per_workgroup(void);
 int ss_group_partial_sums(const int64_t* desc, const int32_t* wg_start, int nprob, int total_workgroups, ss_stream_t stream);
 int ss_transpose16_group(const int64_t* desc, const int32_t* wg_start, int nprob, int total_workgroups, ss_stream_t stream);
diff --git a/scenesplat_amd/_lib.py b/scenesplat_amd/_lib.py
--- a/scenesplat_amd/_lib.py
+++ b/scenesplat_amd/_lib.py
@@ -94,6 +94,10 @@
     "ss_subm_f32_wgrad": (c_i, [c_p, c_p, c_p, c_p, c_p, c_p, c_p, c_i64, c_i, c_i, c_i, c_i, c_p]),
     "ss_add_layernorm_fwd": (c_i, [c_p, c_i, c_p, c_i, c_p, c_p, c_p, c_f, c_p, c_i, c_p, c_p, c_i, c_p, c_p, c_i64, c_i, c_p]),
     "ss_add_layernorm_bwd_blocks": (c_i, [c_i64]),
+    "ss_block_tail_rows": (c_i, []),
+    "ss_block_tail_bwd_blocks": (c_i, [c_i64]),
+    "ss_block_tail_fwd": (c_i, [c_p] * 10 + [c_i, c_p, c_p, c_f] + [c_p] * 8 + [c_i64, c_i, c_p]),
+    "ss_block_tail_bwd": (c_i, [c_p] * 18 + [c_i64, c_i, c_i, c_p]),
     "ss_group_partial_sums_outputs_per_workgroup": (c_i, []),
     "ss_group_partial_sums": (c_i, [c_p, c_p, c_i, c_i, c_p]),
     "ss_transpose16_group": (c_i, [c_p, c_p, c_i, c_i, c_p]),
diff --git a/scenesplat_amd/csrc/block_tail.hip b/scenesplat_amd/csrc/block_tail.hip
--- /dev/null
+++ b/scenesplat_amd/csrc/block_tail.hip
@@ -0,0 +1,337 @@
+#include "common.h"
+#include "rowmath.h"
+#include "../../include/scenesplat_hip.h"
+
+#define BT_R 32
+#define BT_MAX_BWD_BLOCKS 1024
+#define BT_MFMA(a, b, c) __builtin_amdgcn_mfma_f32_16x16x32_bf16((a), (b), (c), 0, 0, 0)
+
+template <int C> struct BtCfg {
+  static constexpr int NW = C <= 64 ? 4 : (C == 128 ? 8 : 16);
+  static constexpr int THREADS = NW * 64;
+  static constexpr int LPR = C / 4;
+  static constexpr int RPP = THREADS / LPR;
+  static constexpr int PASSES = BT_R / RPP;
+  static constexpr int LDC = C + 8, LDH = 4 * C + 8;
+  static_assert(BT_R % RPP == 0 && PASSES >= 1, "row passes must tile the row block");
+};
+
+template <int N, int K, int NW>
+__device__ __forceinline__ void bt_gemm(const unsigned short* sIn, const unsigned short* __restrict__ W,
+                                        const void* __restrict__ bias, int bias_dt, unsigned short* sOut) {
+  constexpr int LDI = K + 8, LDO = N + 8, NT = N / 16;
+  constexpr int RG = NT >= NW ? 2 : 1;
+  constexpr int ITEMS = NT * (2 / RG);
+  constexpr int UNR = NW == 16 ? 4 : 8;
+  const int lane = threadIdx.x & 63, wave = threadIdx.x >> 6;
+  const int fr = lane & 15, fq = lane >> 4;
+  for (int it = wave; it < ITEMS; it += NW) {
+    const int ct = it % NT, rt0 = (it / NT) * RG;
+    f32x4_t acc[RG];
+#pragma unroll
+    for (int g = 0; g < RG; ++g) acc[g] = f32x4_t{0.f, 0.f, 0.f, 0.f};
+    if constexpr (K % 64 == 0) {
+      const unsigned short* wrow = W + (size_t)(ct * 16 + fr) * K + fq * 16;
+      const unsigned short* arow = sIn + (rt0 * 16 + fr) * LDI + fq * 16;
+#pragma unroll UNR / 2
+      for (int k0 = 0; k0 < K; k0 += 64) {
+        const bf16x8_t b0 = *reinterpret_cast<const bf16x8_t*>(wrow + k0);
+        const bf16x8_t b1 = *reinterpret_cast<const bf16x8_t*>(wrow + k0 + 8);
+#pragma unroll
+        for (int g = 0; g < RG; ++g) {
+          const bf16x8_t a0 = *reinterpret_cast<const bf16x8_t*>(arow + g * 16 * LDI + k0);
+          const bf16x8_t a1 = *reinterpret_cast<const bf16x8_t*>(arow + g * 16 * LDI + k0 + 8);
+          acc[g] = BT_MFMA(a0, b0, acc[g]);
+          acc[g] = BT_MFMA(a1, b1, acc[g]);
+        }
+      }
+    } else {
+      const unsigned short* wrow = W + (size_t)(ct * 16 + fr) * K + fq * 8;
+      const unsigned short* arow = sIn + (rt0 * 16 + fr) * LDI + fq * 8;
+#pragma unroll UNR
+      for (int k0 = 0; k0 < K; k0 += 32) {
+        const bf16x8_t b = *reinterpret_cast<const bf16x8_t*>(wrow + k0);
+#pragma unroll
+        for (int g = 0; g < RG; ++g) {
+          const bf16x8_t a = *reinterpret_cast<const bf16x8_t*>(arow + g * 16 * LDI + k0);
+          acc[g] = BT_MFMA(a, b, acc[g]);
+        }
+      }
+    }
+    const int col = ct * 16 + fr;
+    const float bv = !bias ? 0.f : (bias_dt == SS_F32 ? reinterpret_cast<const float*>(bias)[col]
+                                                     : bf16_to_f32(reinterpret_cast<const unsigned short*>(bias)[col]));
+#pragma unroll
+    for (int g = 0; g < RG; ++g)
+#pragma unroll
+      for (int i = 0; i < 4; ++i) sOut[((rt0 + g) * 16 + fq * 4 + i) * LDO + col] = f32_to_bf16(acc[g][i] + bv);
+  }
+}
+
+__device__ __forceinline__ float4 bt_lds_ld4(const unsigned short* p) {
+  const uint2 u = *reinterpret_cast<const uint2*>(p);
+  return make_float4(__uint_as_float(u.x << 16), __uint_as_float(u.x & 0xffff0000u), __uint_as_float(u.y << 16),
+                     __uint_as_float(u.y & 0xffff0000u));
+}
+__device__ __forceinline__ uint2 bt_pack4(const float4& v) {
+  uint2 u; u.x = pack_bf16x2(v.x, v.y); u.y = pack_bf16x2(v.z, v.w);
+  return u;
+}
+
+template <int W, int THREADS>
+__device__ __forceinline__ void bt_tile_load(const unsigned short* __restrict__ src, unsigned short* s, int rows) {
+  for (int i = threadIdx.x; i < BT_R * (W / 8); i += THREADS) {
+    const int r = i / (W / 8), c = (i % (W / 8)) * 8;
+    uint4 v = make_uint4(0u, 0u, 0u, 0u);
+    if (r < rows) v = *reinterpret_cast<const uint4*>(src + (int64_t)r * W + c);
+    *reinterpret_cast<uint4*>(s + r * (W + 8) + c) = v;
+  }
+}
+template <int W, int THREADS>
+__device__ __forceinline__ void bt_tile_store(const unsigned short* s, unsigned short* __restrict__ dst, int rows) {
+  for (int i = threadIdx.x; i < BT_R * (W / 8); i += THREADS) {
+    const int r = i / (W / 8), c = (i % (W / 8)) * 8;
+    if (r < rows) *reinterpret_cast<uint4*>(dst + (int64_t)r * W + c) = *reinterpret_cast<const uint4*>(s + r * (W + 8) + c);
+  }
+}
+
+template <int C>
+__global__ void __launch_bounds__(BtCfg<C>::THREADS)
+k_block_tail_fwd(const unsigned short* __restrict__ feat, const float* __restrict__ x, const float* __restrict__ rs1,
+                 const float* __restrict__ rs2, const unsigned short* __restrict__ Wp, const void* __restrict__ bp,
+                 const unsigned short* __restrict__ W1, const void* __restrict__ b1, const unsigned short* __restrict__ W2,
+                 const void* __restrict__ b2, int bias_dt, const float* __restrict__ gamma, const float* __restrict__ beta, float eps,
+                 float* __restrict__ x_mid, float* __restrict__ mean, float* __restrict__ rstd, unsigned short* __restrict__ h2,
+                 unsigned short* __restrict__ u, unsigned short* __restrict__ a, float* __restrict__ x_out,
+                 unsigned short* __restrict__ xcopy, int64_t n) {
+  using Cf = BtCfg<C>;
+  constexpr int H = 4 * C, LDC = Cf::LDC, LDH = Cf::LDH, T = Cf::THREADS;
+  __shared__ __attribute__((aligned(16))) unsigned short sA[BT_R * LDC];
+  __shared__ __attribute__((aligned(16))) unsigned short sB[BT_R * LDC];
+  __shared__ __attribute__((aligned(16))) unsigned short sH[BT_R * LDH];
+  const int64_t row0 = (int64_t)blockIdx.x * BT_R;
+  const int rows = (int)((n - row0) < BT_R ? (n - row0) : BT_R);
+  const int pr = threadIdx.x / Cf::LPR, pj = (threadIdx.x % Cf::LPR) * 4;
+
+  bt_tile_load<C, T>(feat + row0 * C, sA, rows);
+  __syncthreads();
+  bt_gemm<C, C, Cf::NW>(sA, Wp, bp, bias_dt, sB);
+  __syncthreads();
+
+  float4 xm[Cf::PASSES];
+  const float4 gm = *reinterpret_cast<const float4*>(gamma + pj), bt = *reinterpret_cast<const float4*>(beta + pj);
+#pragma unroll
+  for (int p = 0; p < Cf::PASSES; ++p) {
+    const int r = p * Cf::RPP + pr;
+    const bool valid = r < rows;
+    const int64_t g = (row0 + r) * C + pj;
+    float4 v = make_float4(0.f, 0.f, 0.f, 0.f);
+    if (valid) {
+      v = *reinterpret_cast<const float4*>(x + g);
+      const float s = rs1 ? rs1[row0 + r] : 1.f;
+      const float4 y = bt_lds_ld4(sB + r * LDC + pj);
+      v.x += s * y.x; v.y += s * y.y; v.z += s * y.z; v.w += s * y.w;
+      *reinterpret_cast<float4*>(x_mid + g) = v;
+    }
+    xm[p] = v;
+    const float mu = lanes_reduce_sum<Cf::LPR>(ln_sum4(v)) / C;
+    const float rr = rsqrtf(lanes_reduce_sum<Cf::LPR>(ln_sqdev4(v, mu)) / C + eps);
+    const uint2 hp = bt_pack4(ln_apply4(v, mu, rr, gm, bt));
+    *reinterpret_cast<uint2*>(sA + r * LDC + pj) = hp;
+    if (valid) {
+      *reinterpret_cast<uint2*>(h2 + g) = hp;
+      if (pj == 0) { mean[row0 + r] = mu; rstd[row0 + r] = rr; }
+    }
+  }
+  __syncthreads();
+  bt_gemm<H, C, Cf::NW>(sA, W1, b1, bias_dt, sH);
+  __syncthreads();
+
+  for (int i = threadIdx.x; i < BT_R * (H / 8); i += T) {
+    const int r = i / (H / 8), c = (i % (H / 8)) * 8;
+    const uint4 uv = *reinterpret_cast<const uint4*>(sH + r * LDH + c);
+    float f[8];
+    bf8_unpack(uv, f);
+#pragma unroll
+    for (int e = 0; e < 8; ++e) f[e] = gelu_f(f[e]);
+    const uint4 av = bf8_pack(f);
+    *reinterpret_cast<uint4*>(sH + r * LDH + c) = av;
+    if (r < rows) {
+      const int64_t g = (row0 + r) * H + c;
+      *reinterpret_cast<uint4*>(u + g) = uv;
+      *reinterpret_cast<uint4*>(a + g) = av;
+    }
+  }
+  __syncthreads();
+  bt_gemm<C, H, Cf::NW>(sH, W2, b2, bias_dt, sB);
+  __syncthreads();
+
+#pragma unroll
+  for (int p = 0; p < Cf::PASSES; ++p) {
+    const int r = p * Cf::RPP + pr;
+    if (r < rows) {
+      const int64_t g = (row0 + r) * C + pj;
+      const float s = rs2 ? rs2[row0 + r] : 1.f;
+      const float4 y = bt_lds_ld4(sB + r * LDC + pj);
+      float4 v = xm[p];
+      v.x += s * y.x; v.y += s * y.y; v.z += s * y.z; v.w += s * y.w;
+      *reinterpret_cast<float4*>(x_out + g) = v;
+      if (xcopy) *reinterpret_cast<uint2*>(xcopy + g) = bt_pack4(v);
+    }
+  }
+}
+
+template <int C>
+__global__ void __launch_bounds__(BtCfg<C>::THREADS)
+k_block_tail_bwd(const float* __restrict__ g_xout, const unsigned short* __restrict__ g_xcopy, const float* __restrict__ x_mid,
+                 const float* __restrict__ mean, const float* __restrict__ rstd, const unsigned short* __restrict__ u,
+                 const float* __restrict__ rs1, const float* __restrict__ rs2, const float* __restrict__ gamma,
+                 const unsigned short* __restrict__ Wpt, const unsigned short* __restrict__ W1t,
+                 const unsigned short* __restrict__ W2t, float* __restrict__ g_mid, unsigned short* __restrict__ dfeat,
+                 unsigned short* __restrict__ dy2, unsigned short* __restrict__ du, unsigned short* __restrict__ dy1,
+                 float* __restrict__ part , int64_t n) {
+  using Cf = BtCfg<C>;
+  constexpr int H = 4 * C, LDC = Cf::LDC, LDH = Cf::LDH, T = Cf::THREADS;
+  __shared__ __attribute__((aligned(16))) unsigned short sA[BT_R * LDC];
+  __shared__ __attribute__((aligned(16))) unsigned short sB[BT_R * LDC];
+  __shared__ __attribute__((aligned(16))) unsigned short sH[BT_R * LDH];
+  static_assert(2 * Cf::RPP * C * 4 <= BT_R * LDH * 2, "column partials must fit the hidden tile");
+  const int pr = threadIdx.x / Cf::LPR, pj = (threadIdx.x % Cf::LPR) * 4;
+  const float4 gm = *reinterpret_cast<const float4*>(gamma + pj);
+  float4 dg = make_float4(0.f, 0.f, 0.f, 0.f), db = dg;
+  const int64_t ntiles = (n + BT_R - 1) / BT_R;
+
+  for (int64_t tile = blockIdx.x; tile < ntiles; tile += gridDim.x) {
+    const int64_t row0 = tile * BT_R;
+    const int rows = (int)((n - row0) < BT_R ? (n - row0) : BT_R);
+    float4 gr[Cf::PASSES];
+#pragma unroll
+    for (int p = 0; p < Cf::PASSES; ++p) {
+      const int r = p * Cf::RPP + pr;
+      const int64_t g = (row0 + r) * C + pj;
+      float4 v = make_float4(0.f, 0.f, 0.f, 0.f);
+      float s = 0.f;
+      if (r < rows) {
+        v = *reinterpret_cast<const float4*>(g_xout + g);
+        if (g_xcopy) { const float4 e = ln_ld4(g_xcopy, SS_BF16, g); v.x += e.x; v.y += e.y; v.z += e.z; v.w += e.w; }
+        s = rs2 ? rs2[row0 + r] : 1.f;
+      }
+      gr[p] = v;
+      const uint2 d = bt_pack4(make_float4(s * v.x, s * v.y, s * v.z, s * v.w));
+      *reinterpret_cast<uint2*>(sA + r * LDC + pj) = d;
+      if (r < rows) *reinterpret_cast<uint2*>(dy2 + g) = d;
+    }
+    __syncthreads();
+    bt_gemm<H, C, Cf::NW>(sA, W2t, nullptr, SS_F32, sH);
+    __syncthreads();
+    for (int i = threadIdx.x; i < BT_R * (H / 4); i += T) {
+      const int r = i / (H / 4), c = (i % (H / 4)) * 4;
+      const int64_t g = (row0 + r) * H + c;
+      float4 f = bt_lds_ld4(sH + r * LDH + c);
+      float4 z = make_float4(0.f, 0.f, 0.f, 0.f);
+      if (r < rows) z = ln_ld4(u, SS_BF16, g);
+      f.x *= dgelu_exact(z.x); f.y *= dgelu_exact(z.y); f.z *= dgelu_exact(z.z); f.w *= dgelu_exact(z.w);
+      const uint2 dv = bt_pack4(f);
+      *reinterpret_cast<uint2*>(sH + r * LDH + c) = dv;
+      if (r < rows) *reinterpret_cast<uint2*>(du + g) = dv;
+    }
+    __syncthreads();
+    bt_gemm<C, H, Cf::NW>(sH, W1t, nullptr, SS_F32, sB);
+    __syncthreads();
+#pragma unroll
+    for (int p = 0; p < Cf::PASSES; ++p) {
+      const int r = p * Cf::RPP + pr;
+      const bool valid = r < rows;
+      const int64_t g = (row0 + r) * C + pj;
+      float4 xv = make_float4(0.f, 0.f, 0.f, 0.f), gh = xv;
+      float mu = 0.f, rr = 0.f, s = 0.f;
+      if (valid) {
+        xv = *reinterpret_cast<const float4*>(x_mid + g);
+        gh = bt_lds_ld4(sB + r * LDC + pj);
+        mu = mean[row0 + r]; rr = rstd[row0 + r];
+        s = rs1 ? rs1[row0 + r] : 1.f;
+      }
+      const float4 xh = ln_xhat4(xv, mu, rr);
+      const float4 gy = make_float4(gh.x * gm.x, gh.y * gm.y, gh.z * gm.z, gh.w * gm.w);
+      const float c1 = lanes_reduce_sum<Cf::LPR>(ln_sum4(gy)) / C;
+      const float c2 = lanes_reduce_sum<Cf::LPR>(gy.x * xh.x + gy.y * xh.y + gy.z * xh.z + gy.w * xh.w) / C;
+      float4 gv = ln_dx4(gy, xh, c1, c2, rr);
+      gv.x += gr[p].x; gv.y += gr[p].y; gv.z += gr[p].z; gv.w += gr[p].w;
+      dg.x += gh.x * xh.x; dg.y += gh.y * xh.y; dg.z += gh.z * xh.z; dg.w += gh.w * xh.w;
+      db.x += gh.x; db.y += gh.y; db.z += gh.z; db.w += gh.w;
+      const uint2 d = bt_pack4(make_float4(s * gv.x, s * gv.y, s * gv.z, s * gv.w));
+      *reinterpret_cast<uint2*>(sA + r * LDC + pj) = d;
+      if (valid) {
+        *reinterpret_cast<float4*>(g_mid + g) = gv;
+        *reinterpret_cast<uint2*>(dy1 + g) = d;
+      }
+    }
+    __syncthreads();
+    bt_gemm<C, C, Cf::NW>(sA, Wpt, nullptr, SS_F32, sB);
+    __syncthreads();
+    bt_tile_store<C, T>(sB, dfeat + row0 * C, rows);
+    __syncthreads();
+  }
+
+  float* red = reinterpret_cast<float*>(sH);
+  *reinterpret_cast<float4*>(red + (0 * Cf::RPP + pr) * C + pj) = dg;
+  *reinterpret_cast<float4*>(red + (1 * Cf::RPP + pr) * C + pj) = db;
+  __syncthreads();
+  for (int j = threadIdx.x; j < 2 * C; j += T) {
+    const int k = j / C, c = j - k * C;
+    float acc = 0.f;
+    for (int q = 0; q < Cf::RPP; ++q) acc += red[(k * Cf::RPP + q) * C + c];
+    part[((int64_t)k * gridDim.x + blockIdx.x) * C + c] = acc;
+  }
+}
+
+extern "C" int ss_block_tail_rows(void) { return BT_R; }
+
+extern "C" int ss_block_tail_bwd_blocks(int64_t n) {
+  int64_t b = (n + BT_R - 1) / BT_R;
+  if (b > BT_MAX_BWD_BLOCKS) b = BT_MAX_BWD_BLOCKS;
+  return (int)(b < 1 ? 1 : b);
+}
+
+static bool bt_aligned16(const void* p) { return (reinterpret_cast<uintptr_t>(p) & 15) == 0; }
+
+extern "C" int ss_block_tail_fwd(const void* feat, const float* x, const float* rs1, const float* rs2, const void* wp,
+                                 const void* bp, const void* w1, const void* b1, const void* w2, const void* b2, int bias_dtype,
+                                 const float* gamma, const float* beta, float eps, float* x_mid, float* mean, float* rstd,
+                                 void* h2, void* u, void* a, float* x_out, void* xcopy_bf16, int64_t n, int channels,
+                                 hipStream_t stream) {
+  if (n < 0 || !(channels == 32 || channels == 64 || channels == 128 || channels == 256)) return SS_ERR_ARG;
+  if (bias_dtype != SS_F32 && bias_dtype != SS_BF16) return SS_ERR_ARG;
+  if (!feat || !x || !wp || !bp || !w1 || !b1 || !w2 || !b2 || !gamma || !beta || !x_mid || !mean || !rstd || !h2 || !u || !a || !x_out)
+    return SS_ERR_ARG;
+  const void* al[] = {feat, x, wp, w1, w2, gamma, beta, x_mid, h2, u, a, x_out, xcopy_bf16};
+  for (const void* p : al) if (!bt_aligned16(p)) return SS_ERR_ARG;
+  if (n == 0) return SS_OK;
+  const dim3 g((unsigned)((n + BT_R - 1) / BT_R));
+#define SS_BT_FWD(CC) SS_LAUNCH(k_block_tail_fwd<CC>, g, dim3(BtCfg<CC>::THREADS), 0, stream, (const unsigned short*)feat, x, rs1, rs2, \
+    (const unsigned short*)wp, bp, (const unsigned short*)w1, b1, (const unsigned short*)w2, b2, bias_dtype, gamma, beta, eps, x_mid, mean, rstd, \
+    (unsigned short*)h2, (unsigned short*)u, (unsigned short*)a, x_out, (unsigned short*)xcopy_bf16, n)
+  switch (channels) { case 32: SS_BT_FWD(32); break; case 64: SS_BT_FWD(64); break; case 128: SS_BT_FWD(128); break; default: SS_BT_FWD(256); break; }
+#undef SS_BT_FWD
+  return SS_OK;
+}
+
+extern "C" int ss_block_tail_bwd(const float* g_xout, const void* g_xcopy_bf16, const float* x_mid, const float* mean,
+                                 const float* rstd, const void* u, const float* rs1, const float* rs2, const float* gamma,
+                                 const void* wp_t, const void* w1_t, const void* w2_t, float* g_mid, void* dfeat, void* dy2,
+                                 void* du, void* dy1, float* part, int64_t n, int channels, int nblocks, hipStream_t stream) {
+  if (n < 0 || !(channels == 32 || channels == 64 || channels == 128 || channels == 256)) return SS_ERR_ARG;
+  if (!g_xout || !x_mid || !mean || !rstd || !u || !gamma || !wp_t || !w1_t || !w2_t || !g_mid || !dfeat || !dy2 || !du || !dy1 || !part)
+    return SS_ERR_ARG;
+  if (nblocks < 1 || nblocks > BT_MAX_BWD_BLOCKS) return SS_ERR_ARG;
+  const void* al[] = {g_xout, g_xcopy_bf16, x_mid, u, gamma, wp_t, w1_t, w2_t, g_mid, dfeat, dy2, du, dy1};
+  for (const void* p : al) if (!bt_aligned16(p)) return SS_ERR_ARG;
+  if (n == 0) return SS_OK;
+  const dim3 g((unsigned)nblocks);
+#define SS_BT_BWD(CC) SS_LAUNCH(k_block_tail_bwd<CC>, g, dim3(BtCfg<CC>::THREADS), 0, stream, g_xout, (const unsigned short*)g_xcopy_bf16, \
+    x_mid, mean, rstd, (const unsigned short*)u, rs1, rs2, gamma, (const unsigned short*)wp_t, (const unsigned short*)w1_t, \
+    (const unsigned short*)w2_t, g_mid, (unsigned short*)dfeat, (unsigned short*)dy2, (unsigned short*)du, (unsigned short*)dy1, part, n)
+  switch (channels) { case 32: SS_BT_BWD(32); break; case 64: SS_BT_BWD(64); break; case 128: SS_BT_BWD(128); break; default: SS_BT_BWD(256); break; }
+#undef SS_BT_BWD
+  return SS_OK;
+}
diff --git a/scenesplat_amd/csrc/norm.hip b/scenesplat_amd/csrc/norm.hip
--- a/scenesplat_amd/csrc/norm.hip
+++ b/scenesplat_amd/csrc/norm.hip
@@ -1,20 +1,10 @@
 #include "common.h"
+#include "rowmath.h"
 #include "../../include/scenesplat_hip.h"
 
 #define LN_THREADS 256
 #define LN_MAXIT 4
 
-__device__ __forceinline__ float4 ln_ld4(const void* p, int dtype, int64_t idx) {
-  if (dtype == SS_F32) return *reinterpret_cast<const float4*>((const float*)p + idx);
-  uint2 u = *reinterpret_cast<const uint2*>((const unsigned short*)p + idx);
-  return make_float4(__uint_as_float(u.x << 16), __uint_as_float(u.x & 0xffff0000u), __uint_as_float(u.y << 16),
-                     __uint_as_float(u.y & 0xffff0000u));
-}
-__device__ __forceinline__ void ln_st4(void* p, int dtype, int64_t idx, float4 v) {
-  if (dtype == SS_F32) { *reinterpret_cast<float4*>((float*)p + idx) = v; return; }
-  uint2 u; u.x = pack_bf16x2(v.x, v.y); u.y = pack_bf16x2(v.z, v.w);
-  *reinterpret_cast<uint2*>((unsigned short*)p + idx) = u;
-}
 
 template <int IT>
 __global__ void __launch_bounds__(LN_THREADS)
@@ -38,7 +28,7 @@
       v[i] = a;
       if (xout) ln_st4(xout, xout_dt, row * C + j, a);
       if (xcopy) ln_st4(xcopy, SS_BF16, row * C + j, a);
-      sum += a.x + a.y + a.z + a.w;
+      sum += ln_sum4(a);
     }
   }
   if (!gamma) return;
@@ -47,10 +37,7 @@
 #pragma unroll
   for (int i = 0; i < IT; ++i) {
     int j = i * 256 + lane * 4;
-    if (j < C) {
-      float dx = v[i].x - mu, dy = v[i].y - mu, dz = v[i].z - mu, dw = v[i].w - mu;
-      sq += dx * dx + dy * dy + dz * dz + dw * dw;
-    }
+    if (j < C) sq += ln_sqdev4(v[i], mu);
   }
   const float r = rsqrtf(wave_reduce_sum(sq) / C + eps);
   if (lane == 0) { mean[row] = mu; rstd[row] = r; }
@@ -59,9 +46,7 @@
     int j = i * 256 + lane * 4;
     if (j < C) {
       float4 g = *reinterpret_cast<const float4*>(gamma + j), b = *reinterpret_cast<const float4*>(beta + j);
-      float4 o = make_float4((v[i].x - mu) * r * g.x + b.x, (v[i].y - mu) * r * g.y + b.y, (v[i].z - mu) * r * g.z + b.z,
-                             (v[i].w - mu) * r * g.w + b.w);
-      ln_st4(h, h_dt, row * C + j, o);
+      ln_st4(h, h_dt, row * C + j, ln_apply4(v[i], mu, r, g, b));
     }
   }
 }
@@ -97,9 +82,9 @@
         xh[i] = make_float4(0.f, 0.f, 0.f, 0.f); gy[i] = xh[i];
         if (j < C) {
           float4 a = ln_ld4(v_in, v_dt, row * C + j), g = ln_ld4(g_h, gh_dt, row * C + j);
-          xh[i] = make_float4((a.x - mu) * r, (a.y - mu) * r, (a.z - mu) * r, (a.w - mu) * r);
+          xh[i] = ln_xhat4(a, mu, r);
           gy[i] = make_float4(g.x * gm[i].x, g.y * gm[i].y, g.z * gm[i].z, g.w * gm[i].w);
-          c1 += gy[i].x + gy[i].y + gy[i].z + gy[i].w;
+          c1 += ln_sum4(gy[i]);
           c2 += gy[i].x * xh[i].x + gy[i].y * xh[i].y + gy[i].z * xh[i].z + gy[i].w * xh[i].w;
           dg[i].x += g.x * xh[i].x; dg[i].y += g.y * xh[i].y; dg[i].z += g.z * xh[i].z; dg[i].w += g.w * xh[i].w;
           db[i].x += g.x; db[i].y += g.y; db[i].z += g.z; db[i].w += g.w;
@@ -108,8 +93,7 @@
       c1 = wave_reduce_sum(c1) / C; c2 = wave_reduce_sum(c2) / C;
 #pragma unroll
       for (int i = 0; i < IT; ++i)
-        gv[i] = make_float4(r * (gy[i].x - c1 - xh[i].x * c2), r * (gy[i].y - c1 - xh[i].y * c2),
-                            r * (gy[i].z - c1 - xh[i].z * c2), r * (gy[i].w - c1 - xh[i].w * c2));
+        gv[i] = ln_dx4(gy[i], xh[i], c1, c2, r);
     } else {
 #pragma unroll
       for (int i = 0; i < IT; ++i) gv[i] = make_float4(0.f, 0.f, 0.f, 0.f);
@@ -206,14 +190,14 @@
   for (int i = 0; i < IT; ++i) {
     int j = i * 256 + lane * 4;
     v[i] = make_float4(0.f, 0.f, 0.f, 0.f);
-    if (j < C) { v[i] = ln_ld4(t, t_dt, row * C + j); sum += v[i].x + v[i].y + v[i].z + v[i].w; }
+    if (j < C) { v[i] = ln_ld4(t, t_dt, row * C + j); sum += ln_sum4(v[i]); }
   }
   const float mu0 = wave_reduce_sum(sum) / C;
   float sq = 0.f;
 #pragma unroll
   for (int i = 0; i < IT; ++i) {
     int j = i * 256 + lane * 4;
-    if (j < C) { float a = v[i].x - mu0, b = v[i].y - mu0, c = v[i].z - mu0, d = v[i].w - mu0; sq += a * a + b * b + c * c + d * d; }
+    if (j < C) sq += ln_sqdev4(v[i], mu0);
   }
   const float r0 = rsqrtf(wave_reduce_sum(sq) / C + eps0);
   sum = 0.f;
@@ -227,7 +211,7 @@
       a.z += (v[i].z - mu0) * r0 * g.z + b.z; a.w += (v[i].w - mu0) * r0 * g.w + b.w;
       v[i] = a;
       *reinterpret_cast<float4*>(xout + row * C + j) = a;
-      sum += a.x + a.y + a.z + a.w;
+      sum += ln_sum4(a);
     }
   }
   const float mu1 = wave_reduce_sum(sum) / C;
@@ -235,7 +219,7 @@
 #pragma unroll
   for (int i = 0; i < IT; ++i) {
     int j = i * 256 + lane * 4;
-    if (j < C) { float a = v[i].x - mu1, b = v[i].y - mu1, c = v[i].z - mu1, d = v[i].w - mu1; sq += a * a + b * b + c * c + d * d; }
+    if (j < C) sq += ln_sqdev4(v[i], mu1);
   }
   const float r1 = rsqrtf(wave_reduce_sum(sq) / C + eps1);
   if (lane == 0) *reinterpret_cast<float4*>(stats + row * 4) = make_float4(mu0, r0, mu1, r1);
@@ -244,8 +228,7 @@
     int j = i * 256 + lane * 4;
     if (j < C) {
       float4 g = *reinterpret_cast<const float4*>(gamma1 + j), b = *reinterpret_cast<const float4*>(beta1 + j);
-      ln_st4(h, h_dt, row * C + j, make_float4((v[i].x - mu1) * r1 * g.x + b.x, (v[i].y - mu1) * r1 * g.y + b.y,
-                                               (v[i].z - mu1) * r1 * g.z + b.z, (v[i].w - mu1) * r1 * g.w + b.w));
+      ln_st4(h, h_dt, row * C + j, ln_apply4(v[i], mu1, r1, g, b));
     }
   }
 }
@@ -254,13 +237,11 @@
   {                                                                                                       \
     float c1_ = 0.f, c2_ = 0.f;                                                                           \
     _Pragma("unroll") for (int i = 0; i < IT; ++i) {                                                      \
-      c1_ += GY[i].x + GY[i].y + GY[i].z + GY[i].w;                                                       \
+      c1_ += ln_sum4(GY[i]);                                                                              \
       c2_ += GY[i].x * XH[i].x + GY[i].y * XH[i].y + GY[i].z * XH[i].z + GY[i].w * XH[i].w;               \
     }                                                                                                     \
     c1_ = wave_reduce_sum(c1_) / C; c2_ = wave_reduce_sum(c2_) / C;                                       \
-    _Pragma("unroll") for (int i = 0; i < IT; ++i)                                                        \
-      OUT[i] = make_float4(R * (GY[i].x - c1_ - XH[i].x * c2_), R * (GY[i].y - c1_ - XH[i].y * c2_),      \
-                           R * (GY[i].z - c1_ - XH[i].z * c2_), R * (GY[i].w - c1_ - XH[i].w * c2_));     \
+    _Pragma("unroll") for (int i = 0; i < IT; ++i) OUT[i] = ln_dx4(GY[i], XH[i], c1_, c2_, R);            \
   }
 
 template <int IT>
@@ -288,7 +269,7 @@
       if (j < C) {
         float4 a = *reinterpret_cast<const float4*>(xout + row * C + j), g = make_float4(0.f, 0.f, 0.f, 0.f);
         if (g_h) g = ln_ld4(g_h, gh_dt, row * C + j);
-        xh[i] = make_float4((a.x - st.z) * st.w, (a.y - st.z) * st.w, (a.z - st.z) * st.w, (a.w - st.z) * st.w);
+        xh[i] = ln_xhat4(a, st.z, st.w);
         const float4 gm1 = *reinterpret_cast<const float4*>(&gam[1][j]);
         gy[i] = make_float4(g.x * gm1.x, g.y * gm1.y, g.z * gm1.z, g.w * gm1.w);
         dg1[i].x += g.x * xh[i].x; dg1[i].y += g.y * xh[i].y; dg1[i].z += g.z * xh[i].z; dg1[i].w += g.w * xh[i].w;
@@ -312,7 +293,7 @@
       xh[i] = make_float4(0.f, 0.f, 0.f, 0.f); gy[i] = xh[i];
       if (j < C) {
         float4 a = ln_ld4(t, t_dt, row * C + j);
-        xh[i] = make_float4((a.x - st.x) * st.y, (a.y - st.x) * st.y, (a.z - st.x) * st.y, (a.w - st.x) * st.y);
+        xh[i] = ln_xhat4(a, st.x, st.y);
         const float4 gm0 = *reinterpret_cast<const float4*>(&gam[0][j]);
         gy[i] = make_float4(gv[i].x * gm0.x, gv[i].y * gm0.y, gv[i].z * gm0.z, gv[i].w * gm0.w);
         dg0[i].x += gv[i].x * xh[i].x; dg0[i].y += gv[i].y * xh[i].y; dg0[i].z += gv[i].z * xh[i].z; dg0[i].w += gv[i].w * xh[i].w;
@@ -380,10 +361,6 @@
   return SS_OK;
 }
 
-__device__ __forceinline__ float gelu_f(float z) { return 0.5f * z * (1.f + erff(z * 0.70710678118654752f)); }
-__device__ __forceinline__ float dgelu_f(float z) {
-  return 0.5f * (1.f + erff(z * 0.70710678118654752f)) + z * 0.3989422804014327f * __expf(-0.5f * z * z);
-}
 
 template <int IT>
 __device__ __forceinline__ void col_partials_store(float4 (&a)[IT], float4 (&b)[IT], float* pa, float* pb, int C) {
@@ -687,17 +664,6 @@
 }
 
 
-__device__ __forceinline__ float dgelu_exact(float z) {
-  return 0.5f * (1.f + erff(z * 0.70710678118654752f)) + z * 0.3989422804014327f * expf(-0.5f * z * z);
-}
-__device__ __forceinline__ void bf8_unpack(const uint4& u, float (&v)[8]) {
-  v[0] = __uint_as_float(u.x << 16); v[1] = __uint_as_float(u.x & 0xffff0000u); v[2] = __uint_as_float(u.y << 16); v[3] = __uint_as_float(u.y & 0xffff0000u);
-  v[4] = __uint_as_float(u.z << 16); v[5] = __uint_as_float(u.z & 0xffff0000u); v[6] = __uint_as_float(u.w << 16); v[7] = __uint_as_float(u.w & 0xffff0000u);
-}
-__device__ __forceinline__ uint4 bf8_pack(const float (&v)[8]) {
-  uint4 o; o.x = pack_bf16x2(v[0], v[1]); o.y = pack_bf16x2(v[2], v[3]); o.z = pack_bf16x2(v[4], v[5]); o.w = pack_bf16x2(v[6], v[7]);
-  return o;
-}
 
 template <bool BWD>
 __global__ void __launch_bounds__(256)
diff --git a/scenesplat_amd/csrc/rowmath.h b/scenesplat_amd/csrc/rowmath.h
--- /dev/null
+++ b/scenesplat_amd/csrc/rowmath.h
@@ -0,0 +1,51 @@
+#pragma once
+#include "common.h"
+
+__device__ __forceinline__ float4 ln_ld4(const void* p, int dtype, int64_t idx) {
+  if (dtype == SS_F32) return *reinterpret_cast<const float4*>((const float*)p + idx);
+  uint2 u = *reinterpret_cast<const uint2*>((const unsigned short*)p + idx);
+  return make_float4(__uint_as_float(u.x << 16), __uint_as_float(u.x & 0xffff0000u), __uint_as_float(u.y << 16),
+                     __uint_as_float(u.y & 0xffff0000u));
+}
+__device__ __forceinline__ void ln_st4(void* p, int dtype, int64_t idx, float4 v) {
+  if (dtype == SS_F32) { *reinterpret_cast<float4*>((float*)p + idx) = v; return; }
+  uint2 u; u.x = pack_bf16x2(v.x, v.y); u.y = pack_bf16x2(v.z, v.w);
+  *reinterpret_cast<uint2*>((unsigned short*)p + idx) = u;
+}
+
+__device__ __forceinline__ float gelu_f(float z) { return 0.5f * z * (1.f + erff(z * 0.70710678118654752f)); }
+__device__ __forceinline__ float dgelu_f(float z) {
+  return 0.5f * (1.f + erff(z * 0.70710678118654752f)) + z * 0.3989422804014327f * __expf(-0.5f * z * z);
+}
+__device__ __forceinline__ float dgelu_exact(float z) {
+  return 0.5f * (1.f + erff(z * 0.70710678118654752f)) + z * 0.3989422804014327f * expf(-0.5f * z * z);
+}
+__device__ __forceinline__ void bf8_unpack(const uint4& u, float (&v)[8]) {
+  v[0] = __uint_as_float(u.x << 16); v[1] = __uint_as_float(u.x & 0xffff0000u); v[2] = __uint_as_float(u.y << 16); v[3] = __uint_as_float(u.y & 0xffff0000u);
+  v[4] = __uint_as_float(u.z << 16); v[5] = __uint_as_float(u.z & 0xffff0000u); v[6] = __uint_as_float(u.w << 16); v[7] = __uint_as_float(u.w & 0xffff0000u);
+}
+__device__ __forceinline__ uint4 bf8_pack(const float (&v)[8]) {
+  uint4 o; o.x = pack_bf16x2(v[0], v[1]); o.y = pack_bf16x2(v[2], v[3]); o.z = pack_bf16x2(v[4], v[5]); o.w = pack_bf16x2(v[6], v[7]);
+  return o;
+}
+
+__device__ __forceinline__ float ln_sum4(const float4& a) { return a.x + a.y + a.z + a.w; }
+__device__ __forceinline__ float ln_sqdev4(const float4& a, float mu) {
+  const float dx = a.x - mu, dy = a.y - mu, dz = a.z - mu, dw = a.w - mu;
+  return dx * dx + dy * dy + dz * dz + dw * dw;
+}
+__device__ __forceinline__ float4 ln_apply4(const float4& v, float mu, float r, const float4& g, const float4& b) {
+  return make_float4((v.x - mu) * r * g.x + b.x, (v.y - mu) * r * g.y + b.y, (v.z - mu) * r * g.z + b.z, (v.w - mu) * r * g.w + b.w);
+}
+__device__ __forceinline__ float4 ln_xhat4(const float4& a, float mu, float r) {
+  return make_float4((a.x - mu) * r, (a.y - mu) * r, (a.z - mu) * r, (a.w - mu) * r);
+}
+__device__ __forceinline__ float4 ln_dx4(const float4& gy, const float4& xh, float c1, float c2, float r) {
+  return make_float4(r * (gy.x - c1 - xh.x * c2), r * (gy.y - c1 - xh.y * c2), r * (gy.z - c1 - xh.z * c2), r * (gy.w - c1 - xh.w * c2));
+}
+template <int W>
+__device__ __forceinline__ float lanes_reduce_sum(float v) {
+#pragma unroll
+  for (int o = W / 2; o > 0; o >>= 1) v += __shfl_xor(v, o, 64);
+  return v;
+}
diff --git a/scenesplat_amd/functional.py b/scenesplat_amd/functional.py
--- a/scenesplat_amd/functional.py
+++ b/scenesplat_amd/functional.py
@@ -532,6 +532,12 @@
             ent[1] = None
 
 
+def unregister_transposed(weights):
+    for p in weights:
+        if p in _SHADOW_T:
+            del _SHADOW_T[p]
+
+
 def bf16_t_of(p):
     if not isinstance(p, torch.nn.Parameter):
         return None
@@ -897,6 +903,135 @@
         ga, be = gamma, beta
         stage = _eff_stage(ga, be) if ga is not None else None
     return _AddLayerNorm.apply(x, y, rowscale, ga, be, eps, want_copy, h_dtype, stage)
+
+
+BLOCK_TAIL_CHANNELS = (32, 64, 128, 256)
+BLOCK_TAIL_MAX_CHANNELS = int(os.environ.get("SS_BLOCK_TAIL_MAX_CHANNELS", "64"))
+BLOCK_TAIL_CALLS = 0
+
+
+def block_tail_rows():
+    return int(nv.lib().ss_block_tail_rows())
+
+
+def block_tail_fwd_raw(feat, x, rs1, rs2, wp, bp, w1, b1, w2, b2, gamma, beta, eps, want_copy):
+    n, C = x.shape
+    H = 4 * C
+    rq = nv._req
+    rq(feat, torch.bfloat16, "feat", (n, C)); rq(x, torch.float32, "x")
+    rq(wp, torch.bfloat16, "wp", (C, C)); rq(w1, torch.bfloat16, "w1", (H, C)); rq(w2, torch.bfloat16, "w2", (C, H))
+    rq(bp, None, "bp", (C,)); rq(b1, bp.dtype, "b1", (H,)); rq(b2, bp.dtype, "b2", (C,))
+    rq(gamma, torch.float32, "gamma", (C,)); rq(beta, torch.float32, "beta", (C,))
+    for t, nm in ((rs1, "rs1"), (rs2, "rs2")):
+        if t is not None:
+            rq(t, torch.float32, nm, (n,))
+    dev = x.device
+    o = dict(x_mid=torch.empty((n, C), dtype=torch.float32, device=dev), mean=torch.empty(n, dtype=torch.float32, device=dev),
+             rstd=torch.empty(n, dtype=torch.float32, device=dev), h2=torch.empty((n, C), dtype=torch.bfloat16, device=dev),
+             u=torch.empty((n, H), dtype=torch.bfloat16, device=dev), a=torch.empty((n, H), dtype=torch.bfloat16, device=dev),
+             x_out=torch.empty((n, C), dtype=torch.float32, device=dev),
+             xcopy=torch.empty((n, C), dtype=torch.bfloat16, device=dev) if want_copy else None)
+    p = nv._p
+    nv.check(nv.lib().ss_block_tail_fwd(p(feat), p(x), p(rs1), p(rs2), p(wp), p(bp), p(w1), p(b1), p(w2), p(b2), nv.dtype_code(bp), p(gamma), p(beta),
+                                        float(eps), p(o["x_mid"]), p(o["mean"]), p(o["rstd"]), p(o["h2"]), p(o["u"]), p(o["a"]),
+                                        p(o["x_out"]), p(o["xcopy"]), n, C, nv._stream()), "ss_block_tail_fwd")
+    return o
+
+
+def block_tail_bwd_raw(g_xout, g_xcopy, x_mid, mean, rstd, u, rs1, rs2, gamma, wpt, w1t, w2t, nblocks=None):
+    n, C = x_mid.shape
+    H = 4 * C
+    rq = nv._req
+    rq(g_xout, torch.float32, "g_xout", (n, C)); rq(x_mid, torch.float32, "x_mid"); rq(u, torch.bfloat16, "u", (n, H))
+    rq(mean, torch.float32, "mean", (n,)); rq(rstd, torch.float32, "rstd", (n,)); rq(gamma, torch.float32, "gamma", (C,))
+    rq(wpt, torch.bfloat16, "wp_t", (C, C)); rq(w1t, torch.bfloat16, "w1_t", (C, H)); rq(w2t, torch.bfloat16, "w2_t", (H, C))
+    if g_xcopy is not None:
+        rq(g_xcopy, torch.bfloat16, "g_xcopy", (n, C))
+    for t, nm in ((rs1, "rs1"), (rs2, "rs2")):
+        if t is not None:
+            rq(t, torch.float32, nm, (n,))
+    dev = x_mid.device
+    nb = int(nv.lib().ss_block_tail_bwd_blocks(n)) if nblocks is None else int(nblocks)
+    g_mid = torch.empty((n, C), dtype=torch.float32, device=dev)
+    dfeat, dy2, dy1 = (torch.empty((n, C), dtype=torch.bfloat16, device=dev) for _ in range(3))
+    du = torch.empty((n, H), dtype=torch.bfloat16, device=dev)
+    part = torch.empty((2, nb, C), dtype=torch.float32, device=dev)
+    p = nv._p
+    nv.check(nv.lib().ss_block_tail_bwd(p(g_xout), p(g_xcopy), p(x_mid), p(mean), p(rstd), p(u), p(rs1), p(rs2), p(gamma), p(wpt),
+                                        p(w1t), p(w2t), p(g_mid), p(dfeat), p(dy2), p(du), p(dy1), p(part), n, C, nb, nv._stream()),
+             "ss_block_tail_bwd")
+    return g_mid, dfeat, dy2, du, dy1, part
+
+
+class _BlockTail(torch.autograd.Function):
+
+    @staticmethod
+    def forward(ctx, feat, x, rs1, rs2, wp, bp, w1, b1, w2, b2, gamma, beta, eps, want_copy, stage, ops):
+        global BLOCK_TAIL_CALLS
+        BLOCK_TAIL_CALLS += 1
+        feat, x = feat.contiguous(), x.contiguous()
+        g32 = gamma.detach().contiguous()
+        o = block_tail_fwd_raw(feat, x, rs1, rs2, ops[0], ops[6], ops[1], ops[7], ops[2], ops[8], g32, beta.detach().contiguous(), eps,
+                               want_copy)
+        ctx.save_for_backward(feat, o["x_mid"], o["mean"], o["rstd"], o["h2"], o["u"], o["a"], rs1, rs2, g32, ops[3], ops[4], ops[5])
+        ctx.stage = stage
+        ctx.set_materialize_grads(False)
+        return o["x_out"], o["xcopy"]
+
+    @staticmethod
+    def backward(ctx, g_xout, g_xcopy):
+        feat, x_mid, mean, rstd, h2, u, a, rs1, rs2, g32, wpt, w1t, w2t = ctx.saved_tensors
+        if g_xout is None and g_xcopy is None:
+            return (None,) * 16
+        g_xout = g_xout.float().contiguous() if g_xout is not None else torch.zeros_like(x_mid)
+        g_xcopy = g_xcopy.contiguous().to(torch.bfloat16) if g_xcopy is not None else None
+        g_mid, dfeat, dy2, du, dy1, part = block_tail_bwd_raw(g_xout, g_xcopy, x_mid, mean, rstd, u, rs1, rs2, g32, wpt, w1t, w2t)
+        need = ctx.needs_input_grad
+        stage = ctx.stage
+        _, dwp, dbp = _linear_backward(feat, None, False, torch.float32, True, stage, dy1, False, need[4], need[5])
+        _, dw1, db1 = _linear_backward(h2, None, False, torch.float32, True, stage, du, False, need[6], need[7])
+        _, dw2, db2 = _linear_backward(a, None, False, torch.float32, True, stage, dy2, False, need[8], need[9])
+        dg = db = None
+        if need[10] or need[11]:
+            if stage is not None:
+                dst = torch.empty((2, part.shape[2]), dtype=torch.float32, device=part.device)
+                stage.redq.append((part, dst))
+                _UNFLUSHED.add(stage)
+                dg, db = dst[0], dst[1]
+            else:
+                red = part.sum(1)
+                dg, db = red[0], red[1]
+        return (dfeat if need[0] else None, g_mid if need[1] else None, None, None, dwp, dbp, dw1, db1, dw2, db2, dg, db,
+                None, None, None, None)
+
+
+def block_tail_eligible(x, proj, ln2, fc1, fc2):
+    C = x.shape[1]
+    if not (x.is_cuda and x.dim() == 2 and x.dtype == torch.float32 and C in BLOCK_TAIL_CHANNELS and C <= BLOCK_TAIL_MAX_CHANNELS):
+        return False
+    if type(ln2) is not torch.nn.LayerNorm or ln2.weight is None or ln2.bias is None or tuple(ln2.normalized_shape) != (C,):
+        return False
+    if tuple(proj.weight.shape) != (C, C) or tuple(fc1.weight.shape) != (4 * C, C) or tuple(fc2.weight.shape) != (C, 4 * C):
+        return False
+    for p in (proj.weight, proj.bias, fc1.weight, fc1.bias, fc2.weight, fc2.bias, ln2.weight, ln2.bias):
+        if not isinstance(p, torch.nn.Parameter) or p.dtype != torch.float32 or not p.is_cuda or not p.is_contiguous():
+            return False
+    for w in (proj.weight, fc1.weight, fc2.weight):
+        ent = _SHADOW.get(w)
+        if ent is None or not _shadow_current(ent, w) or bf16_t_of(w) is None:
+            return False
+    return True
+
+
+def block_tail(feat, x, rs1, rs2, proj, ln2, fc1, fc2, want_copy=False):
+    params = (proj.weight, proj.bias, fc1.weight, fc1.bias, fc2.weight, fc2.bias, ln2.weight, ln2.bias)
+    routed = [_routed(p) for p in params] if torch.is_grad_enabled() else [(p, None) for p in params]
+    stage = routed[0][1]
+    if stage is None or any(s is not stage for _, s in routed):
+        stage, routed = None, [(p, None) for p in params]
+    ops = tuple(bf16_of(w) for w in (proj.weight, fc1.weight, fc2.weight)) + tuple(bf16_t_of(w) for w in (proj.weight, fc1.weight, fc2.weight)) \
+        + tuple(bf16_of(b) for b in (proj.bias, fc1.bias, fc2.bias))
+    return _BlockTail.apply(feat.to(torch.bfloat16), x, rs1, rs2, *[a for a, _ in routed], ln2.eps, want_copy, stage, ops)
 
 
 class _BatchNormAct(torch.autograd.Function):
diff --git a/scenesplat_amd/pointcept_api/ptv3.py b/scenesplat_amd/pointcept_api/ptv3.py
--- a/scenesplat_amd/pointcept_api/ptv3.py
+++ b/scenesplat_amd/pointcept_api/ptv3.py
@@ -14,7 +14,8 @@
 
 RUNTIME = dict(attn_impl=nv.ATTN_SIMT, conv_dtype=None,
                attn_headmajor=os.environ.get("SS_ATTN_HM", "1") != "0",
-               param_shadows=os.environ.get("SS_PARAM_SHADOWS", "1") != "0")
+               param_shadows=os.environ.get("SS_PARAM_SHADOWS", "1") != "0",
+               fuse_block_tail=os.environ.get("SS_BLOCK_TAIL", "1") != "0")
 
 
 def bench_runtime():
@@ -113,7 +114,7 @@
             raise ValueError("enable_rpe: every batch element needs at least one point")
         return k
 
-    def _forward_rpe(self, x, level):
+    def _forward_rpe(self, x, level, pre_proj=False):
         win = level.window(self.order_index, self.rpe_window_size(level))
         qkv = _lin(self.qkv, x)
         bf16 = (x.is_cuda and torch.is_autocast_enabled() and torch.get_autocast_dtype("cuda") == torch.bfloat16) \
@@ -125,24 +126,24 @@
         a = qkv.to(torch.bfloat16) if bf16 else qkv
         feat = SF.window_attention_rpe(a, win, level.grid_coord, self.rpe.rpe_table, self.rpe.pos_bnd, self.num_heads,
                                        self.scale, impl).to(qkv.dtype)
-        return _lin(self.proj, feat)
-
-    def forward(self, x, level):
+        return feat if pre_proj else _lin(self.proj, feat)
+
+    def forward(self, x, level, pre_proj=False):
         if self.enable_rpe:
-            return self._forward_rpe(x, level)
+            return self._forward_rpe(x, level, pre_proj)
         win = level.window(self.order_index, self.patch_size)
         impl = RUNTIME["attn_impl"]
         if (impl == nv.ATTN_MFMA and RUNTIME.get("attn_headmajor", True) and x.is_cuda and torch.is_autocast_enabled()
                 and torch.get_autocast_dtype("cuda") == torch.bfloat16 and self.qkv.weight.dtype == torch.float32
                 and (self.channels // self.num_heads) in (16, 32, 48, 64)):
             feat = SF.qkv_window_attention(x, self.qkv.weight, self.qkv.bias, win, self.num_heads, self.scale)
-            return _lin(self.proj, feat)
+            return feat if pre_proj else _lin(self.proj, feat)
         qkv = _lin(self.qkv, x)
         if impl == nv.ATTN_MFMA and qkv.dtype != torch.bfloat16:
             feat = SF.window_attention(qkv.to(torch.bfloat16), win, self.num_heads, self.scale, impl).to(qkv.dtype)
         else:
             feat = SF.window_attention(qkv, win, self.num_heads, self.scale, impl)
-        return _lin(self.proj, feat)
+        return feat if pre_proj else _lin(self.proj, feat)
 
 
 class MLP(nn.Module):
@@ -189,9 +190,25 @@
         else:
             t = SF.layer_norm(t, ln0.weight, ln0.bias, ln0.eps)
             x, h, _ = SF.add_layer_norm(x, t, None, ln1.weight, ln1.bias, ln1.eps, False, hdt)
+        if self._tail_fusable(x, ln2):
+            feat = self.attn(h, level, pre_proj=True)
+            rs1, rs2 = self._row_scale(x), self._row_scale(x)
+            mlp = self.mlp[0]
+            return SF.block_tail(feat, x, rs1, rs2, self.attn.proj, ln2, mlp.fc1, mlp.fc2, want_copy)
         x, h, _ = SF.add_layer_norm(x, self.attn(h, level), self._row_scale(x), ln2.weight, ln2.bias, ln2.eps, False, hdt)
         x, _, xb = SF.add_layer_norm(x, self.mlp(h), self._row_scale(x), None, None, 0.0, want_copy, hdt)
         return x, xb
+
+    def _tail_fusable(self, x, ln2):
+        if not (RUNTIME.get("fuse_block_tail", True) and RUNTIME.get("fuse_ln_seam", True) and x.is_cuda
+                and torch.is_autocast_enabled() and torch.get_autocast_dtype("cuda") == torch.bfloat16):
+            return False
+        mlp = self.mlp[0]
+        if isinstance(self.norm2[0], PDNorm):
+            return False
+        if not (isinstance(mlp, MLP) and type(mlp.act) is nn.GELU and getattr(mlp.act, "approximate", "none") == "none"):
+            return False
+        return SF.block_tail_eligible(x, self.attn.proj, ln2, mlp.fc1, mlp.fc2)
 
     def _row_scale(self, x):
         dp = self.drop_path[0]
@@ -432,7 +449,8 @@
 
     def _refresh_shadows(self):
         ps = self.__dict__.get("_shadow_lists")
-        if ps is None or ps[2] != next(self.parameters()).device:
+        tail = SF.BLOCK_TAIL_MAX_CHANNELS if RUNTIME.get("fuse_block_tail", True) else 0
+        if ps is None or ps[2] != next(self.parameters()).device or ps[4] != tail:
             params, skip = [], self._modulation_linears()
             for m in self.modules():
                 if isinstance(m, nn.Linear) and id(m) not in skip:
@@ -446,10 +464,18 @@
                     wide += [m.weight for m in st.modules() if isinstance(m, nn.Linear) and m.weight.numel() >= 65536]
             if RUNTIME.get("dgrad_nt", True):
                 SF.register_transposed(wide)
+            keep = {id(w) for w in wide} if RUNTIME.get("dgrad_nt", True) else set()
+            mine = [w for m in self.modules() if isinstance(m, Block) and m.channels in SF.BLOCK_TAIL_CHANNELS and m.channels <= tail
+                    and m.pre_norm and not isinstance(m.norm2[0], PDNorm)
+                    and tuple(m.mlp[0].fc1.weight.shape) == (4 * m.channels, m.channels)
+                    for w in (m.attn.proj.weight, m.mlp[0].fc1.weight, m.mlp[0].fc2.weight) if id(w) not in keep]
+            SF.unregister_transposed([w for w in self.__dict__.get("_tail_transposed", []) if id(w) not in {id(v) for v in mine}])
+            SF.register_transposed(mine)
+            self.__dict__["_tail_transposed"] = mine
             SF.register_mirrored([m.weight for m in self.modules() if isinstance(m, SubMConv3d)
                                   and conv_dtype_for(m.weight.shape[0]) == torch.bfloat16])
             total = sum(((p.numel() + 3) & ~3) for p in params if p is not None) + 4 * len(params)
-            ps = (src, dst, next(self.parameters()).device, total)
+            ps = (src, dst, next(self.parameters()).device, total, tail)
             self.__dict__["_shadow_lists"] = ps
         SF.refresh_shadows(ps[0], ps[1])
         if torch.is_grad_enabled():
```

After: 2.860 million (median of 6 runs). 1.02x the previous value.
